# ztaylor797/APMBackend

Hardware: AMD Instinct MI355X
Metric: log-lines/sec z-scored (whole node) (higher is better)
Workload: dtype fp64

## Files before the change

### apmbackend_amd/csrc/kernels/devjoin.hip

```cpp
#include "kernel_api.h"

#include <rocprim/rocprim.hpp>

#include <chrono>
#include <climits>
#include <cstdlib>
#include <cstddef>
#include <cstring>
#include <vector>

#include "devjoin_api.h"
#include "devjoin_dev.h"
#include "devscan.h"
#include "prim.h"
#include "textout.h"

namespace apm {
using namespace dj;

namespace {

constexpr int TB = 256;

__device__ __forceinline__ uint32_t grid_n(uint32_t n) { return (n + TB - 1) / TB; }
// ... 330 lines not shown
          f.flags = PRE_SOAP_VALID;
        }
      }
      return 1;
    }
  }
  return 0;
}

enum : uint8_t { SEL_HOST = 1, SEL_MH = 2, SEL_WALK = 4 };

constexpr int SEL_MH_SHIFT = 22, SEL_WALK_SHIFT = 43;
__device__ __forceinline__ SelCount sel_unpack(uint64_t v) {
  return SelCount{(uint32_t)(v & ((1ull << SEL_MH_SHIFT) - 1)),
                  (uint32_t)((v >> SEL_MH_SHIFT) & ((1ull << (SEL_WALK_SHIFT - SEL_MH_SHIFT)) - 1)),
                  (uint32_t)(v >> SEL_WALK_SHIFT), 0u};
}

constexpr int HF_SLOT = 256;
constexpr int HF_PITCH = HF_SLOT + 16;

__device__ __forceinline__ bool hf_needs_bytes(const Event& e) {
  if (e.kind == LK_APP) return !(e.mask & PM_HOST);
  if (e.mask & PM_HOST) return false;
  if (e.kind == LK_CT_EXIT) return (e.mask & PM_KEYS) && e.ntok >= 3 && (e.mask & PM_BAF);
  if (e.kind == LK_SOAP) return (e.mask & (PM_SOAP_IN | PM_SOAP_ACCT | PM_SOAP_VALUE)) != 0;
  return false;
}

__device__ __forceinline__ uint8_t hf_fields(const Event& e, const uint8_t* __restrict__ p, uint64_t fkey, AudF* aud,
                                             uint32_t i) {
  uint8_t fl = 0;
  if (e.kind == LK_APP) {
    bool host = (e.mask & PM_HOST) != 0;
    if (!host) {
      AudF f;
      host = !aud_fields(e, p, fkey, f);
      if (!host) aud[i] = f;
    }
    if (host) fl |= SEL_HOST;
  } else {
    AudF f;
    const int r = pre_fields(e, p, f);
    if (r < 0) fl |= SEL_HOST;
    else if (r > 0) aud[i] = f;
  }
  return fl;
}

__device__ __forceinline__ uint32_t wave_append(bool want, uint32_t* counter) {
  const uint64_t m = __ballot(want);
  if (!m) return ~0u;
  const uint32_t lane = threadIdx.x & (APM_WAVE - 1);
  const uint32_t leader = (uint32_t)__ffsll((unsigned long long)m) - 1u;
  uint32_t base = 0;
  if (lane == leader) base = atomicAdd(counter, (uint32_t)__popcll(m));
  base = (uint32_t)__shfl((int)base, (int)leader, APM_WAVE);
  return want ? base + (uint32_t)__popcll(m & ((1ull << lane) - 1ull)) : ~0u;
}

__device__ __forceinline__ uint64_t sel_pack(uint8_t fl) {
  return (uint64_t)(fl & SEL_HOST) | ((fl & SEL_MH) ? 1ull << SEL_MH_SHIFT : 0ull) |
         ((fl & SEL_WALK) ? 1ull << SEL_WALK_SHIFT : 0ull);
}

__device__ __forceinline__ uint8_t app_bits(const Event& e) {
  if (e.kind != LK_APP) return 0;
  return (e.mask & PM_AUTR_MAP) ? SEL_MH : (uint8_t)(SEL_WALK | ((e.mask & PM_AUTR_HDR) ? SEL_MH : 0));
}

__device__ __forceinline__ uint8_t hf_event(const Event& e, uint32_t i, const uint8_t* __restrict__ bytes,
                                            const uint32_t* __restrict__ chunk_file,
                                            const uint64_t* __restrict__ file_fkey, AudF* __restrict__ aud,
                                            uint8_t* stage) {
  const uint64_t fkey = e.kind == LK_APP ? file_fkey[chunk_file[e.chunk]] : 0;
  const uint8_t* p = bytes + e.off;
  const uint32_t lead = e.off & 15u;
  const uint32_t nvec = (lead + e.len + 15u) >> 4;
  if (hf_needs_bytes(e) && nvec * 16u <= (uint32_t)HF_SLOT) {
    const uint4* __restrict__ src = reinterpret_cast<const uint4*>(bytes + (e.off - lead));
    uint4* dst = reinterpret_cast<uint4*>(stage + threadIdx.x * HF_PITCH);
    for (uint32_t k = 0; k < nvec; k += 4) {
      const uint4 v0 = src[k];
      const uint4 v1 = k + 1 < nvec ? src[k + 1] : v0;
      const uint4 v2 = k + 2 < nvec ? src[k + 2] : v0;
      const uint4 v3 = k + 3 < nvec ? src[k + 3] : v0;
      dst[k] = v0;
      if (k + 1 < nvec) dst[k + 1] = v1;
      if (k + 2 < nvec) dst[k + 2] = v2;
      if (k + 3 < nvec) dst[k + 3] = v3;
    }
    p = stage + threadIdx.x * HF_PITCH + lead;
  }
  return (uint8_t)(hf_fields(e, p, fkey, aud, i) | app_bits(e));
}

__global__ __launch_bounds__(TB) void k_host_flags(const Event* __restrict__ ev, const uint32_t* __restrict__ n_ev_dev,
                                                   const uint8_t* __restrict__ bytes,
                                                   uint8_t* __restrict__ flag, uint64_t* __restrict__ val,
                                                   AudF* __restrict__ aud, SelCount* __restrict__ totals, uint32_t cap,
                                                   uint32_t* __restrict__ list, uint32_t* __restrict__ list_n) {
  const uint32_t i = blockIdx.x * blockDim.x + threadIdx.x;
  const uint32_t n = min(*n_ev_dev, cap);
  if (blockIdx.x * blockDim.x >= n) return;
  uint32_t ab = 0;
  Event e;
  bool defer = false, front = false;
  if (i < n) {
    e = ev[i];
    if (e.kind == LK_APP && (e.mask & (PM_AUTR_MAP | PM_SW_NAME))) ab = e.len;
    defer = hf_needs_bytes(e);
    front = defer && e.kind == LK_APP;
  }
  const uint32_t f = wave_append(front, &list_n[0]);
  const uint32_t b = wave_append(defer && !front, &list_n[1]);
  if (front) list[f] = i;
  if (defer && !front) list[cap - 1 - b] = i;
  if (i < n && !defer) {
    const uint8_t fl = (uint8_t)(hf_fields(e, bytes + e.off, 0, aud, i) | app_bits(e));
    flag[i] = fl;
    val[i] = sel_pack(fl);
  }
  for (int o = APM_WAVE / 2; o > 0; o >>= 1) ab += __shfl_xor(ab, o, APM_WAVE);
  if ((threadIdx.x & (APM_WAVE - 1)) == 0 && ab) atomicAdd(&totals->aud_bytes, ab);
}

__global__ __launch_bounds__(TB) void k_host_flags_bytes(const Event* __restrict__ ev, const uint8_t* __restrict__ bytes,
                                                         const uint32_t* __restrict__ chunk_file,
                                                         const uint64_t* __restrict__ file_fkey,
                                                         uint8_t* __restrict__ flag, uint64_t* __restrict__ val,
                                                         AudF* __restrict__ aud, uint32_t cap,
                                                         const uint32_t* __restrict__ list,
                                                         const uint32_t* __restrict__ list_n) {
  __shared__ __attribute__((aligned(16))) uint8_t stage[TB * HF_PITCH];
  const uint32_t nf = list_n[0], nb = list_n[1];
  const uint32_t b0 = blockIdx.x * blockDim.x, b1 = b0 + blockDim.x;
  if (b0 >= nf && b1 <= cap - nb) return;
  const uint32_t t = b0 + threadIdx.x;
  if (t >= cap || (t >= nf && t < cap - nb)) return;
  const uint32_t i = list[t];
  const Event e = ev[i];
  const uint8_t fl = hf_event(e, i, bytes, chunk_file, file_fkey, aud, stage);
  flag[i] = fl;
  val[i] = sel_pack(fl);
}

struct SelValF {
  const uint64_t* val;
  __device__ uint64_t operator()(uint32_t i) const { return val[i]; }
};
struct SelScatterG {
  const Event* ev;
  const uint8_t* flag;
  const uint64_t* total;
  Event* out;
  uint32_t *out_idx, *mh_idx, *walk_idx;
  SelCount* totals;
  __device__ void operator()(uint32_t i, uint64_t pos) const {
    if (i == 0) {
      const SelCount t = sel_unpack(*total);
      totals->host = t.host; totals->mh = t.mh; totals->walk = t.walk;
    }
    const uint8_t fl = flag[i];
    if (!fl) return;
    const SelCount p = sel_unpack(pos);
    if (fl & SEL_HOST) { out[p.host] = ev[i]; out_idx[p.host] = i; }
    if (fl & SEL_MH) mh_idx[p.mh] = i;
    if (fl & SEL_WALK) walk_idx[p.walk] = i;
  }
};

enum : uint8_t { SC_NONE = 0, SC_IN = 1, SC_OUT = 2, SC_ACCT = 3, SC_KEY = 4, SC_VALUE = 5 };

__device__ const HostOp* find_hop(const HostOp* __restrict__ h, uint32_t n, uint32_t ev) {
  uint32_t lo = 0, hi = n;
  while (lo < hi) {
    const uint32_t mid = (lo + hi) >> 1;
    if (h[mid].ev < ev) lo = mid + 1; else hi = mid;
  }
  return (lo < n && h[lo].ev == ev) ? &h[lo] : nullptr;
}

__global__ __launch_bounds__(TB) void k_build_ops(DJArgs a) {
  const uint32_t i = blockIdx.x * blockDim.x + threadIdx.x;
  if (i >= a.n_ev) return;
  const Event e = a.ev[i];
  JOp op;
  op.gkey = 0; op.svc = 0; op.ts = apm_nan(); op.num = apm_nan(); op.aux = apm_nan(); op.aux2 = apm_nan();
  op.line = e.line; op.lid = 0; op.svc_ref = 0; op.lid_len = 0; op.svc_len = 0;
  op.flags = 0; op.op = JOP_NONE; op.pad = 0;
  const int32_t file = (int32_t)a.chunk_file[e.chunk];
  const int32_t server = a.file_server[file];
  const uint64_t skey = a.file_skey[file];
  op.server = server;
  uint8_t code = SC_NONE;
  double snum = apm_nan();
  uint64_t shash = 0;
  const uint8_t* p = a.bytes + e.off;
  if (e.kind == LK_APP) {
    AudF f;
    bool ok = false;
    if (a.host_flag[i] & SEL_HOST) {
      const HostOp* h = find_hop(a.hops, a.n_hops, i);
      if (h && h->kind == HOP_AUD) { f = *reinterpret_cast<const AudF*>(&h->op); ok = true; }
      if (!ok) {
        f.h_item = 0; f.el = apm_nan(); f.h_sw = 0; f.ts = apm_nan(); f.ref = 0; f.len = 0; f.flags = 0;
      }
      a.aud[i] = f;
    } else {
      f = a.aud[i];
    }
    if ((e.mask & PM_AUTR_MAP) && (f.flags & AF_ACCT)) {
      if (!(f.flags & AF_ACCT_VALID)) {
        atomicAdd(&a.counts->invalid_acct, 1ULL);
      } else if (f.len > 0) {
        op.op = JOP_ACCT;
        op.gkey = gkey_of(f.h_sw, skey);
        op.num = f.el;
      }
    }
  } else if (a.host_flag[i] & SEL_HOST) {
    const HostOp* h = find_hop(a.hops, a.n_hops, i);
    if (h) {
      switch (h->kind) {
        case HOP_JOIN: op = h->op; break;
        case HOP_SOAP_IN: code = SC_IN; shash = h->lid_hash; break;
        case HOP_SOAP_OUT: code = SC_OUT; break;
        case HOP_SOAP_ACCT: if (h->op.flags & JF_BAF_VALID) { code = SC_ACCT; snum = h->op.num; } break;
        case HOP_SOAP_KEY: code = SC_KEY; break;
        case HOP_SOAP_VALUE: if (h->op.flags & JF_BAF_VALID) { code = SC_VALUE; snum = h->op.num; } break;
        default: break;
      }
    }
  } else if (e.kind >= LK_EJB_ENTRY && e.kind <= LK_CT_EXIT) {
    const bool ejb = e.kind <= LK_EJB_EXIT;
    const bool entry = e.kind == LK_EJB_ENTRY || e.kind == LK_CT_ENTRY;
    op.lid = e.off + e.t0s;
    op.lid_len = (uint16_t)(e.t0e - e.t0s);
    op.svc = e.svc;
    op.flags = JF_HAS_SVC | (ejb ? JF_EJB : 0);
    if (e.tAs == 0xffff) op.flags |= JF_SVC_UNDEF;
    else { op.svc_ref = e.off + e.tAs; op.svc_len = (uint16_t)(e.tAe - e.tAs); }
    op.ts = e.ts;
    const bool empty_lid = op.lid_len == 0;
    if (entry) {
      if (!empty_lid) { op.op = JOP_ENTRY; op.gkey = gkey_of(e.key, skey); }
      else op.flags = 0;
    } else {
      op.num = (e.kind == LK_EJB_EXIT || e.tBs != 0xffff) ? e.num : apm_nan();
      if (e.kind == LK_CT_EXIT && (e.mask & PM_BAF)) {
        const AudF& f = a.aud[i];
        if (f.flags & PRE_BAF) {
          op.flags |= JF_BAF;
          op.aux = f.el;
          if (f.flags & PRE_BAF_VALID) { op.flags |= JF_BAF_VALID; op.aux2 = f.el; }
        }
      }
      if (empty_lid) op.op = JOP_DIRECT;
      else { op.op = e.kind == LK_EJB_EXIT ? JOP_EJB_EXIT : JOP_CT_EXIT; op.gkey = gkey_of(e.key, skey); }
    }
  } else if (e.kind == LK_SOAP) {
    const uint32_t m = e.mask;
    if (m & PM_SOAP_IN) {
      code = SC_IN;
      shash = a.aud[i].h_item;
    } else if (m & PM_SOAP_OUT) {
      code = SC_OUT;
    } else if (m & (PM_SOAP_ACCT | PM_SOAP_KEY | PM_SOAP_VALUE)) {
      const bool acct = m & PM_SOAP_ACCT;
      if (!acct && (m & PM_SOAP_KEY)) {
        code = SC_KEY;
      } else {
        const AudF& f = a.aud[i];
        if (f.flags & PRE_SOAP_VALID) {
          snum = f.el;
          code = acct ? SC_ACCT : SC_VALUE;
        }
      }
    }
  }
  a.ops[i] = op;
  a.soap_code[i] = code;
  a.soap_num[i] = snum;
  a.soap_hash[i] = shash;
}

constexpr uint32_t F_CONST = 1u << 31;
constexpr uint32_t F_ID = 1u | (2u << 2);
constexpr uint32_t F_KEY = 2u | (2u << 2);
constexpr uint32_t F_VALUE = 1u | (0u << 2);

__device__ __forceinline__ uint32_t map_tag(uint32_t g, uint32_t tag) {
  return tag == 0 ? 0u : (tag == 1 ? (g & 3u) : ((g >> 2) & 3u));
}
__device__ __forceinline__ uint32_t fcompose(uint32_t g, uint32_t f) {
  if (g & F_CONST) return g;
  if (f & F_CONST) {
    const uint32_t t = map_tag(g, f & 3u);
    return t ? (F_CONST | t | (f & ~(F_CONST | 3u))) : F_CONST;
  }
  return map_tag(g, f & 3u) | (map_tag(g, (f >> 2) & 3u) << 2);
}
__device__ __forceinline__ uint32_t code_fn(uint8_t c, uint32_t ev) {
  switch (c) {
    case SC_IN: return F_CONST | 1u | ((ev + 1) << 2);
    case SC_OUT: case SC_ACCT: return F_CONST;
    case SC_KEY: return F_KEY;
    case SC_VALUE: return F_VALUE;
    default: return F_ID;
  }
}

__device__ __forceinline__ void soap_range(const uint32_t* lo_tab, uint32_t c, int g, uint32_t& lo, uint32_t& hi) {
  const uint32_t c0 = lo_tab[c], c1 = lo_tab[c + 1];
  const uint32_t n = c1 - c0;
  const uint32_t seg = ((n + SOAP_SEGS - 1) / SOAP_SEGS + APM_WAVE - 1) / APM_WAVE * APM_WAVE;
  lo = min(c1, c0 + (uint32_t)g * seg);
  hi = min(c1, lo + seg);
}

__device__ __forceinline__ uint32_t wave_fscan(uint32_t f, int lane) {
// ... 744 lines not shown

constexpr uint32_t GWB_LDS = 4096;
constexpr int GWB_THREADS = 256;
__global__ __launch_bounds__(GWB_THREADS) void k_group_walk_big(DJArgs a) {
  __shared__ uint32_t lds[GWB_LDS];
  __shared__ uint32_t s_g, s_off;
  const uint32_t nb = a.big[0];
  for (uint32_t b = blockIdx.x; b < nb; b += gridDim.x) {
    const uint32_t slot = a.op_slot_sorted[b];
    if (threadIdx.x == 0) {
      uint32_t g = 0;
      for (uint32_t j = a.slot_head[slot]; j != ~0u; j = a.op_idx[j]) ++g;
      const uint32_t off = atomicAdd(&a.big[1], g);
      uint32_t k = 0;
      for (uint32_t j = a.slot_head[slot]; j != ~0u; j = a.op_idx[j]) a.op_idx_sorted[off + k++] = j;
      a.slot_head[slot] = ~0u;
      s_g = g;
      s_off = off;
    }
    __syncthreads();
    const uint32_t g = s_g;
    uint32_t* v = a.op_idx_sorted + s_off;
    if (g <= GWB_LDS) {
      for (uint32_t t = threadIdx.x; t < g; t += blockDim.x) lds[t] = v[t];
      __syncthreads();
      v = lds;
    }
    block_sort_asc(v, g);
    if (threadIdx.x == 0) walk_group(a, slot, [v](uint32_t q) { return v[q]; }, g);
    __syncthreads();
  }
}

template <class M>
__device__ void walk_group(DJArgs& a, uint32_t slot, const M& mem, uint32_t g) {
  KeyState ks = a.table[slot];
  const double now = a.now;
  bool acct_live = ks.acct_exp >= now;
  if (!(ks.rec_exp >= now) && ks.n_part > 0) {
    atomicAdd(&a.counts->expired_partials, (unsigned long long)ks.n_part);
    part_clear(a, ks);
  }
  NeedEnt* ne = nullptr;
  int32_t nidx = -1;
  if (ks.need >= 0) {
    NeedEnt* c = &a.arena[ks.need];
    if (c->key == ks.key && c->exp >= now) { ne = c; nidx = ks.need; }
  }
  for (uint32_t q = 0; q < g; ++q) {
    const uint32_t ev = mem(q);
    const JOp op = a.ops[ev];
    Emitter em{a.stage, a.ovf, &a.counts->pad[0], ev, 0};
    const bool ts_empty = (op.flags & JF_TS_EMPTY) != 0;
    switch (op.op) {
      case JOP_ENTRY: {
        if (!(ks.rec_exp >= now)) { ks.rec_exp = now + a.rec_ttl; part_clear(a, ks); }
        const int f = part_find(a, ks, op.svc);
        if (f >= 0) part_set(a, ks, f, op.svc, op.ts);
        else if (!part_append(a, ks, op.svc, op.ts)) atomicAdd(&a.counts->partial_overflow, 1ULL);
        break;
      }
      case JOP_EJB_EXIT:
      case JOP_CT_EXIT: {
        const bool ct = op.op == JOP_CT_EXIT;
        const int f = (ks.rec_exp >= now) ? part_find(a, ks, op.svc) : -1;
        if (f < 0) {
          if (!ct) { atomicAdd(&a.counts->ejb_unmatched, 1ULL); break; }
          if ((op.flags & JF_BAF) && (op.flags & JF_BAF_VALID)) {
            ks.acct = op.aux2; ks.acct_exp = now + a.acct_ttl; acct_live = true;
            if (ne && ne->n) need_drain(a, *ne, nidx, op.aux2, em);
          } else if (op.flags & JF_BAF) {
            atomicAdd(&a.counts->invalid_acct, 1ULL);
          }
          em.put(make_tx(op.server, op.svc, LID_NONE, 0, 0, (op.flags & JF_BAF) ? op.aux : apm_nan(), 0.0, true,
                         op.ts, ts_empty, op.num, false));
          break;
        }
        const double pstart = part_get_start(a, ks, f);
        auto remove_part = [&]() { part_remove(a, ks, f); };
        if (acct_live) {
          remove_part();
          em.put(make_tx(op.server, op.svc, lid_src_of(op), op.lid, op.lid_len, ks.acct, pstart, false, op.ts,
                         ts_empty, op.num, false));
          break;
        }
        if (!ne) { nidx = need_alloc(a, op, ks.key); ne = nidx >= 0 ? &a.arena[nidx] : nullptr; ks.need = nidx; }
        double alt = apm_nan();
        if (ct && (op.flags & JF_BAF)) {
          alt = op.aux;
          if (op.flags & JF_BAF_VALID) {
            ks.acct = op.aux2; ks.acct_exp = now + a.acct_ttl; acct_live = true;
            if (ne && ne->n) need_drain(a, *ne, nidx, op.aux2, em);
          } else {
            atomicAdd(&a.counts->invalid_acct, 1ULL);
          }
        }
        if (ne) {
          NeedItem it;
          it.svc = op.svc; it.start = pstart; it.end = op.ts; it.elapsed = op.num; it.alt = alt;
          it.flags = ts_empty ? JF_TS_EMPTY : 0; it.pad = 0;
          need_put(a, *ne, it);
        }
        remove_part();
        break;
      }
      case JOP_ACCT: {
        ks.acct = op.num; ks.acct_exp = now + a.acct_ttl; acct_live = true;
        if (ne && ne->n) need_drain(a, *ne, nidx, op.num, em);
        break;
      }
      case JOP_AUDIT_TX: {
        const bool to_db = (op.flags & JF_TO_DB) != 0;
        if (acct_live) {
          em.put(make_tx(op.server, op.svc, lid_src_of(op), op.lid, op.lid_len, ks.acct, op.aux,
                         (op.flags & JF_START_EMPTY) != 0, op.ts, ts_empty, op.num, to_db));
          break;
        }
        if (!ne) { nidx = need_alloc(a, op, ks.key); ne = nidx >= 0 ? &a.arena[nidx] : nullptr; ks.need = nidx; }
        if (ne) {
          NeedItem it;
          it.svc = op.svc; it.start = op.aux; it.end = op.ts; it.elapsed = op.num; it.alt = op.aux2;
          it.flags = (ts_empty ? JF_TS_EMPTY : 0) | ((op.flags & JF_START_EMPTY) ? JF_START_EMPTY : 0) | (to_db ? JF_TO_DB : 0);
          it.pad = 0;
          need_put(a, *ne, it);
        }
        break;
      }
      default: break;
    }
    a.out_cnt[ev] = em.sub;
  }
  a.table[slot] = ks;
}

__global__ __launch_bounds__(TB) void k_exp_keys(DJArgs a) {
  const uint32_t e = blockIdx.x * blockDim.x + threadIdx.x;
  if (e >= a.n_exp_entries) return;
  uint64_t rem = e, v = 0;
  for (uint32_t r = 0; r < a.n_exp_regions; ++r) {
    const uint64_t n = a.exp_hi[r] - a.exp_lo[r];
    if (rem < n) { v = a.exp_lo[r] + rem; break; }
    rem -= n;
  }
  const uint32_t idx = (uint32_t)(v & (uint64_t)(a.arena_cap - 1));
  const NeedEnt& ne = a.arena[idx];
  a.exp_key[e] = ne.n > 0 ? ne.created : ~0ULL;
  a.exp_idx[e] = idx;
  if (ne.n == 0) {
    a.arena[idx].key = 0;
    if (ne.lblk) chain_free(a.pool, a.pool_ring, a.pool_mask, a.counts, ne.lblk);
  }
}

__global__ __launch_bounds__(TB) void k_exp_count(DJArgs a) {
  const uint32_t e = blockIdx.x * blockDim.x + threadIdx.x;
  if (e > a.n_exp_entries) return;
  if (e == a.n_exp_entries) { a.exp_cnt[e] = 0; return; }
  a.exp_cnt[e] = a.exp_key_sorted[e] == ~0ULL ? 0u : (uint32_t)a.arena[a.exp_idx_sorted[e]].n;
}

__global__ void k_exp_emit(DJArgs a) {
  const uint32_t e = blockIdx.x * blockDim.x + threadIdx.x;
  if (e == 0) {
    a.counts->n_exp_out = a.n_exp_entries ? a.exp_pos[a.n_exp_entries] : 0;
    atomicAdd(&a.counts->need_expired, (unsigned long long)a.counts->n_exp_out);
  }
  if (e >= a.n_exp_entries) return;
  const uint32_t n = a.exp_cnt[e];
  if (!n) return;
  const uint32_t idx = a.exp_idx_sorted[e];
  NeedEnt& ne = a.arena[idx];
  const uint32_t base = a.exp_pos[e];
  int32_t b = 0;
  for (uint32_t k = 0; k < n && base + k < a.out_cap; ++k) {
    const NeedItem& r = need_item(a.pool, ne, (int)k, b);
    a.out[base + k] = make_tx(ne.server, r.svc, LID_NEED, idx, (uint32_t)ne.lid_len, r.alt, r.start,
                              (r.flags & JF_START_EMPTY) != 0, r.end, (r.flags & JF_TS_EMPTY) != 0, r.elapsed,
                              (r.flags & JF_TO_DB) != 0);
  }
  if (ne.iblk) chain_free(a.pool, a.pool_ring, a.pool_mask, a.counts, ne.iblk);
  if (ne.lblk) chain_free(a.pool, a.pool_ring, a.pool_mask, a.counts, ne.lblk);
  ne.iblk = 0;
  ne.n = 0;
  ne.key = 0;
}

__global__ __launch_bounds__(TB) void k_place(DJArgs a) {
  const uint32_t i = blockIdx.x * blockDim.x + threadIdx.x;
  const uint32_t base = a.counts->n_exp_out;
  if (i == 0) a.counts->n_out = base + a.out_pos[a.n_ev];
  if (i >= a.n_ev * 2) return;
  const uint32_t ev = i >> 1, sub = i & 1;
  if (sub >= a.out_cnt[ev]) return;
  const uint32_t p = base + a.out_pos[ev] + sub;
  if (p < a.out_cap) a.out[p] = a.stage[(size_t)ev * 2 + sub];
}

__global__ __launch_bounds__(TB) void k_place_ovf(DJArgs a) {
  const uint32_t k = blockIdx.x * blockDim.x + threadIdx.x;
  const uint32_t n = min(a.counts->pad[0], DJ_OVF_CAP);
  if (k >= n) return;
  const DJOverflow& o = a.ovf[k];
  const uint32_t p = a.counts->n_exp_out + a.out_pos[o.ev] + o.sub;
  if (p < a.out_cap) a.out[p] = o.t;
}

struct U4 {
  uint32_t x, y, z, w;
};
struct U4Plus {
  __device__ __host__ U4 operator()(const U4& a, const U4& b) const { return U4{a.x + b.x, a.y + b.y, a.z + b.z, a.w + b.w}; }
};

__device__ __forceinline__ const char* lid_ptr(const DJFormatArgs& f, const TxDev& t) {
  switch (t.lid_src) {
    case LID_BATCH: return (const char*)f.bytes + t.lid;
    case LID_HOST: return (const char*)f.hbuf + t.lid;
    case LID_NEED: return f.arena[t.lid & (f.arena_cap - 1)].lid;
    case LID_AUD: return f.aud_txt + t.lid;
    default: return "";
  }
}

__device__ __forceinline__ bool stat_usable(const TxDev& t) { return !t.to_db && t.end == t.end && t.end >= 10000.0; }

__device__ uint32_t line_len(const DJFormatArgs& f, const TxDev& t) {
  if (t.raw < 0) return 0;
  const RawSvc rs = f.raw[t.raw];
  uint32_t n = 3 + rs.srv_len + 1 + rs.norm_len + 1 + t.lid_len + 1;
  n += js_num(nullptr, t.acct, nullptr) + 1 + js_num(nullptr, t.start, nullptr) + 1 + js_num(nullptr, t.end, nullptr) +
       1 + js_num(nullptr, t.elapsed, nullptr) + 1 + 1;
  return n + 1;
}

__global__ __launch_bounds__(TB) void k_resolve_len(DJFormatArgs f) {
  const uint32_t i = blockIdx.x * blockDim.x + threadIdx.x;
  const uint32_t n = f.n_out;
  U4* lens = reinterpret_cast<U4*>(f.lens);
  if (i == n) { lens[n] = U4{0, 0, 0, 0}; return; }
  if (i > n) return;
  TxDev t = f.out[i];
  const int32_t raw = reg_find(f.reg, f.reg_mask, regkey_of(t.svc, t.server));
  t.raw = raw >= 0 ? raw : -1;
  f.out[i].raw = t.raw;
  const uint32_t len = line_len(f, t);
  const bool st = stat_usable(t);
  lens[i] = U4{len, st ? 1u : 0u, t.to_db ? 0u : len, t.to_db ? len : 0u};
  if (t.to_db) atomicAdd(&f.counts->n_db, 1u);
  else if (!st) atomicAdd(&f.counts->n_dropped, 1u);
}

__global__ void k_plan_totals(DJFormatArgs f) {
  const U4 o = reinterpret_cast<const U4*>(f.offs)[f.n_out];
  f.counts->text_bytes = o.x;
  f.counts->n_stats = o.y;
  f.counts->tx_text_bytes = o.z;
  f.counts->db_text_bytes = o.w;
  const uint64_t base = ring_place(f.ring_head, o.x, f.ring_cap);
  uint32_t v = DJ_WRITE_OK;
  if ((uint64_t)o.x > f.ring_cap / 4) v = DJ_WRITE_TOO_BIG;
  else if (base + o.x > f.ring_low + f.ring_cap) v = DJ_WRITE_RING_FULL;
  else if ((f.want_tx && o.z > f.txt_cap) || (f.want_db && o.w > f.txt_cap)) v = DJ_WRITE_TXT;
  *f.ring_pos = base;
  f.counts->pad[1] = v;
}

__device__ __forceinline__ uint32_t tx_head_len(const TxDev& t, const RawSvc& rs) {
  return 3u + rs.srv_len + 1u + rs.norm_len + 1u + t.lid_len + 1u;
}
template <class O>
__device__ __forceinline__ void tx_line_head(const DJFormatArgs& f, const TxDev& t, const RawSvc& rs, O& o);
template <class O>
__device__ __forceinline__ void tx_line_tail(const TxDev& t, const RawSvc& rs, O& o, bool& inexact) {
  o.jsnum(t.acct, inexact); o.c('|');
  o.jsnum(t.start, inexact); o.c('|');
  o.jsnum(t.end, inexact); o.c('|');
  o.jsnum(t.elapsed, inexact); o.c('|');
  o.c(rs.toplevel ? 'Y' : 'N');
  o.c('\n');
}
template <class O>
__device__ __forceinline__ void tx_line(const DJFormatArgs& f, const TxDev& t, const RawSvc& rs, O& o, bool& inexact) {
  tx_line_head(f, t, rs, o);
  tx_line_tail(t, rs, o, inexact);
}
template <class O>
__device__ __forceinline__ void tx_line_head(const DJFormatArgs& f, const TxDev& t, const RawSvc& rs, O& o) {
  o.lit("tx|");
  o.s(f.names + rs.srv_off, rs.srv_len);
  o.c('|');
  o.s(f.names + rs.norm_off, rs.norm_len);
  o.c('|');
  if (t.lid_src != LID_NEED || t.lid_len <= NEED_LID) {
    o.s(lid_ptr(f, t), t.lid_len);
  } else {
    const NeedEnt& ne = f.arena[t.lid & (f.arena_cap - 1)];
    o.s((const char*)ne.lid, NEED_LID);
    int rem = (int)t.lid_len - NEED_LID;
    for (int32_t b = ne.lblk; b && rem > 0; b = blk_next(f.pool, b)) {
      const LidBlk* lb = (const LidBlk*)blk_ptr(f.pool, b);
      const int m = rem < LBLK_N ? rem : LBLK_N;
      o.s((const char*)lb->b, m);
      rem -= m;
    }
  }
  o.c('|');
}

constexpr int TXW_LINES = 64;
constexpr int TXW_THREADS = 2 * TXW_LINES;
constexpr uint32_t TXW_LDS = 8192;
__device__ __forceinline__ void write_one(const DJFormatArgs& f, const TxDev& t, uint32_t i, uint64_t ring_base,
                                          char* staged_line);
__device__ __forceinline__ void write_tail(const DJFormatArgs& f, const TxDev& t, uint32_t i, uint64_t ring_base,
                                           char* staged_line);

__device__ __forceinline__ void txw_copy_out(const char* __restrict__ lds, char* __restrict__ out, uint32_t g0,
                                             uint32_t g1) {
  const uint32_t a0 = g0 & ~3u;
  const uint32_t nd = (g1 - a0 + 3) / 4;
  for (uint32_t d = threadIdx.x; d < nd; d += blockDim.x) {
    const uint32_t ga = a0 + 4 * d;
    if (ga >= g0 && ga + 4 <= g1) {
      *reinterpret_cast<uint32_t*>(out + ga) = *reinterpret_cast<const uint32_t*>(lds + 4 * d);
    } else {
      for (uint32_t b = 0; b < 4; ++b)
        if (ga + b >= g0 && ga + b < g1) out[ga + b] = lds[4 * d + b];
    }
  }
}

__global__ __launch_bounds__(TXW_THREADS) void k_write(DJFormatArgs f) {
  __shared__ __align__(16) char stage[TXW_LDS];
  if (f.counts->pad[1] != DJ_WRITE_OK) return;
  const uint64_t ring_base = *f.ring_pos;
  const uint32_t j0 = blockIdx.x * TXW_LINES;
  const uint32_t j1 = min(f.n_out, j0 + TXW_LINES);
  const bool tail = threadIdx.x >= (unsigned)TXW_LINES;
  const uint32_t i = j0 + (threadIdx.x & (TXW_LINES - 1));
  const U4* offs = reinterpret_cast<const U4*>(f.offs);
  const uint64_t rb = ring_base & (f.ring_cap - 1);
  const uint32_t p0 = (uint32_t)(rb + offs[j0].x), p1 = (uint32_t)(rb + offs[j1].x);
  const bool staged = p1 - (p0 & ~3u) <= TXW_LDS;
  if (i < j1) {
    const TxDev t = f.out[i];
    char* const sl = staged ? stage + ((uint32_t)(rb + offs[i].x) - (p0 & ~3u)) : nullptr;
    if (t.raw >= 0) {
      if (tail) write_tail(f, t, i, ring_base, sl);
      else write_one(f, t, i, ring_base, sl);
    }
  }
  if (staged) {
    __syncthreads();
    txw_copy_out(stage, f.ring, p0, p1);
  }
}

__device__ __forceinline__ void write_tail(const DJFormatArgs& f, const TxDev& t, uint32_t i, uint64_t ring_base,
                                           char* staged_line) {
  const U4 o = reinterpret_cast<const U4*>(f.offs)[i];
  const uint64_t vpos = ring_base + o.x;
  char* p0 = staged_line ? staged_line : f.ring + (vpos & (f.ring_cap - 1));
  const RawSvc rs = f.raw[t.raw];
  bool inexact = false;
  OutT<true> w(p0 + tx_head_len(t, rs));
  tx_line_tail(t, rs, w, inexact);
  w.finish();
}

__device__ __forceinline__ void write_one(const DJFormatArgs& f, const TxDev& t, uint32_t i, uint64_t ring_base,
                                          char* staged_line) {
  const U4 o = reinterpret_cast<const U4*>(f.offs)[i];
  const U4 l = reinterpret_cast<const U4*>(f.lens)[i];
  const uint64_t vpos = ring_base + o.x;
  char* p0 = staged_line ? staged_line : f.ring + (vpos & (f.ring_cap - 1));
  const RawSvc rs = f.raw[t.raw];
  bool inexact = false;
  {
    OutT<true> w(p0);
    tx_line_head(f, t, rs, w);
    w.finish();
  }
  const uint32_t len = l.x;
  if (f.want_tx && !t.to_db) {
    OutT<true> w(f.txt_tx + o.z);
    tx_line(f, t, rs, w, inexact);
    w.finish();
  }
  if (f.want_db && t.to_db) {
    OutT<true> w(f.txt_db + o.w);
    tx_line(f, t, rs, w, inexact);
    w.finish();
  }
  if (l.y) {
    const uint32_t j = o.y;
    TxRec r;
    r.end_ms = (int64_t)t.end;
    const int32_t s = f.raw_series[t.raw];
    r.series = s;
    const double e = t.elapsed;
    r.elapsed = (e == e && e >= -2147483647.0 && e <= 2147483647.0) ? (int32_t)e : ELAPSED_NAN;
    f.tx[j] = r;
    f.tx_raw[j] = t.raw;
    f.tx_gid[j] = (int64_t)((vpos << 20) | (uint64_t)(len - 1));
    f.tx_bucket[j] = r.end_ms / 10000;
    if (s < 0) atomicMin(&f.raw_first[t.raw], (int32_t)j);
  }
}

__global__ __launch_bounds__(TB) void k_cands(DJFormatArgs f) {
  const uint32_t j = blockIdx.x * blockDim.x + threadIdx.x;
  if (f.counts->pad[1] != DJ_WRITE_OK || j >= f.counts->n_stats) return;
  if (j == 0 || f.tx_bmax[j] > f.tx_bmax[j - 1]) {
    const uint32_t k = atomicAdd(&f.counts->n_cand, 1u);
    f.cand[k] = j;
    f.cand_bucket[k] = f.tx_bucket[j];
  }
  const int32_t r = f.tx_raw[j];
  if (f.raw_first[r] == (int32_t)j) {
    const uint32_t k = atomicAdd(&f.counts->n_unresolved, 1u);
    f.unresolved[2 * k] = j;
    f.unresolved[2 * k + 1] = (uint32_t)r;
  }
}

__global__ void k_reset_first(DJFormatArgs f) {
  const uint32_t j = blockIdx.x * blockDim.x + threadIdx.x;
  if (f.counts->pad[1] != DJ_WRITE_OK || j >= f.counts->n_stats) return;
  const int32_t r = f.tx_raw[j];
  if (f.raw_first[r] != INT_MAX) f.raw_first[r] = INT_MAX;
}

__global__ void k_rebuild(const KeyState* __restrict__ old, uint32_t old_cap, KeyState* __restrict__ fresh,
                          uint32_t mask, const NeedEnt* __restrict__ arena, uint32_t arena_cap, double now,
                          JoinCounts* cnt, unsigned long long* live, const uint8_t* pool, uint32_t* pool_ring,
                          uint32_t pool_mask) {
  const uint32_t i = blockIdx.x * blockDim.x + threadIdx.x;
  if (i >= old_cap) return;
  KeyState s = old[i];
  if (!s.key) return;
  const bool rec = s.rec_exp >= now && s.n_part > 0;
  const bool acct = s.acct_exp >= now;
  bool need = false;
  if (s.need >= 0) {
    const NeedEnt& ne = arena[(uint32_t)s.need & (arena_cap - 1)];
    need = ne.key == s.key && ne.exp >= now;
  }
  if (!rec && s.n_part > 0 && !(s.rec_exp >= now)) atomicAdd(&cnt->expired_partials, (unsigned long long)s.n_part);
  if (!rec && s.pblk) {
    chain_free(pool, pool_ring, pool_mask, cnt, s.pblk);
    s.pblk = 0;
  }
  if (!rec && !acct && !need) return;
  if (!(s.rec_exp >= now)) s.n_part = 0;
  uint32_t h = home_of(s.key, mask);
  for (uint32_t probe = 0; probe <= mask; ++probe) {
    const uint32_t idx = (h + probe) & mask;
    if (atomicCAS((unsigned long long*)&fresh[idx].key, 0ULL, (unsigned long long)s.key) == 0ULL) {
      fresh[idx] = s;
      atomicAdd(live, 1ULL);
      return;
    }
  }
}

constexpr uint32_t RB_SEG = 8;

__global__ void k_rebuild_starts(const KeyState* __restrict__ t, uint32_t cap, uint32_t* __restrict__ starts) {
  const uint32_t seg = blockIdx.x * blockDim.x + threadIdx.x;
  const uint32_t n_seg = cap / RB_SEG;
  if (seg >= n_seg) return;
  const uint32_t mask = cap - 1, lo = seg * RB_SEG, hi = lo + RB_SEG;
  uint32_t p = lo;
  if (t[(lo + mask) & mask].key != 0)
    while (p < hi && t[p].key != 0) ++p;
  starts[seg] = p;
}

__device__ __forceinline__ bool rb_live(KeyState& s, const NeedEnt* __restrict__ arena, uint32_t arena_cap, double now,
                                        JoinCounts* cnt, const uint8_t* pool, uint32_t* pool_ring, uint32_t pool_mask,
                                        bool& changed) {
  const bool rec = s.rec_exp >= now && s.n_part > 0;
  const bool acct = s.acct_exp >= now;
  bool need = false;
  if (s.need >= 0) {
    const NeedEnt& ne = arena[(uint32_t)s.need & (arena_cap - 1)];
    need = ne.key == s.key && ne.exp >= now;
  }
  if (!rec && s.n_part > 0 && !(s.rec_exp >= now)) atomicAdd(&cnt->expired_partials, (unsigned long long)s.n_part);
  if (!rec && s.pblk) {
    chain_free(pool, pool_ring, pool_mask, cnt, s.pblk);
    s.pblk = 0;
    changed = true;
  }
  if (!rec && !acct && !need) return false;
  if (!(s.rec_exp >= now) && s.n_part != 0) { s.n_part = 0; changed = true; }
  return true;
}

constexpr int RB_TB = 128;
constexpr int RB_BITS = 1024;
__global__ __launch_bounds__(RB_TB) void k_rebuild_inplace(KeyState* __restrict__ t, uint32_t cap,
                                                           const uint32_t* __restrict__ starts,
                                                           const NeedEnt* __restrict__ arena, uint32_t arena_cap,
                                                           double now, JoinCounts* cnt, unsigned long long* live,
                                                           const uint8_t* pool, uint32_t* pool_ring, uint32_t pool_mask) {
  __shared__ uint32_t occ_s[RB_TB][RB_BITS / 32];
  uint32_t* occ = occ_s[threadIdx.x];
  const uint32_t seg = blockIdx.x * blockDim.x + threadIdx.x;
  const uint32_t n_seg = cap / RB_SEG;
  uint32_t n_live = 0;
  if (seg < n_seg) {
    const uint32_t mask = cap - 1, hi = seg * RB_SEG + RB_SEG;
    uint64_t p = starts[seg];
    while (p < hi) {
      if (t[p & mask].key == 0) { ++p; continue; }
      uint64_t q = p;
      while (t[q & mask].key != 0 && q < p + cap) ++q;
      const uint32_t L = (uint32_t)(q - p);
      if (L > RB_BITS) {
        n_live += L;
        p = q + 1;
        continue;
      }
      for (uint32_t i = 0; i < (L + 31) / 32; ++i) occ[i] = 0;
      for (uint64_t r = p; r < q; ++r) {
        KeyState s = t[r & mask];
        bool changed = false;
        if (!rb_live(s, arena, arena_cap, now, cnt, pool, pool_ring, pool_mask, changed)) continue;
        uint32_t i = (uint32_t)(r - (((uint32_t)r - home_of(s.key, mask)) & mask) - p);
        while (i < L && (occ[i >> 5] & (1u << (i & 31)))) ++i;
        if (i >= L) i = (uint32_t)(r - p);
        occ[i >> 5] |= 1u << (i & 31);
        if (p + i != r || changed) t[(p + i) & mask] = s;
        ++n_live;
      }
      for (uint32_t i = 0; i < L; ++i)
        if (!(occ[i >> 5] & (1u << (i & 31)))) t[(p + i) & mask].key = 0;
      p = q + 1;
    }
  }
  for (int o = APM_WAVE / 2; o > 0; o >>= 1) n_live += __shfl_xor(n_live, o, APM_WAVE);
  if ((threadIdx.x & (APM_WAVE - 1)) == 0 && n_live) atomicAdd(live, (unsigned long long)n_live);
}

__global__ __launch_bounds__(TB) void k_rebase_gids(const int64_t* __restrict__ gid, int64_t n,
                                                    const uint32_t* __restrict__ offs, uint64_t base,
                                                    int64_t* __restrict__ out) {
  const int64_t i = (int64_t)blockIdx.x * blockDim.x + threadIdx.x;
  if (i < n) out[i] = (int64_t)(((base + offs[i]) << 20) | ((uint64_t)gid[i] & 0xfffffu));
}

__global__ void k_gather_len(const int64_t* __restrict__ gid, int64_t n_upper, const int64_t* __restrict__ d_n,
                             uint32_t* __restrict__ lens) {
  const int64_t i = (int64_t)blockIdx.x * blockDim.x + threadIdx.x;
  if (i > n_upper) return;
  const int64_t n = d_n ? *d_n : n_upper;
  lens[i] = i >= n ? 0u : (uint32_t)((uint64_t)gid[i] & 0xfffffu) + 1u;
}

constexpr int GL_LINES = 128;
constexpr int GL_TB = 256;

__device__ __forceinline__ uint4 window16(const uint32_t (&w)[8], uint32_t o) {
  const uint32_t q = o >> 2, rb = o & 3u;
  uint32_t d[5];
#pragma unroll
  for (int k = 0; k < 5; ++k) {
    const uint32_t a0 = w[k < 8 ? k : 7], a1 = w[k + 1 < 8 ? k + 1 : 7], a2 = w[k + 2 < 8 ? k + 2 : 7],
                   a3 = w[k + 3 < 8 ? k + 3 : 7], a4 = w[k + 4 < 8 ? k + 4 : 7];
    d[k] = q == 0 ? a0 : q == 1 ? a1 : q == 2 ? a2 : q == 3 ? a3 : a4;
  }
  uint4 r;
  r.x = __builtin_amdgcn_alignbyte(d[1], d[0], rb);
  r.y = __builtin_amdgcn_alignbyte(d[2], d[1], rb);
  r.z = __builtin_amdgcn_alignbyte(d[3], d[2], rb);
  r.w = __builtin_amdgcn_alignbyte(d[4], d[3], rb);
  return r;
}

__device__ __forceinline__ uint4 load_line16(const char* p, uint32_t avail) {
  const uint32_t sh = (uint32_t)((uintptr_t)p & 15u);
  const uint4* pa = reinterpret_cast<const uint4*>(p - sh);
  const uint4 v0 = pa[0];
  const uint4 v1 = sh + avail > 16u ? pa[1] : v0;
  const uint32_t w[8] = {v0.x, v0.y, v0.z, v0.w, v1.x, v1.y, v1.z, v1.w};
  return window16(w, sh);
}

__device__ __forceinline__ uint4 merge16(uint4 a, uint4 b, uint32_t k) {
  auto m = [k](uint32_t x, uint32_t y, uint32_t i) -> uint32_t {
    const uint32_t lo = 4u * i;
    if (k >= lo + 4u) return x;
    if (k <= lo) return y;
    const uint32_t mask = (1u << (8u * (k - lo))) - 1u;
    return (x & mask) | (y & ~mask);
  };
  return make_uint4(m(a.x, b.x, 0), m(a.y, b.y, 1), m(a.z, b.z, 2), m(a.w, b.w, 3));
}

__global__ __launch_bounds__(GL_TB) void k_gather_lines(const int64_t* __restrict__ gid, int64_t n,
                                                        const char* __restrict__ ring, uint64_t ring_cap,
                                                        const uint32_t* __restrict__ offs, char* __restrict__ out) {
  __shared__ uint32_t s_off[GL_LINES + 1];
  __shared__ uint64_t s_src[GL_LINES];
  const int64_t l0 = (int64_t)blockIdx.x * GL_LINES;
  const int cnt = (int)min<int64_t>(GL_LINES, n - l0);
  for (int i = threadIdx.x; i <= cnt; i += GL_TB) s_off[i] = offs[l0 + i];
  for (int i = threadIdx.x; i < cnt; i += GL_TB) s_src[i] = ((uint64_t)gid[l0 + i] >> 20) & (ring_cap - 1);
  __syncthreads();
  const uint32_t O0 = s_off[0], O1 = s_off[cnt];
  const uint32_t c0 = O0 >> 4, c1 = (O1 + 15u) >> 4;
  int lo_hint = 0;
  for (uint32_t c = c0 + threadIdx.x; c < c1; c += GL_TB) {
    const uint32_t p = c << 4;
    const uint32_t q = p < O0 ? O0 : p;
    int lo = lo_hint, hi = cnt;
    while (hi - lo > 1) {
      const int mid = (lo + hi) >> 1;
      if (s_off[mid] <= q) lo = mid; else hi = mid;
    }
    lo_hint = lo;
    if (p >= O0 && p + 16u <= O1) {
      const uint32_t eA = s_off[lo + 1];
      const char* a = ring + s_src[lo] + (p - s_off[lo]);
      if (p + 16u <= eA) {
        *reinterpret_cast<uint4*>(out + p) = load_line16(a, 16u);
        continue;
      }
      if (lo + 2 <= cnt && p + 16u <= s_off[lo + 2]) {
        const uint32_t dA = eA - p;
        const uint4 va = load_line16(a, dA);
        const uint4 vb = load_line16(ring + s_src[lo + 1], 16u - dA);
        const uint32_t w[8] = {0u, 0u, 0u, 0u, vb.x, vb.y, vb.z, vb.w};
        *reinterpret_cast<uint4*>(out + p) = merge16(va, window16(w, 16u - dA), dA);
        continue;
      }
    }
    int l = lo;
    for (uint32_t k = 0; k < 16u; ++k) {
      const uint32_t pos = p + k;
      if (pos < O0) continue;
      if (pos >= O1) break;
      while (pos >= s_off[l + 1]) ++l;
      out[pos] = ring[s_src[l] + (pos - s_off[l])];
    }
  }
}

__global__ __launch_bounds__(256) void k_cache_stats(const KeyState* __restrict__ t, uint32_t cap, double now,
                                                     unsigned long long* __restrict__ out) {
  unsigned long long c[5] = {0, 0, 0, 0, 0};
  for (uint32_t i = blockIdx.x * blockDim.x + threadIdx.x; i < cap; i += gridDim.x * blockDim.x) {
    const KeyState& k = t[i];
    if (!k.key) continue;
    c[0] += 1;
    c[1] += k.acct_exp >= now;
    const bool rec = k.rec_exp >= now && k.n_part > 0;
    c[2] += rec;
    c[3] += rec ? (unsigned long long)k.n_part : 0ull;
    c[4] += k.need >= 0;
  }
  for (int j = 0; j < 5; ++j) {
    unsigned long long v = c[j];
    for (int o = APM_WAVE / 2; o > 0; o >>= 1) v += __shfl_xor(v, o, APM_WAVE);
    if ((threadIdx.x & (APM_WAVE - 1)) == 0 && v) atomicAdd(out + j, v);
  }
}

__global__ __launch_bounds__(1024) void k_min_pos(const int64_t* __restrict__ gid, int64_t n, unsigned long long* out) {
  __shared__ unsigned long long red[1024 / APM_WAVE];
  unsigned long long v = ~0ULL;
  const int64_t stride = (int64_t)gridDim.x * blockDim.x;
  int64_t i = (int64_t)blockIdx.x * blockDim.x + threadIdx.x;
  for (; i + 3 * stride < n; i += 4 * stride) {
    const uint64_t g0 = (uint64_t)gid[i], g1 = (uint64_t)gid[i + stride];
    const uint64_t g2 = (uint64_t)gid[i + 2 * stride], g3 = (uint64_t)gid[i + 3 * stride];
    const unsigned long long a = (g0 >> 20) < (g1 >> 20) ? (g0 >> 20) : (g1 >> 20);
    const unsigned long long b = (g2 >> 20) < (g3 >> 20) ? (g2 >> 20) : (g3 >> 20);
    const unsigned long long m = a < b ? a : b;
    v = m < v ? m : v;
  }
  for (; i < n; i += stride) {
    const unsigned long long p = (unsigned long long)((uint64_t)gid[i] >> 20);
    v = p < v ? p : v;
  }
  for (int o = APM_WAVE / 2; o > 0; o >>= 1) {
    const unsigned long long x = __shfl_xor(v, o, APM_WAVE);
    v = x < v ? x : v;
  }
  if ((threadIdx.x & (APM_WAVE - 1)) == 0) red[threadIdx.x / APM_WAVE] = v;
  __syncthreads();
  if (threadIdx.x == 0) {
    for (int w = 1; w < (int)(blockDim.x / APM_WAVE); ++w) v = red[w] < v ? red[w] : v;
    if (v != ~0ULL) atomicMin(out, v);
  }
}

__global__ void k_relocate(int64_t* __restrict__ gid, int64_t n, char* __restrict__ ring, uint64_t ring_cap,
                           uint64_t below, uint64_t dst_base, unsigned long long* cursor) {
  const int64_t w = ((int64_t)blockIdx.x * blockDim.x + threadIdx.x) / APM_WAVE;
  const int lane = threadIdx.x & (APM_WAVE - 1);
  if (w >= n) return;
  const uint64_t g = (uint64_t)gid[w];
  const uint64_t pos = g >> 20;
  if (pos >= below) return;
  const uint32_t len = (uint32_t)(g & 0xfffffu) + 1u;
  unsigned long long at = 0;
  if (lane == 0) at = atomicAdd(cursor, (unsigned long long)len);
  at = __shfl(at, 0, APM_WAVE);
  const uint64_t np = dst_base + at;
  const char* src = ring + (pos & (ring_cap - 1));
  char* dst = ring + (np & (ring_cap - 1));
  for (uint32_t k = lane; k < len; k += APM_WAVE) dst[k] = src[k];
  if (lane == 0) gid[w] = (int64_t)((np << 20) | (g & 0xfffffu));
}

__global__ void k_pool_fix(JoinCounts* c) {
  const unsigned long long h = c->pool_head, t = c->pool_tail;
  c->pool_head = h < t ? h : t;
  c->pool_tail = c->pool_ptail;
}

__global__ void k_pool_init(uint32_t* ring, uint32_t n, JoinCounts* c) {
  const uint32_t i = blockIdx.x * blockDim.x + threadIdx.x;
  if (i < n) ring[i] = i;
  if (i == 0) { c->pool_head = 0; c->pool_tail = n; c->pool_ptail = n; }
}

__global__ void k_pool_grow(const uint32_t* __restrict__ old_ring, uint32_t old_mask, uint32_t* __restrict__ fresh,
                            uint32_t old_n, uint32_t new_n, const JoinCounts* c) {
  const uint32_t i = blockIdx.x * blockDim.x + threadIdx.x;
  const unsigned long long head = c->pool_head;
  const uint32_t avail = (uint32_t)(c->pool_tail - head);
  if (i < avail) fresh[i] = old_ring[(head + i) & old_mask];
  else if (i < avail + (new_n - old_n)) fresh[i] = old_n + (i - avail);
}

__global__ void k_pool_grow_set(JoinCounts* c, uint32_t old_n, uint32_t new_n) {
  const unsigned long long avail = c->pool_tail - c->pool_head;
  c->pool_head = 0;
  c->pool_tail = c->pool_ptail = avail + (new_n - old_n);
}

__global__ void k_arena_move(const NeedEnt* __restrict__ old, uint32_t old_cap, NeedEnt* __restrict__ fresh,
                             uint32_t fresh_cap, uint64_t lo, uint64_t n) {
  constexpr int Q = sizeof(NeedEnt) / 16;
  const uint64_t t = (uint64_t)blockIdx.x * blockDim.x + threadIdx.x;
  const uint64_t e = t / Q;
  if (e >= n) return;
  const uint64_t v = lo + e;
  const uint4* s = reinterpret_cast<const uint4*>(old + (v & (old_cap - 1)));
  uint4* d = reinterpret_cast<uint4*>(fresh + (v & (fresh_cap - 1)));
  d[t % Q] = s[t % Q];
}

__global__ void k_arena_remap(KeyState* __restrict__ table, uint32_t cap, const NeedEnt* __restrict__ old,
                              uint32_t old_cap, uint32_t fresh_cap, uint64_t lo, uint64_t hi) {
  const uint32_t i = blockIdx.x * blockDim.x + threadIdx.x;
  if (i >= cap) return;
  KeyState& s = table[i];
  if (!s.key || s.need < 0) return;
  const NeedEnt& ne = old[(uint32_t)s.need & (old_cap - 1)];
  s.need = (ne.key == s.key && ne.vidx >= lo && ne.vidx < hi) ? (int32_t)(ne.vidx & (fresh_cap - 1)) : -1;
}

__global__ void k_gather_blocks(const uint8_t* __restrict__ pool, const int32_t* __restrict__ idx, uint32_t n,
                                uint8_t* __restrict__ out) {
  const uint32_t t = blockIdx.x * blockDim.x + threadIdx.x;
  constexpr uint32_t Q = CHAIN_BLK / 16;
  if (t >= n * Q) return;
  const uint32_t b = t / Q, q = t % Q;
  reinterpret_cast<uint4*>(out)[(size_t)b * Q + q] =
      reinterpret_cast<const uint4*>(pool + (size_t)(idx[b] - 1) * CHAIN_BLK)[q];
}

__global__ void k_reg_fill(RegSlot* __restrict__ reg, const int32_t* __restrict__ pairs, uint32_t n) {
  const uint32_t i = blockIdx.x * blockDim.x + threadIdx.x;
  if (i < n) reg[pairs[2 * i]].raw = pairs[2 * i + 1];
}

__global__ void k_scatter_i32(int32_t* __restrict__ dst, const int32_t* __restrict__ pairs, uint32_t n) {
  const uint32_t i = blockIdx.x * blockDim.x + threadIdx.x;
  if (i < n) dst[pairs[2 * i]] = pairs[2 * i + 1];
}

__global__ void k_fill_series(TxRec* __restrict__ tx, const int32_t* __restrict__ raw, uint32_t n,
                              const int32_t* __restrict__ raw_series, unsigned long long* __restrict__ unmapped) {
  const uint32_t i = blockIdx.x * blockDim.x + threadIdx.x;
  if (i >= n) return;
  if (tx[i].series >= 0) return;
  const int32_t s = raw_series[raw[i]];
  tx[i].series = s;
  if (s < 0 && unmapped) atomicAdd(unmapped, 1ULL);
}

__global__ void k_gather_u8(const uint8_t* __restrict__ src, const int32_t* __restrict__ idx, uint32_t n,
                            uint8_t* __restrict__ out) {
  const uint32_t i = blockIdx.x * blockDim.x + threadIdx.x;
  if (i < n) out[i] = src[idx[i]];
}

__global__ void k_count_le(const int64_t* __restrict__ end, int64_t n, int64_t edge, int64_t* __restrict__ out) {
  int64_t lo = 0, hi = n;
  while (lo < hi) {
    const int64_t mid = (lo + hi) >> 1;
    if (end[mid] <= edge) lo = mid + 1; else hi = mid;
  }
  *out = lo;
}

__global__ void k_keys_sync(const KeyState* __restrict__ t, uint32_t cap, uint64_t* __restrict__ keys) {
  const uint32_t i = blockIdx.x * blockDim.x + threadIdx.x;
  if (i < cap) keys[i] = t[i].key;
}

}
}

extern "C" {
using namespace apm;

static bool dj_marks_on() {
  static const bool v = [] { const char* e = std::getenv("APM_DJ_MARKS"); return e && e[0] == '1'; }();
  return v;
}
constexpr int DJ_MARKS = 64;
static double g_mark_t[DJ_MARKS];
static const char* g_mark_n[DJ_MARKS];
static int g_mark_k = 0;

static void dj_check(hipStream_t s, const char* what) {
  if (dj_marks_on() && g_mark_k < DJ_MARKS) {
    g_mark_t[g_mark_k] =
        std::chrono::duration<double, std::milli>(std::chrono::steady_clock::now().time_since_epoch()).count();
    g_mark_n[g_mark_k++] = what;
  }
  static const bool dbg = std::getenv("APM_DJ_DEBUG") != nullptr;
  if (!dbg) return;
  const hipError_t e = hipStreamSynchronize(s);
  if (e != hipSuccess) {
    fprintf(stderr, "[devjoin debug] %s: %s\n", what, hipGetErrorString(e));
    fflush(stderr);
    abort();
  }
}

__global__ void k_gather_field(const uint8_t* __restrict__ base, size_t stride, uint32_t n, int words,
                               uint32_t* __restrict__ out) {
  const uint32_t i = blockIdx.x * blockDim.x + threadIdx.x;
  if (i >= n) return;
  const uint32_t* p = reinterpret_cast<const uint32_t*>(base + (size_t)i * stride);
  for (int k = 0; k < words; ++k) out[(size_t)i * words + k] = p[k];
}

void apm_dj_gather_field(const void* base, size_t stride, uint32_t n, int words, uint32_t* out, hipStream_t s) {
  if (!n) return;
  hipLaunchKernelGGL(k_gather_field, dim3((n + TB - 1) / TB), dim3(TB), 0, s, (const uint8_t*)base, stride, n, words, out);
}

int apm_dj_take_marks(double* t, const char** names, int cap) {
  const int k = std::min(g_mark_k, cap);
  for (int i = 0; i < k; ++i) { t[i] = g_mark_t[i]; names[i] = g_mark_n[i]; }
  g_mark_k = 0;
  return k;
}

static int dj_sort_keys(PrimScratch& sc, const uint64_t* key, uint64_t* key_sorted, const uint32_t* val,
                        uint32_t* val_sorted, size_t n, hipStream_t s) {
  return prim_sort_pairs(sc, key, key_sorted, val, val_sorted, n, s);
}
static int dj_scan_counts(PrimScratch& sc, const uint32_t* cnt, uint32_t* pos, size_t n, hipStream_t s) {
  return prim_exclusive_scan(sc, cnt, pos, 0u, n, rocprim::plus<uint32_t>(), s);
}
static int dj_scan_lens(PrimScratch& sc, const U4* lens, U4* offs, size_t n, hipStream_t s) {
  return prim_exclusive_scan(sc, lens, offs, U4{0, 0, 0, 0}, n, U4Plus(), s);
}
static int dj_scan_bucket_max(PrimScratch& sc, const int64_t* bucket, int64_t* bmax, size_t n, hipStream_t s) {
  return prim_inclusive_scan(sc, bucket, bmax, n, rocprim::maximum<int64_t>(), s);
}

size_t apm_dj_tmp_bytes(uint32_t max_ev, uint32_t max_out) {
  PrimScratch q;
  const size_t n = std::max<size_t>(max_ev, 1) + 1;
  dj_sort_keys(q, nullptr, nullptr, nullptr, nullptr, n, 0);
  dj_scan_counts(q, nullptr, nullptr, n, 0);
  dj_scan_lens(q, nullptr, nullptr, (size_t)max_out + 1, 0);
  dj_scan_bucket_max(q, nullptr, nullptr, (size_t)max_out + 1, 0);
  return q.need + 4096;
}

int apm_dj_select_host(DJArgs* a, const uint32_t* d_n_ev, uint32_t max_ev, hipStream_t s) {
  if (max_ev == 0) return 0;
  uint32_t* list = reinterpret_cast<uint32_t*>(a->sel_pos);
  uint32_t* list_n = dj_select_list_n(a->sel_pos, max_ev);
  const dim3 grid((max_ev + TB - 1) / TB);
  hipLaunchKernelGGL(k_host_flags, grid, dim3(TB), 0, s, a->ev, d_n_ev, a->bytes, a->host_flag, a->sel_val, a->aud,
                     a->n_host, max_ev, list, list_n);
  dj_check(s, "k_host_flags");
  hipLaunchKernelGGL(k_host_flags_bytes, grid, dim3(TB), 0, s, a->ev, a->bytes, a->chunk_file, a->file_fkey,
                     a->host_flag, a->sel_val, a->aud, max_ev, list, list_n);
  dj_check(s, "k_host_flags_bytes");
  uint64_t* total = a->sel_pos + (max_ev + DS_TILE - 1) / DS_TILE + 1;
  if (ds_scan_apply<uint64_t>(SelValF{a->sel_val},
                              SelScatterG{a->ev, a->host_flag, total, a->host_ev, a->host_ev_idx, a->mh_idx,
                                          a->walk_idx, a->n_host},
                              d_n_ev, max_ev, a->sel_pos, total, s) != 0)
    return -1;
  dj_check(s, "k_ds_scan (host selection)");
  return 0;
}

static int apm_dj_audit(DJArgs* a, bool filled, hipStream_t s) {
  if (a->n_files && !filled) HIP_OK(hipMemsetAsync(a->gout.carry, 0, (size_t)a->n_files * sizeof(AudCarry), s));
  const uint32_t N = a->gin.n_autr + a->n_mh;
  if (N) {
    hipLaunchKernelGGL(k_aud_keys, dim3((N + TB - 1) / TB), dim3(TB), 0, s, *a);
    dj_check(s, "k_aud_keys");
    PrimScratch sc(a->tmp, a->tmp_bytes);
    if (dj_sort_keys(sc, a->aud_key, a->aud_key_sorted, a->aud_ord, a->aud_ord_sorted, N, s) != 0) return -1;
    dj_check(s, "rocprim_radix_sort_pairs");
    hipLaunchKernelGGL(k_aud_autr, dim3((N + TB - 1) / TB), dim3(TB), 0, s, *a);
    dj_check(s, "k_aud_autr");
  }
  if (a->n_walk || a->gin.n_txt) {
    if (a->n_files && !filled) HIP_OK(hipMemsetAsync(a->file_first_chunk, 0xff, (size_t)a->n_files * 4, s));
    const uint32_t lanes = std::max(a->n_chunks + 1, a->n_walk + 1);
    hipLaunchKernelGGL(k_aud_chunks, dim3((lanes + TB - 1) / TB), dim3(TB), 0, s, *a);
    dj_check(s, "k_aud_chunks");
    const uint32_t L = a->n_walk + a->n_files;
    hipLaunchKernelGGL(k_aud_walk, dim3((L + 63) / 64), dim3(64), 0, s, *a);
    dj_check(s, "k_aud_walk");
  }
  return 0;
}

int apm_dj_join(DJArgs* a, hipStream_t s) {
  const uint32_t n = a->n_ev;
  PrimScratch sc(a->tmp, a->tmp_bytes);
  static_assert(offsetof(JoinCounts, ejb_unmatched) % 4 == 0, "JoinCounts zero range");
  const uint32_t zw = (uint32_t)(offsetof(JoinCounts, ejb_unmatched) / 4);
  if (n) {
    static_assert(sizeof(AudCarry) % 4 == 0, "carry words");
    const uint32_t cw = a->n_files * (uint32_t)(sizeof(AudCarry) / 4);
    const uint32_t lanes = std::max(std::max(std::max(a->n_chunks + 1, n + 1), zw), cw);
    hipLaunchKernelGGL(k_chunk_events, dim3((lanes + TB - 1) / TB), dim3(TB), 0, s, a->ev, n, a->n_chunks,
                       a->chunk_ev_lo, (uint32_t*)a->counts, zw, a->out_cnt, (uint32_t*)a->gout.carry, cw,
                       (uint32_t*)a->file_first_chunk, a->n_files);
    dj_check(s, "k_chunk_events");
    hipLaunchKernelGGL(k_build_ops, dim3((n + TB - 1) / TB), dim3(TB), 0, s, *a);
    dj_check(s, "k_build_ops");
  } else {
    HIP_OK(hipMemsetAsync(a->counts, 0, offsetof(JoinCounts, ejb_unmatched), s));
  }
  if (apm_dj_audit(a, n != 0, s) != 0) return -1;
  if (n) {
    hipLaunchKernelGGL(k_soap_summary, dim3(a->n_chunks, SOAP_SEGS), dim3(APM_WAVE), 0, s, *a);
    dj_check(s, "k_soap_summary");
    hipLaunchKernelGGL(k_soap_carry, dim3((a->n_chunks + 63) / 64), dim3(64), 0, s, *a);
    dj_check(s, "k_soap_carry");
    hipLaunchKernelGGL(k_soap_apply, dim3(a->n_chunks, SOAP_SEGS), dim3(APM_WAVE), 0, s, *a);
    dj_check(s, "k_soap_apply");
    hipLaunchKernelGGL(k_claim, dim3((n + TB - 1) / TB), dim3(TB), 0, s, *a);
    dj_check(s, "k_claim");
  }
  const uint32_t E = a->n_exp_entries;
  if (E) {
    hipLaunchKernelGGL(k_exp_keys, dim3((E + TB - 1) / TB), dim3(TB), 0, s, *a);
    dj_check(s, "k_exp_keys");
    if (dj_sort_keys(sc, a->exp_key, a->exp_key_sorted, a->exp_idx, a->exp_idx_sorted, E, s) != 0) return -1;
    dj_check(s, "rocprim_radix_sort_pairs");
    hipLaunchKernelGGL(k_exp_count, dim3((E + 1 + TB - 1) / TB), dim3(TB), 0, s, *a);
    dj_check(s, "k_exp_count");
    if (dj_scan_counts(sc, a->exp_cnt, a->exp_pos, (size_t)E + 1, s) != 0) return -1;
    dj_check(s, "rocprim_exclusive_scan");
  }
  hipLaunchKernelGGL(k_exp_emit, dim3((std::max<uint32_t>(E, 1) + TB - 1) / TB), dim3(TB), 0, s, *a);
  dj_check(s, "k_exp_emit");
  if (n) {
    hipLaunchKernelGGL(k_group_walk, dim3((n + TB - 1) / TB), dim3(TB), 0, s, *a);
    dj_check(s, "k_group_walk");
    hipLaunchKernelGGL(k_group_walk_big, dim3(32), dim3(GWB_THREADS), 0, s, *a);
    dj_check(s, "k_group_walk_big");
    if (dj_scan_counts(sc, a->out_cnt, a->out_pos, (size_t)n + 1, s) != 0) return -1;
    dj_check(s, "rocprim_exclusive_scan");
    hipLaunchKernelGGL(k_place, dim3((2 * n + TB - 1) / TB), dim3(TB), 0, s, *a);
    dj_check(s, "k_place");
    hipLaunchKernelGGL(k_place_ovf, dim3(DJ_OVF_CAP / TB), dim3(TB), 0, s, *a);
    dj_check(s, "k_place_ovf");
  } else {
    HIP_OK(hipMemsetAsync(a->out_pos, 0, 4, s));
    hipLaunchKernelGGL(k_place, dim3(1), dim3(TB), 0, s, *a);
    dj_check(s, "k_place");
  }
  hipLaunchKernelGGL(k_pool_fix, dim3(1), dim3(1), 0, s, a->counts);
  dj_check(s, "k_pool_fix");
  return 0;
}

int apm_dj_plan(DJFormatArgs* f, hipStream_t s) {
  const uint32_t n = f->n_out;
  hipLaunchKernelGGL(k_resolve_len, dim3((n + 1 + TB - 1) / TB), dim3(TB), 0, s, *f);
  dj_check(s, "k_resolve_len");
  PrimScratch sc(f->tmp, f->tmp_bytes);
  if (dj_scan_lens(sc, reinterpret_cast<const U4*>(f->lens), reinterpret_cast<U4*>(f->offs), (size_t)n + 1, s) != 0)
    return -1;
  dj_check(s, "rocprim_exclusive_scan (plan)");
  hipLaunchKernelGGL(k_plan_totals, dim3(1), dim3(1), 0, s, *f);
  dj_check(s, "k_plan_totals");
  return 0;
}

int apm_dj_write(DJFormatArgs* f, hipStream_t s) {
  const uint32_t n = f->n_out;
  if (!n) return 0;
  hipLaunchKernelGGL(k_write, dim3((n + TXW_LINES - 1) / TXW_LINES), dim3(TXW_THREADS), 0, s, *f);
  dj_check(s, "k_write");
  PrimScratch sc(f->tmp, f->tmp_bytes);
  if (dj_scan_bucket_max(sc, f->tx_bucket, f->tx_bmax, (size_t)n, s) != 0) return -1;
  dj_check(s, "rocprim_inclusive_scan (bucket max)");
  hipLaunchKernelGGL(k_cands, dim3((n + TB - 1) / TB), dim3(TB), 0, s, *f);
  hipLaunchKernelGGL(k_reset_first, dim3((n + TB - 1) / TB), dim3(TB), 0, s, *f);
  dj_check(s, "k_cands+k_reset_first");
  return 0;
}

namespace {
struct KeyLive {
  __device__ bool operator()(const KeyState& k) const { return k.key != 0; }
};
}

static int dj_select_live(PrimScratch& sc, const KeyState* table, uint32_t cap, KeyState* out, uint32_t* d_n,
                          hipStream_t s) {
  return prim_select(sc, table, out, d_n, cap, KeyLive(), s);
}

size_t apm_dj_live_tmp_bytes(uint32_t cap) {
  PrimScratch q;
  dj_select_live(q, nullptr, cap, nullptr, nullptr, 0);
  return q.need;
}

void apm_dj_live_compact(const KeyState* table, uint32_t cap, KeyState* out, uint32_t* d_n, void* tmp,
                         size_t tmp_bytes, hipStream_t s) {
  PrimScratch sc(tmp, tmp_bytes);
  if (dj_select_live(sc, table, cap, out, d_n, s) != 0)
    throw std::runtime_error("live compaction: scratch smaller than apm_dj_live_tmp_bytes(cap)");
}

size_t apm_dj_rebuild_scratch_bytes(uint32_t cap) { return ((size_t)cap / RB_SEG + 1) * 4; }

void apm_dj_rebuild_inplace(KeyState* table, uint32_t cap, uint32_t* scratch, const NeedEnt* arena, uint32_t arena_cap,
                            double now, JoinCounts* counts, unsigned long long* live, uint8_t* pool,
                            uint32_t* pool_ring, uint32_t pool_mask, hipStream_t s) {
  if (cap < RB_SEG || (cap & (cap - 1))) throw std::runtime_error("in-place rebuild: table size not a power of two >= 8");
  const uint32_t n_seg = cap / RB_SEG;
  hipLaunchKernelGGL(k_rebuild_starts, dim3((n_seg + TB - 1) / TB), dim3(TB), 0, s, table, cap, scratch);
  dj_check(s, "k_rebuild_starts");
  hipLaunchKernelGGL(k_rebuild_inplace, dim3((n_seg + RB_TB - 1) / RB_TB), dim3(RB_TB), 0, s, table, cap, scratch, arena,
                     arena_cap, now, counts, live, pool, pool_ring, pool_mask);
  dj_check(s, "k_rebuild_inplace");
  hipLaunchKernelGGL(k_pool_fix, dim3(1), dim3(1), 0, s, counts);
}

std::vector<double> apm_dj_rebuild_selftest(uint32_t cap, double load, double dead, uint64_t seed, bool copy) {
  std::vector<KeyState> h(cap);
  std::memset(h.data(), 0, (size_t)cap * sizeof(KeyState));
  const uint32_t mask = cap - 1;
  uint64_t x = seed * 0x9E3779B97F4A7C15ull + 1;
  auto rnd = [&]() { x ^= x >> 12; x ^= x << 25; x ^= x >> 27; return x * 0x2545F4914F6CDD1Dull; };
  const double now = 1000.0;
  const uint32_t n = (uint32_t)(load * cap);
  uint64_t want_live = 0, probes_before = 0;
  for (uint32_t i = 0; i < n; ++i) {
    uint64_t k = rnd() | 1;
    uint32_t idx = home_of(k, mask);
    uint32_t d = 0;
    while (h[idx].key && h[idx].key != k) { idx = (idx + 1) & mask; ++d; }
    if (h[idx].key == k) continue;
    KeyState& e = h[idx];
    e.key = k;
    const bool is_dead = (double)(rnd() >> 11) * (1.0 / 9007199254740992.0) < dead;
    e.acct = (double)(k % 1000003);
    e.acct_exp = is_dead ? now - 1 : now + 10;
    e.rec_exp = -__builtin_inf();
    e.need = -1;
    e.n_part = 0;
    e.pblk = 0;
    want_live += !is_dead;
    probes_before += d;
  }
  KeyState* d_t = nullptr;
  KeyState* d_f = nullptr;
  uint32_t* d_scr = nullptr;
  NeedEnt* d_arena = nullptr;
  JoinCounts* d_c = nullptr;
  unsigned long long* d_live = nullptr;
  HIP_OK(hipMalloc((void**)&d_t, (size_t)cap * sizeof(KeyState)));
  HIP_OK(hipMalloc((void**)&d_f, (size_t)cap * sizeof(KeyState)));
  HIP_OK(hipMalloc((void**)&d_scr, apm_dj_rebuild_scratch_bytes(cap)));
  HIP_OK(hipMalloc((void**)&d_arena, sizeof(NeedEnt)));
  HIP_OK(hipMalloc((void**)&d_c, sizeof(JoinCounts)));
  HIP_OK(hipMalloc((void**)&d_live, 8));
  HIP_OK(hipMemset(d_arena, 0, sizeof(NeedEnt)));
  HIP_OK(hipMemset(d_c, 0, sizeof(JoinCounts)));
  HIP_OK(hipMemset(d_live, 0, 8));
  HIP_OK(hipMemset(d_f, 0, (size_t)cap * sizeof(KeyState)));
  HIP_OK(hipMemcpy(d_t, h.data(), (size_t)cap * sizeof(KeyState), hipMemcpyHostToDevice));
  hipEvent_t e0, e1;
  HIP_OK(hipEventCreate(&e0));
  HIP_OK(hipEventCreate(&e1));
  HIP_OK(hipEventRecord(e0, 0));
  if (copy)
    apm_dj_rebuild(d_t, cap, d_f, mask, d_arena, 1, now, d_c, d_live, nullptr, nullptr, 0, 0);
  else
    apm_dj_rebuild_inplace(d_t, cap, d_scr, d_arena, 1, now, d_c, d_live, nullptr, nullptr, 0, 0);
  HIP_OK(hipEventRecord(e1, 0));
  HIP_OK(hipEventSynchronize(e1));
  float ms = 0;
  HIP_OK(hipEventElapsedTime(&ms, e0, e1));
  unsigned long long live = 0;
  HIP_OK(hipMemcpy(&live, d_live, 8, hipMemcpyDeviceToHost));
  std::vector<KeyState> r(cap);
  HIP_OK(hipMemcpy(r.data(), copy ? d_f : d_t, (size_t)cap * sizeof(KeyState), hipMemcpyDeviceToHost));
  for (void* p : {(void*)d_t, (void*)d_f, (void*)d_scr, (void*)d_arena, (void*)d_c, (void*)d_live}) HIP_OK(hipFree(p));
  HIP_OK(hipEventDestroy(e0));
  HIP_OK(hipEventDestroy(e1));
  uint64_t found = 0, dead_left = 0, occupied = 0, probes_after = 0;
  for (uint32_t i = 0; i < cap; ++i) {
    const KeyState& e = h[i];
    if (!e.key) continue;
    uint32_t idx = home_of(e.key, mask), d = 0;
    while (r[idx].key && r[idx].key != e.key && d <= mask) { idx = (idx + 1) & mask; ++d; }
    const bool there = r[idx].key == e.key;
    if (e.acct_exp >= now) {
      found += there && r[idx].acct == e.acct && r[idx].acct_exp == e.acct_exp && r[idx].need == -1;
      probes_after += d;
    } else {
      dead_left += there;
    }
  }
  for (uint32_t i = 0; i < cap; ++i) occupied += r[i].key != 0;
  return {(double)live, (double)want_live, (double)found, (double)dead_left, (double)occupied, (double)probes_before,
          (double)probes_after, 1000.0 * ms};
}
void apm_dj_rebuild(const KeyState* old, uint32_t old_cap, KeyState* fresh, uint32_t fresh_mask, const NeedEnt* arena,
                    uint32_t arena_cap, double now, JoinCounts* counts, unsigned long long* live, uint8_t* pool,
                    uint32_t* pool_ring, uint32_t pool_mask, hipStream_t s) {
  if (old_cap)
    hipLaunchKernelGGL(k_rebuild, dim3((old_cap + TB - 1) / TB), dim3(TB), 0, s, old, old_cap, fresh, fresh_mask, arena,
                       arena_cap, now, counts, live, pool, pool_ring, pool_mask);
  hipLaunchKernelGGL(k_pool_fix, dim3(1), dim3(1), 0, s, counts);
}

void apm_dj_gather_blocks(const uint8_t* pool, const int32_t* idx, uint32_t n, uint8_t* out, hipStream_t s) {
  if (!n) return;
  const uint32_t t = n * (CHAIN_BLK / 16);
  hipLaunchKernelGGL(k_gather_blocks, dim3((t + TB - 1) / TB), dim3(TB), 0, s, pool, idx, n, out);
}

void apm_dj_pool_init(uint32_t* ring, uint32_t n, JoinCounts* counts, hipStream_t s) {
  hipLaunchKernelGGL(k_pool_init, dim3((n + TB - 1) / TB), dim3(TB), 0, s, ring, n, counts);
}

void apm_dj_pool_grow(const uint32_t* old_ring, uint32_t old_mask, uint32_t* fresh_ring, uint32_t old_n, uint32_t new_n,
                      JoinCounts* counts, hipStream_t s) {
  hipLaunchKernelGGL(k_pool_grow, dim3((new_n + TB - 1) / TB), dim3(TB), 0, s, old_ring, old_mask, fresh_ring, old_n,
                     new_n, counts);
  hipLaunchKernelGGL(k_pool_grow_set, dim3(1), dim3(1), 0, s, counts, old_n, new_n);
}

void apm_dj_arena_grow(const NeedEnt* old, uint32_t old_cap, NeedEnt* fresh, uint32_t fresh_cap, uint64_t lo,
                       uint64_t hi, KeyState* table, uint32_t table_cap, hipStream_t s) {
  const uint64_t n = hi - lo;
  const uint64_t threads = n * (sizeof(NeedEnt) / 16);
// ... 71 lines not shown
```

### apmbackend_amd/csrc/kernels/devjoin_api.h

```cpp
#pragma once
#include <vector>
#include <hip/hip_runtime.h>
#include <stdint.h>

#include "../apm_types.h"
#include "devjoin_types.h"

namespace apm {

constexpr int SOAP_SEGS = 16;
constexpr uint32_t DJ_OVF_CAP = 1u << 16;

enum : uint32_t {
  DJ_WRITE_OK = 0,
  DJ_WRITE_TXT = 1,
  DJ_WRITE_TOO_BIG = 2,
  DJ_WRITE_RING_FULL = 3,
};

__host__ __device__ inline uint64_t ring_place(uint64_t head, uint64_t bytes, uint64_t cap) {
  return ((head & (cap - 1)) + bytes > cap) ? (head + cap - 1) & ~(cap - 1) : head;
}

struct DJOverflow {
  uint32_t ev, sub;
  uint32_t pad[14];
  TxDev t;
};

struct AudGen {
  AudCarry* carry;
  AutrEnt* autr;
  AudItem* items;
  char* txt;
  uint32_t n_autr, n_items, n_txt;
  uint32_t cap_autr, cap_items, cap_txt;
};

struct SelCount {
  uint32_t host;
  uint32_t mh;
  uint32_t walk;
  uint32_t aud_bytes;
};

inline uint32_t* dj_select_list_n(uint64_t* sel_pos, uint32_t max_ev) {
  return reinterpret_cast<uint32_t*>(sel_pos) + max_ev;
}

struct DJArgs {
  const Event* ev;
  uint32_t n_ev;
  const uint8_t* bytes;
  const uint32_t* chunk_file;
  const uint8_t* chunk_kind;
  uint32_t n_chunks;
  const int32_t* chunk_next;
  const uint8_t* chunk_first;
  const int32_t* file_server;
  const uint64_t* file_skey;
  const uint64_t* file_fkey;
  const HostOp* hops;
  uint32_t n_hops;
  const uint8_t* hbuf;
  double now;
  uint64_t batch_no;
  double rec_ttl, acct_ttl, need_ttl;
  uint8_t* host_flag;
  uint64_t* sel_val;
  uint64_t* sel_pos;
  Event* host_ev;
  uint32_t* host_ev_idx;
  uint32_t* mh_idx;
  uint32_t* walk_idx;
  SelCount* n_host;
  uint32_t n_mh, n_walk;
  uint32_t n_files;
  AudF* aud;
  AudGen gin, gout;
  uint64_t* aud_key;
  uint64_t* aud_key_sorted;
  uint32_t* aud_ord;
  uint32_t* aud_ord_sorted;
  uint32_t* walk_lo;
  int32_t* file_first_chunk;
  AudItem* aud_slots;
  JOp* ops;
  uint8_t* soap_code;
  double* soap_num;
  uint64_t* soap_hash;
  uint32_t* chunk_ev_lo;
  uint32_t* seg_f;
  uint32_t* seg_in;
  uint64_t* chain_hash;
  SoapState* soap_state;
  uint32_t* op_slot;
  uint32_t* op_slot_sorted;
  uint32_t* op_idx;
  uint32_t* op_idx_sorted;
  uint32_t* slot_head;
  uint32_t* big;
  void* tmp;
  size_t tmp_bytes;
  KeyState* table;
  uint64_t* keys;
  uint32_t table_mask;
  RegSlot* reg;
  uint32_t reg_mask;
  RegMiss* miss;
  uint32_t miss_cap;
  NeedEnt* arena;
  uint32_t arena_cap;
  uint64_t arena_base;
  uint32_t arena_limit;
  uint8_t* pool;
  uint32_t* pool_ring;
  uint32_t pool_mask;
  const uint64_t* exp_lo;
  const uint64_t* exp_hi;
  uint32_t n_exp_regions;
  uint32_t n_exp_entries;
  uint64_t* exp_key;
  uint64_t* exp_key_sorted;
  uint32_t* exp_idx;
  uint32_t* exp_idx_sorted;
  uint32_t* exp_cnt;
  uint32_t* exp_pos;
  uint32_t* out_cnt;
  uint32_t* out_pos;
  TxDev* stage;
  DJOverflow* ovf;
  TxDev* out;
  uint32_t out_cap;
  JoinCounts* counts;
};

struct DJFormatArgs {
  TxDev* out;
  uint32_t n_out;
  const RegSlot* reg;
  uint32_t reg_mask;
  const RawSvc* raw;
  const int32_t* raw_series;
  int32_t* raw_first;
  const char* names;
  const uint8_t* bytes;
  const uint8_t* hbuf;
  const char* aud_txt;
  const NeedEnt* arena;
  uint32_t arena_cap;
  const uint8_t* pool;
  uint32_t* lens;
  uint32_t* offs;
  char* ring;
  uint64_t ring_cap;
  uint64_t ring_head;
  uint64_t ring_low;
  uint64_t* ring_pos;
  uint64_t txt_cap;
  TxRec* tx;
  int32_t* tx_raw;
  int64_t* tx_gid;
  int64_t* tx_bucket;
  int64_t* tx_bmax;
  uint32_t* cand;
  int64_t* cand_bucket;
  uint32_t* unresolved;
  char* txt_tx;
  char* txt_db;
  int want_tx, want_db;
  JoinCounts* counts;
  void* tmp;
  size_t tmp_bytes;
};

}

extern "C" {
size_t apm_dj_tmp_bytes(uint32_t max_ev, uint32_t max_out);
int apm_dj_take_marks(double* t, const char** names, int cap);
void apm_dj_gather_field(const void* base, size_t stride, uint32_t n, int words, uint32_t* out, hipStream_t s);
int apm_dj_select_host(apm::DJArgs* a, const uint32_t* d_n_ev, uint32_t max_ev, hipStream_t s);
int apm_dj_join(apm::DJArgs* a, hipStream_t s);
int apm_dj_plan(apm::DJFormatArgs* f, hipStream_t s);
int apm_dj_write(apm::DJFormatArgs* f, hipStream_t s);
void apm_dj_rebuild(const apm::KeyState* old, uint32_t old_cap, apm::KeyState* fresh, uint32_t fresh_mask,
                    const apm::NeedEnt* arena, uint32_t arena_cap, double now, apm::JoinCounts* counts,
                    unsigned long long* live, uint8_t* pool, uint32_t* pool_ring, uint32_t pool_mask, hipStream_t s);
size_t apm_dj_rebuild_scratch_bytes(uint32_t cap);
std::vector<double> apm_dj_rebuild_selftest(uint32_t cap, double load, double dead, uint64_t seed, bool copy);
void apm_dj_rebuild_inplace(apm::KeyState* table, uint32_t cap, uint32_t* scratch, const apm::NeedEnt* arena,
                            uint32_t arena_cap, double now, apm::JoinCounts* counts, unsigned long long* live,
                            uint8_t* pool, uint32_t* pool_ring, uint32_t pool_mask, hipStream_t s);
size_t apm_dj_live_tmp_bytes(uint32_t cap);
void apm_dj_live_compact(const apm::KeyState* table, uint32_t cap, apm::KeyState* out, uint32_t* d_n, void* tmp,
                         size_t tmp_bytes, hipStream_t s);
void apm_dj_gather_blocks(const uint8_t* pool, const int32_t* idx, uint32_t n, uint8_t* out, hipStream_t s);
void apm_dj_pool_init(uint32_t* ring, uint32_t n, apm::JoinCounts* counts, hipStream_t s);
void apm_dj_pool_grow(const uint32_t* old_ring, uint32_t old_mask, uint32_t* fresh_ring, uint32_t old_n, uint32_t new_n,
                      apm::JoinCounts* counts, hipStream_t s);
void apm_dj_arena_grow(const apm::NeedEnt* old, uint32_t old_cap, apm::NeedEnt* fresh, uint32_t fresh_cap, uint64_t lo,
                       uint64_t hi, apm::KeyState* table, uint32_t table_cap, hipStream_t s);
int apm_dj_gather_plan(const int64_t* gid, int64_t n_upper, const int64_t* d_n, uint32_t* lens, uint32_t* offs,
                       void* tmp, size_t tmp_bytes, hipStream_t s);
int apm_dj_txcopy_plan(const int64_t* gid, int64_t n_upper, const int64_t* d_n, const char* ring, uint64_t ring_cap,
                       uint32_t* lens, uint32_t* offs, uint32_t* fb_count, void* tmp, size_t tmp_bytes, hipStream_t s);
void apm_dj_txcopy_write(const int64_t* gid, int64_t n, const char* ring, uint64_t ring_cap, const uint32_t* offs,
                         char* out, hipStream_t s);
void apm_dj_gather_copy(const int64_t* gid, int64_t n, const char* ring, uint64_t ring_cap, const uint32_t* offs,
                        char* out, uint64_t total_bytes, hipStream_t s);
void apm_dj_rebase_gids(const int64_t* gid, int64_t n, const uint32_t* offs, uint64_t base, int64_t* out,
                        hipStream_t s);
void apm_dj_min_pos(const int64_t* gid, int64_t n, unsigned long long* out, hipStream_t s);
void apm_dj_reg_fill(apm::RegSlot* reg, const int32_t* pairs, uint32_t n, hipStream_t s);
void apm_dj_scatter_i32(int32_t* dst, const int32_t* pairs, uint32_t n, hipStream_t s);
void apm_dj_fill_series(apm::TxRec* tx, const int32_t* raw, uint32_t n, const int32_t* raw_series,
                        unsigned long long* unmapped, hipStream_t s);
void apm_dj_gather_u8(const uint8_t* src, const int32_t* idx, uint32_t n, uint8_t* out, hipStream_t s);
void apm_dj_cache_stats(const apm::KeyState* table, uint32_t cap, double now, unsigned long long* out, hipStream_t s);
void apm_dj_keys_sync(const apm::KeyState* table, uint32_t cap, uint64_t* keys, hipStream_t s);
void apm_dj_count_le(const int64_t* end, int64_t n, int64_t edge, int64_t* out, hipStream_t s);
void apm_dj_relocate(int64_t* gid, int64_t n, char* ring, uint64_t ring_cap, uint64_t below, uint64_t dst_base,
                     unsigned long long* cursor, hipStream_t s);
}
```

### apmbackend_amd/csrc/kernels/devscan.h

```cpp
#pragma once
#include <rocprim/rocprim.hpp>

#include "common.h"

namespace apm {

constexpr int DS_BLOCK = 256, DS_ITEMS = 16, DS_TILE = DS_BLOCK * DS_ITEMS;
constexpr int DS_TILES_BLOCK = 1024, DS_TILES_ITEMS = 4, DS_MAX_TILES = DS_TILES_BLOCK * DS_TILES_ITEMS;

__device__ __forceinline__ uint32_t ds_count(const uint32_t* d_n, uint32_t cap) {
  const uint32_t n = *d_n;
  return n < cap ? n : cap;
}

template <class T, class F>
__global__ __launch_bounds__(DS_BLOCK) void k_ds_reduce(F f, const uint32_t* __restrict__ d_n, uint32_t cap,
                                                        T* __restrict__ tile_sum) {
  const uint32_t n = ds_count(d_n, cap);
  const uint32_t t0 = blockIdx.x * (uint32_t)DS_TILE;
  if (t0 >= n) return;
  T acc = 0;
#pragma unroll
  for (int k = 0; k < DS_ITEMS; ++k) {
    const uint32_t i = t0 + (uint32_t)k * DS_BLOCK + threadIdx.x;
    if (i < n) acc += f(i);
  }
  typedef rocprim::block_reduce<T, DS_BLOCK> R;
  __shared__ typename R::storage_type st;
  T s;
  R().reduce(acc, s, st);
  if (threadIdx.x == 0) tile_sum[blockIdx.x] = s;
}

template <class T>
__global__ __launch_bounds__(DS_TILES_BLOCK) void k_ds_tiles(T* __restrict__ tile_sum, const uint32_t* __restrict__ d_n,
                                                             uint32_t cap, T* __restrict__ total) {
  const uint32_t n = ds_count(d_n, cap);
  const uint32_t nt = (n + DS_TILE - 1) / DS_TILE;
  T v[DS_TILES_ITEMS];
#pragma unroll
  for (int k = 0; k < DS_TILES_ITEMS; ++k) {
    const uint32_t j = threadIdx.x * DS_TILES_ITEMS + k;
    v[k] = j < nt ? tile_sum[j] : T(0);
  }
  typedef rocprim::block_scan<T, DS_TILES_BLOCK> S;
  __shared__ typename S::storage_type st;
  T lane = 0;
#pragma unroll
  for (int k = 0; k < DS_TILES_ITEMS; ++k) lane += v[k];
  T excl, sum;
  S().exclusive_scan(lane, excl, T(0), sum, st);
#pragma unroll
  for (int k = 0; k < DS_TILES_ITEMS; ++k) {
    const uint32_t j = threadIdx.x * DS_TILES_ITEMS + k;
    if (j < nt) tile_sum[j] = excl;
    excl += v[k];
  }
  if (threadIdx.x == 0) *total = sum;
}

template <class T, class F, class G>
__global__ __launch_bounds__(DS_BLOCK) void k_ds_apply(F f, G g, const uint32_t* __restrict__ d_n, uint32_t cap,
                                                       const T* __restrict__ tile_off) {
  const uint32_t n = ds_count(d_n, cap);
  const uint32_t t0 = blockIdx.x * (uint32_t)DS_TILE;
  if (t0 >= n) return;
  const uint32_t i0 = t0 + threadIdx.x * (uint32_t)DS_ITEMS;
  T v[DS_ITEMS];
  T lane = 0;
#pragma unroll
  for (int k = 0; k < DS_ITEMS; ++k) {
    v[k] = i0 + k < n ? f(i0 + k) : T(0);
    lane += v[k];
  }
  typedef rocprim::block_scan<T, DS_BLOCK> S;
  __shared__ typename S::storage_type st;
  T excl;
  S().exclusive_scan(lane, excl, T(0), st);
  T p = tile_off[blockIdx.x] + excl;
#pragma unroll
  for (int k = 0; k < DS_ITEMS; ++k) {
    if (i0 + k < n) g(i0 + k, p);
    p += v[k];
  }
}

template <class T, class F, class G>
int ds_scan_apply(F f, G g, const uint32_t* d_n, uint32_t cap, T* tile_sum, T* total, hipStream_t s) {
  const uint32_t tiles = (cap + DS_TILE - 1) / DS_TILE;
  if (tiles > (uint32_t)DS_MAX_TILES) return -1;
  if (tiles == 0) return 0;
  hipLaunchKernelGGL((k_ds_reduce<T, F>), dim3(tiles), dim3(DS_BLOCK), 0, s, f, d_n, cap, tile_sum);
  hipLaunchKernelGGL((k_ds_tiles<T>), dim3(1), dim3(DS_TILES_BLOCK), 0, s, tile_sum, d_n, cap, total);
  hipLaunchKernelGGL((k_ds_apply<T, F, G>), dim3(tiles), dim3(DS_BLOCK), 0, s, f, g, d_n, cap, (const T*)tile_sum);
  return 0;
}

}
```

### apmbackend_amd/csrc/runtime/devjoin.cpp

```cpp
#include "devjoin.h"

#include <algorithm>
#include <chrono>
#include <climits>
#include <cstddef>
#include <cstdlib>
#include <cstring>
#include <stdexcept>

#include "../kernels/common.h"
#include "binio.h"
#include "d2h.h"
#include "../kernels/devjoin_dev.h"
#include "../kernels/kernel_api.h"
#include "join_util.h"
#include "jsutil.h"

namespace apm {

using namespace jstr;

namespace {
double clock_ms() {
  return std::chrono::duration<double, std::milli>(std::chrono::steady_clock::now().time_since_epoch()).count();
}

JOp blank_op(const Event& e, int32_t server) {
  JOp op;
  std::memset(&op, 0, sizeof(op));
  op.ts = op.num = op.aux = op.aux2 = js::nan();
  op.line = e.line;
  op.server = server;
  op.op = JOP_NONE;
  return op;
}

uint64_t pow2_at_least(uint64_t v) {
  uint64_t p = 1;
  while (p < v) p <<= 1;
  return p;
}
}

DeviceJoin::DeviceJoin(const DevJoinConfig& cfg, Dictionary* dict, const std::vector<FileInfo>* files,
                       const std::vector<std::string>* servers)
    : cfg_(cfg), dict_(dict), files_(files), servers_(servers) {
  cfg_.ring_bytes = pow2_at_least(std::max<uint64_t>(cfg_.ring_bytes, 1ull << 24));
  cfg_.arena_cap = (uint32_t)pow2_at_least(std::max<uint32_t>(cfg_.arena_cap, 1024));
  HIP_OK(hipSetDevice(cfg_.device));
  {
    int lo = 0, hi = 0;
    HIP_OK(hipDeviceGetStreamPriorityRange(&lo, &hi));
    const char* pe = std::getenv("APM_JOIN_PRIO");
    HIP_OK(hipStreamCreateWithPriority(&stream_, hipStreamNonBlocking, pe && pe[0] == '0' ? lo : hi));
    res_.adopt(stream_);
  }
  const uint32_t E = std::max<uint32_t>(cfg_.max_events, 1024);
  out_cap_ = 2 * E + (1u << 16);
  for (int k = 0; k < 2; ++k) {
    Slot& s = sl_[k];
    s.d_bytes = (uint8_t*)res_.dmalloc_on(stream_, cfg_.max_batch_bytes + 256);
    s.d_events = (Event*)res_.dmalloc_on(stream_, (size_t)E * sizeof(Event));
    s.host_flag = (uint8_t*)res_.dmalloc_on(stream_, E + 64);
    s.d_mh_idx = (uint32_t*)res_.dmalloc_on(stream_, (size_t)E * 4);
    s.d_walk_idx = (uint32_t*)res_.dmalloc_on(stream_, (size_t)E * 4);
    s.d_aud = (AudF*)res_.dmalloc_on(stream_, (size_t)E * sizeof(AudF));
    s.d_n_host = (SelCount*)res_.dmalloc_on(stream_, 64);
    res_.pin(s.h_host_ev, (size_t)E * sizeof(Event));
    res_.pin(s.h_host_idx, (size_t)E * 4);
    res_.pin(s.h_n_host, 64);
    std::memset(s.h_n_host.h, 0, 64);
    s.d_chunk_next = (int32_t*)res_.dmalloc_on(stream_, ((size_t)cfg_.max_chunks + 2) * 4);
    s.d_chunk_first = (uint8_t*)res_.dmalloc_on(stream_, (size_t)cfg_.max_chunks + 2);
    res_.pin(s.h_chunk_next, ((size_t)cfg_.max_chunks + 2) * 4);
    res_.pin(s.h_chunk_first, (size_t)cfg_.max_chunks + 2);
    s.d_tx = (TxRec*)res_.dmalloc_on(stream_, (size_t)out_cap_ * sizeof(TxRec));
    s.d_tx_raw = (int32_t*)res_.dmalloc_on(stream_, (size_t)out_cap_ * 4);
    s.d_tx_gid = (int64_t*)res_.dmalloc_on(stream_, (size_t)out_cap_ * 8);
    s.free_ev = res_.new_event();
  }
  table_cap_ = 1u << cfg_.table_bits;
  init_table_cap_ = table_cap_;
  init_arena_cap_ = cfg_.arena_cap;
  d_table_ = (KeyState*)res_.dmalloc_on(stream_, (size_t)table_cap_ * sizeof(KeyState));
  d_reg_ = (RegSlot*)res_.dmalloc_on(stream_, ((size_t)1 << cfg_.reg_bits) * sizeof(RegSlot));
  miss_cap_ = E;
  d_miss_ = (RegMiss*)res_.dmalloc_on(stream_, (size_t)miss_cap_ * sizeof(RegMiss));
  res_.pin(h_miss_, (size_t)miss_cap_ * sizeof(RegMiss));
  d_arena_ = (NeedEnt*)res_.dmalloc_on(stream_, (size_t)cfg_.arena_cap * sizeof(NeedEnt));
  d_exp_lo_ = (uint64_t*)res_.dmalloc_on(stream_, 8 * 4096);
  d_exp_hi_ = (uint64_t*)res_.dmalloc_on(stream_, 8 * 4096);
  res_.pin(h_exp_, 2 * 8 * 4096);
  soap_cap_ = 1u << 16;
  d_soap_ = (SoapState*)res_.dmalloc_on(stream_, (size_t)soap_cap_ * sizeof(SoapState));
  if (E >= (1u << 21)) throw std::runtime_error("device join: gpu.maxLinesPerBatch must be below 2^21");
  d_sel_val_ = (uint64_t*)res_.dmalloc_on(stream_, ((size_t)E + 64) * 8);
  d_sel_pos_ = (uint64_t*)res_.dmalloc_on(stream_, ((size_t)E + 64) * 8);
  d_walk_lo_ = (uint32_t*)res_.dmalloc_on(stream_, ((size_t)cfg_.max_chunks + 2) * 4);
  d_file_first_ = (int32_t*)res_.dmalloc_on(stream_, (size_t)soap_cap_ * 4);
  for (AudGen& g : aud_gen_) {
    g.carry = (AudCarry*)res_.dmalloc_on(stream_, (size_t)soap_cap_ * sizeof(AudCarry));
    aud_reserve(g, 4096, 16384, 1u << 20);
  }
  d_file_server_ = (int32_t*)res_.dmalloc_on(stream_, (size_t)soap_cap_ * 4);
  d_file_skey_ = (uint64_t*)res_.dmalloc_on(stream_, (size_t)soap_cap_ * 8);
  d_file_fkey_ = (uint64_t*)res_.dmalloc_on(stream_, (size_t)soap_cap_ * 8);
  h_file_skey_.reserve(soap_cap_);
  h_file_fkey_.reserve(soap_cap_);
  d_rawtab_ = (RawSvc*)res_.dmalloc_on(stream_, (size_t)cfg_.max_raw * sizeof(RawSvc));
  d_raw_series_ = (int32_t*)res_.dmalloc_on(stream_, (size_t)cfg_.max_raw * 4);
  d_raw_first_ = (int32_t*)res_.dmalloc_on(stream_, (size_t)cfg_.max_raw * 4);
  HIP_OK(hipMemsetAsync(d_raw_series_, 0xff, (size_t)cfg_.max_raw * 4, stream_));
  HIP_OK(hipMemsetAsync(d_raw_first_, 0x7f, (size_t)cfg_.max_raw * 4, stream_));
  raw_info_.reserve(cfg_.max_raw);
  res_.pin(h_rawtab_, (size_t)cfg_.max_raw * sizeof(RawSvc));
  d_reg_fill_ = (int32_t*)res_.dmalloc_on(stream_, (size_t)E * 8);
  res_.pin(h_reg_fill_, (size_t)E * 8);
  d_out_ = (TxDev*)res_.dmalloc_on(stream_, (size_t)out_cap_ * sizeof(TxDev));
  d_lens_ = (uint32_t*)res_.dmalloc_on(stream_, ((size_t)out_cap_ + 1) * 16);
  d_offs_ = (uint32_t*)res_.dmalloc_on(stream_, ((size_t)out_cap_ + 1) * 16);
  d_bucket_ = (int64_t*)res_.dmalloc_on(stream_, (size_t)out_cap_ * 8);
  d_bmax_ = (int64_t*)res_.dmalloc_on(stream_, (size_t)out_cap_ * 8);
  d_cand_ = (uint32_t*)res_.dmalloc_on(stream_, (size_t)out_cap_ * 4);
  d_cand_bucket_ = (int64_t*)res_.dmalloc_on(stream_, (size_t)out_cap_ * 8);
  d_unres_ = (uint32_t*)res_.dmalloc_on(stream_, (size_t)out_cap_ * 8);
  res_.pin(h_cand_, (size_t)out_cap_ * 4);
  res_.pin(h_cand_bucket_, (size_t)out_cap_ * 8);
  res_.pin(h_unres_, (size_t)out_cap_ * 8);
  ensure_tmp();
  sel_tmp_bytes_ = apm_dj_tmp_bytes(E, 1024);
  d_sel_tmp_ = res_.dmalloc_on(stream_, sel_tmp_bytes_);
  d_counts_ = (JoinCounts*)res_.dmalloc_on(stream_, sizeof(JoinCounts));
  res_.pin(h_counts_, sizeof(JoinCounts));
  std::memset(h_counts_, 0, sizeof(JoinCounts));
  d_live_ = (unsigned long long*)res_.dmalloc_on(stream_, 64);
  res_.pin(h_live_, 64);
  pool_n_ = (uint32_t)pow2_at_least(cfg_.pool_blocks ? std::max<uint32_t>(cfg_.pool_blocks, 1024)
                                                   : std::max<uint32_t>(E / 2, 1u << 16));
  d_pool_ = (uint8_t*)res_.dmalloc_on(stream_, (size_t)pool_n_ * CHAIN_BLK);
  d_pool_ring_ = (uint32_t*)res_.dmalloc_on(stream_, (size_t)pool_n_ * 4);
  apm_dj_pool_init(d_pool_ring_, pool_n_, d_counts_, stream_);
  h_counts_->pool_tail = h_counts_->pool_ptail = pool_n_;
  d_ops_ = (JOp*)res_.dmalloc_on(stream_, (size_t)E * sizeof(JOp));
  d_soap_code_ = (uint8_t*)res_.dmalloc_on(stream_, E);
  d_soap_num_ = (double*)res_.dmalloc_on(stream_, (size_t)E * 8);
  d_soap_hash_ = (uint64_t*)res_.dmalloc_on(stream_, (size_t)E * 8);
  d_chunk_ev_lo_ = (uint32_t*)res_.dmalloc_on(stream_, ((size_t)cfg_.max_chunks + 2) * 4);
  d_seg_f_ = (uint32_t*)res_.dmalloc_on(stream_, ((size_t)cfg_.max_chunks + 2) * SOAP_SEGS * 4);
  d_seg_in_ = (uint32_t*)res_.dmalloc_on(stream_, ((size_t)cfg_.max_chunks + 2) * SOAP_SEGS * 4);
  d_chain_hash_ = (uint64_t*)res_.dmalloc_on(stream_, ((size_t)cfg_.max_chunks + 2) * 8);
  d_op_slot_ = (uint32_t*)res_.dmalloc_on(stream_, ((size_t)E + 1) * 4);
  d_op_slot_sorted_ = (uint32_t*)res_.dmalloc_on(stream_, ((size_t)E + 1) * 4);
  d_op_idx_ = (uint32_t*)res_.dmalloc_on(stream_, ((size_t)E + 1) * 4);
  d_op_idx_sorted_ = (uint32_t*)res_.dmalloc_on(stream_, ((size_t)E + 1) * 4);
  exp_cap_ = cfg_.arena_cap;
  d_exp_key_ = (uint64_t*)res_.dmalloc_on(stream_, ((size_t)exp_cap_ + 1) * 8);
  d_exp_key_sorted_ = (uint64_t*)res_.dmalloc_on(stream_, ((size_t)exp_cap_ + 1) * 8);
  d_exp_idx_ = (uint32_t*)res_.dmalloc_on(stream_, ((size_t)exp_cap_ + 1) * 4);
  d_exp_idx_sorted_ = (uint32_t*)res_.dmalloc_on(stream_, ((size_t)exp_cap_ + 1) * 4);
  d_exp_cnt_ = (uint32_t*)res_.dmalloc_on(stream_, ((size_t)exp_cap_ + 1) * 4);
  d_exp_pos_ = (uint32_t*)res_.dmalloc_on(stream_, ((size_t)exp_cap_ + 1) * 4);
  d_out_cnt_ = (uint32_t*)res_.dmalloc_on(stream_, ((size_t)E + 1) * 4);
  d_out_pos_ = (uint32_t*)res_.dmalloc_on(stream_, ((size_t)E + 1) * 4);
  d_stage_ = (TxDev*)res_.dmalloc_on(stream_, (size_t)E * 2 * sizeof(TxDev));
  d_ovf_ = (DJOverflow*)res_.dmalloc_on(stream_, (size_t)DJ_OVF_CAP * sizeof(DJOverflow));
  d_ring_ = (char*)res_.dmalloc_on(stream_, cfg_.ring_bytes);
  d_ring_pos_ = (uint64_t*)res_.dmalloc_on(stream_, 8);
  d_big_ = (uint32_t*)res_.dmalloc_on(stream_, 8);
  HIP_OK(hipStreamSynchronize(stream_));
}

void DeviceJoin::ensure_txt(size_t bytes) {
  if (bytes <= txt_cap_ && d_txt_tx_) return;
  const size_t cap = std::max(bytes, txt_cap_);
  char* p = (char*)res_.dmalloc_raw(cap * 2);
  res_.dfree(d_txt_tx_);
  d_txt_tx_ = p;
  d_txt_db_ = p + cap;
  txt_cap_ = cap;
}

DeviceJoin::~DeviceJoin() {
  hipStreamSynchronize(stream_);
  res_.release_all();
}

void DeviceJoin::sync_file_keys() {
  const size_t n = files_->size();
  if (n <= h_file_fkey_.size()) return;
  if (n > soap_cap_) throw std::runtime_error("device join: too many files");
  const size_t lo = h_file_fkey_.size();
  if (lo == 0) HIP_OK(hipStreamSynchronize(stream_));
  for (size_t i = lo; i < n; ++i) {
    const FileInfo& f = (*files_)[i];
    const std::string& srv = (*servers_)[f.server];
    h_file_skey_.push_back(dj::server_key_of(srv.data(), srv.size()));
    h_file_fkey_.push_back(dj::file_key_of(f.path.data(), f.path.size()));
  }
  HIP_OK(hipMemcpy(d_file_skey_ + lo, h_file_skey_.data() + lo, (n - lo) * 8, hipMemcpyHostToDevice));
  HIP_OK(hipMemcpy(d_file_fkey_ + lo, h_file_fkey_.data() + lo, (n - lo) * 8, hipMemcpyHostToDevice));
}

void DeviceJoin::select_host(int k, const uint32_t* d_n_ev, uint32_t max_ev, hipStream_t ps) {
  Slot& s = sl_[k];
  sync_file_keys();
  DJArgs a{};
  a.ev = s.d_events;
  a.bytes = s.d_bytes;
  a.host_flag = s.host_flag;
  a.chunk_file = s.d_chunk_file;
  a.file_fkey = d_file_fkey_;
  a.aud = s.d_aud;
  a.sel_val = d_sel_val_;
  a.sel_pos = d_sel_pos_;
  a.host_ev = s.h_host_ev.d;
  a.host_ev_idx = s.h_host_idx.d;
  a.mh_idx = s.d_mh_idx;
  a.walk_idx = s.d_walk_idx;
  a.n_host = s.d_n_host;
  a.tmp = d_sel_tmp_;
  a.tmp_bytes = sel_tmp_bytes_;
  if (apm_dj_select_host(&a, d_n_ev, std::min<uint32_t>(max_ev, cfg_.max_events), ps) != 0)
    throw std::runtime_error("device join: scan scratch too small");
}

void DeviceJoin::export_select(int k, CopySegs& cs) {
  Slot& s = sl_[k];
  cs.add(s.h_n_host.d, s.d_n_host, sizeof(SelCount));
}

void DeviceJoin::chunk_upload(int k, uint32_t max_ev, CopySegs& cs) {
  Slot& s = sl_[k];
  cs.add(s.d_chunk_next, s.h_chunk_next.d, (size_t)s.n_chunks * 4);
  cs.add(s.d_chunk_first, s.h_chunk_first.d, s.n_chunks);
  max_ev = std::min<uint32_t>(max_ev, cfg_.max_events);
  cs.zero(s.d_n_host, sizeof(SelCount));
  if (max_ev) cs.zero(dj_select_list_n(d_sel_pos_, max_ev), 8);
}

void DeviceJoin::set_chunks(int k, const std::vector<int32_t>& chunk_file, const uint32_t* d_chunk_file,
                            const uint8_t* d_chunk_kind) {
  Slot& s = sl_[k];
  const uint32_t n = (uint32_t)chunk_file.size();
  std::unordered_map<int32_t, int32_t> last;
  for (uint32_t c = 0; c < n; ++c) {
    s.h_chunk_next[c] = -1;
    auto it = last.find(chunk_file[c]);
    if (it == last.end()) {
      s.h_chunk_first[c] = 1;
    } else {
      s.h_chunk_first[c] = 0;
      s.h_chunk_next[it->second] = (int32_t)c;
    }
    last[chunk_file[c]] = (int32_t)c;
  }
  s.d_chunk_file = d_chunk_file;
  s.d_chunk_kind = d_chunk_kind;
  s.n_chunks = n;
  s.chunk_file = chunk_file;
}

void DeviceJoin::host_prepass(int k, const uint8_t* hb, uint32_t n_host, const ParallelFor& parallel,
                              std::vector<HostOp>& hops_out, std::string& hbuf_out) {
  Slot& s = sl_[k];
  hops_out.clear();
  hbuf_out.clear();
  std::unordered_map<int32_t, int> task_of;
  int nt = 0;
  int32_t last_file = -1;
  int last_t = -1;
  for (uint32_t i = 0; i < n_host; ++i) {
    const int32_t file = s.chunk_file[s.h_host_ev[i].chunk];
    if (file == last_file) {
      tasks_[last_t].idx.push_back(i);
      continue;
    }
    auto it = task_of.find(file);
    int t;
    if (it == task_of.end()) {
      t = nt++;
      task_of.emplace(file, t);
      if ((int)tasks_.size() < nt) tasks_.emplace_back();
      PrepassTask& T = tasks_[t];
      T.file = file;
      T.idx.clear(); T.hops.clear(); T.hbuf.clear();
      T.audit_errors = T.invalid_acct = T.pm_host = 0;
    } else {
      t = it->second;
    }
    last_file = file;
    last_t = t;
    tasks_[t].idx.push_back(i);
  }
  auto work = [&](int t) {
    PrepassTask& T = tasks_[t];
    for (uint32_t i : T.idx) host_event(T, s.h_host_ev[i], s.h_host_idx[i], hb);
  };
  if (parallel && nt > 1) parallel(nt, work);
  else for (int t = 0; t < nt; ++t) work(t);
  size_t total = 0;
  std::vector<uint32_t> base(nt);
  for (int t = 0; t < nt; ++t) {
    base[t] = (uint32_t)hbuf_out.size();
    hbuf_out += tasks_[t].hbuf;
    total += tasks_[t].hops.size();
    audit_errors_ += tasks_[t].audit_errors;
    host_invalid_acct_ += tasks_[t].invalid_acct;
    host_pm_ += tasks_[t].pm_host;
  }
  hops_out.reserve(total);
  std::vector<size_t> pos(nt, 0);
  for (;;) {
    int best = -1;
    uint32_t bev = UINT32_MAX;
// ... 242 lines not shown
    r.srv_len = (int32_t)(*servers_)[m.server].size();
    r.norm_off = intern_name(norm);
    r.norm_len = (int32_t)norm.size();
    r.toplevel = norm.size() >= 2 && norm[0] == 'S' && norm[1] == ':';
    r.pad = 0;
    h_reg_fill_[2 * i] = m.slot;
    h_reg_fill_[2 * i + 1] = n;
    ++n;
  }
  if (names_.size() > names_cap_) {
    const size_t cap = std::max<size_t>(names_.size() * 2, 1 << 20);
    char* p = (char*)res_.dmalloc_raw(cap);
    if (d_names_) {
      HIP_OK(hipMemcpyAsync(p, d_names_, names_uploaded_, hipMemcpyDeviceToDevice, s));
      HIP_OK(hipStreamSynchronize(s));
      res_.dfree(d_names_);
    }
    d_names_ = p;
    names_cap_ = cap;
  }
  if (names_.size() > names_uploaded_) {
    HIP_OK(hipMemcpyAsync(d_names_ + names_uploaded_, names_.data() + names_uploaded_, names_.size() - names_uploaded_,
                          hipMemcpyHostToDevice, s));
    HIP_OK(hipStreamSynchronize(s));
    names_uploaded_ = names_.size();
  }
  HIP_OK(hipMemcpyAsync(d_rawtab_ + first, h_rawtab_ + first, (size_t)(n - first) * sizeof(RawSvc), hipMemcpyHostToDevice, s));
  HIP_OK(hipMemcpyAsync(d_reg_fill_, h_reg_fill_, (size_t)n_miss * 8, hipMemcpyHostToDevice, s));
  apm_dj_reg_fill(d_reg_, d_reg_fill_, n_miss, s);
  n_raw_.store(n, std::memory_order_release);
}

uint64_t DeviceJoin::ring_reserve(uint64_t bytes) {
  std::lock_guard<std::mutex> g(ring_mu_);
  const uint64_t cap = cfg_.ring_bytes;
  if (bytes > cap / 4) throw std::runtime_error("device join: one batch of tx text exceeds a quarter of gpu.txTextRingMB");
  uint64_t base = ring_head_.load(std::memory_order_relaxed);
  if ((base & (cap - 1)) + bytes > cap) base = (base + cap - 1) & ~(cap - 1);
  const uint64_t low = ring_low_.load(std::memory_order_acquire);
  if (base + bytes > low + cap)
    throw std::runtime_error("device join: tx text ring exhausted (pending released-tx lines span more than "
                             "gpu.txTextRingMB; raise it)");
  ring_head_.store(base + bytes, std::memory_order_release);
  return base;
}

void DeviceJoin::set_ring_low(uint64_t low) {
  uint64_t cur = ring_low_.load(std::memory_order_relaxed);
  while (low > cur && !ring_low_.compare_exchange_weak(cur, low)) {
  }
}

void DeviceJoin::release_slot(int k, hipStream_t stats_stream) {
  HIP_OK(hipEventRecord(sl_[k].free_ev, stats_stream));
  sl_[k].used = true;
}

void DeviceJoin::ensure_tmp() {
  const uint32_t E = std::max<uint32_t>(cfg_.max_events, 1024);
  const size_t need = std::max(apm_dj_tmp_bytes(E, out_cap_), apm_dj_tmp_bytes(cfg_.arena_cap, out_cap_));
  if (need <= tmp_bytes_ && d_tmp_) return;
  if (d_tmp_) {
    HIP_OK(hipStreamSynchronize(stream_));
    res_.dfree(d_tmp_);
  }
  tmp_bytes_ = need;
  d_tmp_ = res_.dmalloc_on(stream_, tmp_bytes_);
}

void DeviceJoin::rebuild_table(double now, uint32_t new_cap) {
  hipStream_t st = stream_;
  if (new_cap == table_cap_) {
    rebuild_inplace(now);
    sync_keys();
    HIP_OK(hipMemcpyAsync(h_live_, d_live_, 8, hipMemcpyDeviceToHost, st));
    HIP_OK(hipStreamSynchronize(st));
    keys_live_ = *h_live_;
    keys_since_rebuild_ = 0;
    live_pending_ = false;
    ++table_rebuilds_;
    return;
  }
  KeyState* fresh = (KeyState*)res_.dmalloc_on(stream_, (size_t)new_cap * sizeof(KeyState));
  HIP_OK(hipMemsetAsync(fresh, 0, (size_t)new_cap * sizeof(KeyState), st));
  HIP_OK(hipMemsetAsync(d_live_, 0, 8, st));
  apm_dj_rebuild(d_table_, table_cap_, fresh, new_cap - 1, d_arena_, cfg_.arena_cap, now, d_counts_, d_live_, d_pool_,
                 d_pool_ring_, pool_n_ - 1, st);
  HIP_OK(hipMemcpyAsync(h_live_, d_live_, 8, hipMemcpyDeviceToHost, st));
  HIP_OK(hipStreamSynchronize(st));
  res_.dfree(d_table_);
  if (d_table_spare_) res_.dfree(d_table_spare_);
  d_table_spare_ = nullptr;
  ++table_grows_;
  d_table_ = fresh;
  table_cap_ = new_cap;
  keys_live_ = *h_live_;
  keys_since_rebuild_ = 0;
  live_pending_ = false;
  ++table_rebuilds_;
  sync_keys();
}

void DeviceJoin::sync_keys() {
  if (keys_cap_ != table_cap_) {
    if (d_keys_) {
      HIP_OK(hipStreamSynchronize(stream_));
      res_.dfree(d_keys_);
    }
    d_keys_ = (uint64_t*)res_.dmalloc_on(stream_, (size_t)table_cap_ * 8);
    keys_cap_ = table_cap_;
  }
  apm_dj_keys_sync(d_table_, table_cap_, d_keys_, stream_);
  keys_stale_ = false;
}

void DeviceJoin::rebuild_inplace(double now) {
  const size_t need = apm_dj_rebuild_scratch_bytes(table_cap_);
  if (need > rb_scratch_bytes_) {
    if (d_rb_scratch_) res_.dfree(d_rb_scratch_);
    d_rb_scratch_ = (uint32_t*)res_.dmalloc_on(stream_, need);
    rb_scratch_bytes_ = need;
  }
  HIP_OK(hipMemsetAsync(d_live_, 0, 8, stream_));
  apm_dj_rebuild_inplace(d_table_, table_cap_, d_rb_scratch_, d_arena_, cfg_.arena_cap, now, d_counts_, d_live_,
                         d_pool_, d_pool_ring_, pool_n_ - 1, stream_);
}

void DeviceJoin::rebuild_table_async(double now) {
  hipStream_t st = stream_;
  rebuild_inplace(now);
  sync_keys();
  HIP_OK(hipMemcpyAsync(h_live_, d_live_, 8, hipMemcpyDeviceToHost, st));
  if (!live_ev_) live_ev_ = res_.new_event();
  HIP_OK(hipEventRecord(live_ev_, st));
  keys_since_rebuild_ = 0;
  live_pending_ = true;
  ++table_rebuilds_;
}

void DeviceJoin::idle_upkeep(double now, uint32_t n_next) {
  if (live_pending_) return;
  if ((keys_live_ + keys_since_rebuild_ + n_next) * 2 > table_cap_ && table_rebuilds_ > 0 && async_rebuild_fits(n_next))
    rebuild_table_async(now);
}

void DeviceJoin::grow_arena(uint32_t new_cap, uint64_t lo) {
  hipStream_t st = stream_;
  NeedEnt* fresh = (NeedEnt*)res_.dmalloc_on(stream_, (size_t)new_cap * sizeof(NeedEnt));
  apm_dj_arena_grow(d_arena_, cfg_.arena_cap, fresh, new_cap, lo, arena_head_, d_table_, table_cap_, st);
  HIP_OK(hipStreamSynchronize(st));
  res_.dfree(d_arena_);
  d_arena_ = fresh;
  for (void* p : {(void*)d_exp_key_, (void*)d_exp_key_sorted_}) res_.dfree(p);
  for (void* p : {(void*)d_exp_idx_, (void*)d_exp_idx_sorted_, (void*)d_exp_cnt_, (void*)d_exp_pos_})
    res_.dfree(p);
  cfg_.arena_cap = new_cap;
  exp_cap_ = new_cap;
  d_exp_key_ = (uint64_t*)res_.dmalloc_on(stream_, ((size_t)exp_cap_ + 1) * 8);
  d_exp_key_sorted_ = (uint64_t*)res_.dmalloc_on(stream_, ((size_t)exp_cap_ + 1) * 8);
  d_exp_idx_ = (uint32_t*)res_.dmalloc_on(stream_, ((size_t)exp_cap_ + 1) * 4);
  d_exp_idx_sorted_ = (uint32_t*)res_.dmalloc_on(stream_, ((size_t)exp_cap_ + 1) * 4);
  d_exp_cnt_ = (uint32_t*)res_.dmalloc_on(stream_, ((size_t)exp_cap_ + 1) * 4);
  d_exp_pos_ = (uint32_t*)res_.dmalloc_on(stream_, ((size_t)exp_cap_ + 1) * 4);
  ensure_tmp();
  ++arena_grows_;
}

void DeviceJoin::aud_reserve(AudGen& g, uint32_t autr, uint32_t items, uint64_t txt) {
  if (txt >= (1ull << 31)) throw std::runtime_error("device join: audit carry text beyond 2 GB");
  const bool grow = autr > g.cap_autr || items > g.cap_items || txt > g.cap_txt;
  if (!grow) return;
  HIP_OK(hipStreamSynchronize(stream_));
  if (autr > g.cap_autr) {
    res_.dfree(g.autr);
    g.cap_autr = std::max<uint32_t>(autr * 2, 4096);
    g.autr = (AutrEnt*)res_.dmalloc_on(stream_, (size_t)g.cap_autr * sizeof(AutrEnt));
  }
  if (items > g.cap_items) {
    res_.dfree(g.items);
    g.cap_items = std::max<uint32_t>(items * 2, 16384);
    g.items = (AudItem*)res_.dmalloc_on(stream_, (size_t)g.cap_items * sizeof(AudItem));
  }
  if (txt > g.cap_txt) {
    res_.dfree(g.txt);
    g.cap_txt = (uint32_t)std::min<uint64_t>(std::max<uint64_t>(txt * 2, 1u << 20), (1ull << 32) - 1);
    g.txt = (char*)res_.dmalloc_on(stream_, g.cap_txt);
  }
}

uint64_t DeviceJoin::pool_avail(bool exact) {
  if (exact) {
    HIP_OK(hipMemcpyAsync(h_counts_, d_counts_, sizeof(JoinCounts), hipMemcpyDeviceToHost, stream_));
    HIP_OK(hipStreamSynchronize(stream_));
  }
  return h_counts_->pool_tail - h_counts_->pool_head;
}

void DeviceJoin::grow_pool(uint64_t need_free) {
  hipStream_t st = stream_;
  const uint64_t avail = pool_avail(true);
  uint64_t n = pool_n_;
  while (avail + (n - pool_n_) < need_free) n *= 2;
  if (n >= (1ull << 31)) throw std::runtime_error("device join: chain pool beyond 2^31 blocks");
  uint8_t* pool = (uint8_t*)res_.dmalloc_on(stream_, (size_t)n * CHAIN_BLK);
  uint32_t* ring = (uint32_t*)res_.dmalloc_on(stream_, (size_t)n * 4);
  HIP_OK(hipMemcpyAsync(pool, d_pool_, (size_t)pool_n_ * CHAIN_BLK, hipMemcpyDeviceToDevice, st));
  apm_dj_pool_grow(d_pool_ring_, pool_n_ - 1, ring, pool_n_, (uint32_t)n, d_counts_, st);
  HIP_OK(hipStreamSynchronize(st));
  res_.dfree(d_pool_);
  res_.dfree(d_pool_ring_);
  d_pool_ = pool;
  d_pool_ring_ = ring;
  pool_n_ = (uint32_t)n;
  pool_avail(true);
  ++pool_grows_;
}

void DeviceJoin::ensure_capacity(uint32_t n_ev, uint64_t bytes, double now) {
  if (live_pending_) {
    HIP_OK(hipEventSynchronize(live_ev_));
    keys_live_ = *h_live_;
    live_pending_ = false;
  }
  if ((keys_live_ + keys_since_rebuild_ + n_ev) * 2 > table_cap_) {
    if (table_rebuilds_ > 0 && async_rebuild_fits(n_ev)) {
      rebuild_table_async(now);
      return ensure_rest(n_ev, bytes);
    }
    rebuild_table(now, table_cap_);
    uint64_t cap = table_cap_;
    while ((keys_live_ + n_ev) * 2 > cap) cap *= 2;
    if (cap >= (1ull << 31)) throw std::runtime_error("device join: key table beyond 2^31 slots");
    if (cap != table_cap_) rebuild_table(now, (uint32_t)cap);
  }
  ensure_rest(n_ev, bytes);
}

void DeviceJoin::ensure_rest(uint32_t n_ev, uint64_t bytes) {
  {
    const uint64_t low = regions_.empty() ? arena_head_ : regions_.front().lo;
    const uint64_t used = arena_head_ - low;
    uint64_t cap = cfg_.arena_cap;
    while (cap - used < n_ev) cap *= 2;
    if (cap >= (1ull << 31)) throw std::runtime_error("device join: need arena beyond 2^31 entries");
    if (cap != cfg_.arena_cap) grow_arena((uint32_t)cap, low);
  }
  const uint64_t need = 2ull * n_ev + bytes / LBLK_N + 64;
  if (pool_avail(false) < need && pool_avail(true) < need) grow_pool(need);
}

void DeviceJoin::prepass_ahead(int k, const uint8_t* hb, const ParallelFor& parallel) {
  if (ahead_k_ >= 0) throw std::runtime_error("device join: a pre-pass is already ahead");
  host_prepass(k, hb, sl_[k].h_n_host.h->host, parallel, hops_ahead_, hbuf_ahead_);
  ahead_k_ = k;
}

void DeviceJoin::run(int k, const uint8_t* hb, uint32_t n_ev, uint64_t n_bytes, double now, uint64_t batch_no,
                     bool want_tx, bool want_db, DevJoinBatch& out, const ParallelFor& parallel,
                     const std::function<void()>* meanwhile) {
  Slot& s = sl_[k];
  hipStream_t st = stream_;
  if (n_ev > cfg_.max_events) throw std::runtime_error("device join: more events than maxLinesPerBatch");
  events_ += n_ev;
  phase_t[0] = clock_ms();
  if (ahead_k_ == k) {
    std::swap(hops_, hops_ahead_);
    std::swap(hbuf_, hbuf_ahead_);
    ahead_k_ = -1;
  } else {
    if (ahead_k_ >= 0) throw std::runtime_error("device join: pre-pass ahead for another slot");
    host_prepass(k, hb, s.h_n_host.h->host, parallel, hops_, hbuf_);
  }
  phase_t[1] = clock_ms();
  spans.clear();
  double sp = phase_t[1];
  auto span = [&](const char* name) { const double t = clock_ms(); spans.push_back({name, {sp, t}}); sp = t; };
  res_.reserve(h_hops_, hops_.size(), hops_.size() * 2 + 65536, true);
  res_.reserve(h_hbuf_, hbuf_.size(), hbuf_.size() * 2 + (4 << 20), true);
  span("u.hostgrow");
  if (hops_.size() > d_hops_cap_) {
    d_hops_cap_ = hops_.size() * 2 + 65536;
    d_hops_ = (HostOp*)res_.dmalloc_raw(d_hops_cap_ * sizeof(HostOp));
  }
  if (hbuf_.size() > d_hbuf_cap_) {
    d_hbuf_cap_ = hbuf_.size() * 2 + (4 << 20);
    d_hbuf_ = (uint8_t*)res_.dmalloc_raw(d_hbuf_cap_);
  }
  span("u.devgrow");
  if (!hops_.empty()) {
    std::memcpy(h_hops_, hops_.data(), hops_.size() * sizeof(HostOp));
    span("u.hops.memcpy");
    apm_copy(d_hops_, h_hops_.d, hops_.size() * sizeof(HostOp), st);
    span("u.hops.h2d");
  }
  if (!hbuf_.empty()) {
    std::memcpy(h_hbuf_, hbuf_.data(), hbuf_.size());
    span("u.hbuf.memcpy");
    apm_copy(d_hbuf_, h_hbuf_.d, hbuf_.size(), st);
    span("u.hbuf.h2d");
  }
  sync_file_keys();
  if (files_->size() > files_uploaded_) {
    if (files_->size() > soap_cap_) throw std::runtime_error("device join: too many files");
    std::vector<int32_t> fs(files_->size() - files_uploaded_);
    for (size_t i = files_uploaded_; i < files_->size(); ++i) fs[i - files_uploaded_] = (*files_)[i].server;
    HIP_OK(hipMemcpyAsync(d_file_server_ + files_uploaded_, fs.data(), fs.size() * 4, hipMemcpyHostToDevice, st));
    HIP_OK(hipStreamSynchronize(st));
    files_uploaded_ = files_->size();
  }
  ensure_capacity(n_ev, n_bytes + hbuf_.size(), now);
  span("u.capacity");
  const uint64_t arena_low = regions_.empty() ? arena_head_ : regions_.front().lo;
  const uint32_t arena_limit = (uint32_t)((uint64_t)cfg_.arena_cap - (arena_head_ - arena_low));
  uint32_t n_reg = 0, n_exp = 0;
  while (!regions_.empty() && regions_.front().exp < now && n_reg < 4096) {
    h_exp_[n_reg] = regions_.front().lo;
    h_exp_[4096 + n_reg] = regions_.front().hi;
    n_exp += (uint32_t)(regions_.front().hi - regions_.front().lo);
    regions_.pop_front();
    ++n_reg;
  }
  if (n_reg) {
    apm_copy(d_exp_lo_, h_exp_.d, (size_t)n_reg * 8, st);
    apm_copy(d_exp_hi_, (const uint64_t*)h_exp_.d + 4096, (size_t)n_reg * 8, st);
  }
  span("u.files+exp");
  DJArgs& a = a_;
  a = DJArgs{};
  a.ev = s.d_events; a.n_ev = n_ev; a.bytes = s.d_bytes;
  a.chunk_file = s.d_chunk_file; a.chunk_kind = s.d_chunk_kind; a.n_chunks = s.n_chunks;
  a.chunk_next = s.d_chunk_next; a.chunk_first = s.d_chunk_first; a.file_server = d_file_server_;
  a.file_skey = d_file_skey_; a.file_fkey = d_file_fkey_;
  a.hops = d_hops_; a.n_hops = (uint32_t)hops_.size(); a.hbuf = d_hbuf_;
  a.now = now; a.batch_no = batch_no;
  a.rec_ttl = cfg_.record_ttl_ms; a.acct_ttl = cfg_.acct_ttl_ms; a.need_ttl = cfg_.need_ttl_ms;
  a.host_flag = s.host_flag;
  a.ops = d_ops_; a.soap_code = d_soap_code_; a.soap_num = d_soap_num_; a.soap_hash = d_soap_hash_;
  a.chunk_ev_lo = d_chunk_ev_lo_; a.seg_f = d_seg_f_; a.seg_in = d_seg_in_; a.chain_hash = d_chain_hash_;
  a.soap_state = d_soap_;
  a.op_slot = d_op_slot_; a.op_slot_sorted = d_op_slot_sorted_; a.op_idx = d_op_idx_; a.op_idx_sorted = d_op_idx_sorted_;
  a.tmp = d_tmp_; a.tmp_bytes = tmp_bytes_;
  if (heads_cap_ != table_cap_) {
    if (d_slot_head_) { HIP_OK(hipStreamSynchronize(st)); res_.dfree(d_slot_head_); }
    d_slot_head_ = (uint32_t*)res_.dmalloc_on(stream_, (size_t)table_cap_ * 4);
    HIP_OK(hipMemsetAsync(d_slot_head_, 0xff, (size_t)table_cap_ * 4, st));
    heads_cap_ = table_cap_;
  }
  a.slot_head = d_slot_head_; a.big = d_big_;
  if (keys_stale_ || keys_cap_ != table_cap_) sync_keys();
  a.table = d_table_; a.keys = d_keys_; a.table_mask = table_cap_ - 1;
  a.pool = d_pool_; a.pool_ring = d_pool_ring_; a.pool_mask = pool_n_ - 1;
  a.reg = d_reg_; a.reg_mask = (1u << cfg_.reg_bits) - 1; a.miss = d_miss_; a.miss_cap = miss_cap_;
  a.arena = d_arena_; a.arena_cap = cfg_.arena_cap; a.arena_base = arena_head_; a.arena_limit = arena_limit;
  a.exp_lo = d_exp_lo_; a.exp_hi = d_exp_hi_; a.n_exp_regions = n_reg; a.n_exp_entries = n_exp;
  a.exp_key = d_exp_key_; a.exp_key_sorted = d_exp_key_sorted_; a.exp_idx = d_exp_idx_;
  a.exp_idx_sorted = d_exp_idx_sorted_; a.exp_cnt = d_exp_cnt_; a.exp_pos = d_exp_pos_;
  a.out_cnt = d_out_cnt_; a.out_pos = d_out_pos_; a.stage = d_stage_; a.ovf = d_ovf_;
  a.out = d_out_; a.out_cap = out_cap_; a.counts = d_counts_;
  {
    const SelCount tot = *s.h_n_host;
    AudGen& gin = aud_gen_[aud_cur_];
    AudGen& gout = aud_gen_[aud_cur_ ^ 1];
    aud_reserve(gout, gin.n_autr + tot.mh, gin.n_items + tot.walk, (uint64_t)gin.n_txt + tot.aud_bytes);
    const uint32_t N = gin.n_autr + tot.mh;
    if (N + 1 > aud_key_cap_) {
      HIP_OK(hipStreamSynchronize(st));
      for (void* p : {(void*)d_aud_key_, (void*)d_aud_key_sorted_}) res_.dfree(p);
      for (void* p : {(void*)d_aud_ord_, (void*)d_aud_ord_sorted_}) res_.dfree(p);
      aud_key_cap_ = std::max<uint32_t>(2 * (N + 1), 1u << 14);
      d_aud_key_ = (uint64_t*)res_.dmalloc_on(stream_, (size_t)aud_key_cap_ * 8);
      d_aud_key_sorted_ = (uint64_t*)res_.dmalloc_on(stream_, (size_t)aud_key_cap_ * 8);
      d_aud_ord_ = (uint32_t*)res_.dmalloc_on(stream_, (size_t)aud_key_cap_ * 4);
      d_aud_ord_sorted_ = (uint32_t*)res_.dmalloc_on(stream_, (size_t)aud_key_cap_ * 4);
    }
    if (N > std::max<uint32_t>(cfg_.max_events, cfg_.arena_cap)) {
      const size_t need = apm_dj_tmp_bytes(N, out_cap_);
      if (need > tmp_bytes_) {
        HIP_OK(hipStreamSynchronize(st));
        res_.dfree(d_tmp_);
        tmp_bytes_ = need;
        d_tmp_ = res_.dmalloc_on(stream_, tmp_bytes_);
        a.tmp = d_tmp_; a.tmp_bytes = tmp_bytes_;
      }
    }
    const uint32_t slots = tot.walk + gin.n_items;
    if (slots > aud_slots_cap_) {
      HIP_OK(hipStreamSynchronize(st));
      res_.dfree(d_aud_slots_);
      aud_slots_cap_ = std::max<uint32_t>(2 * slots, 1u << 14);
      d_aud_slots_ = (AudItem*)res_.dmalloc_on(stream_, (size_t)aud_slots_cap_ * sizeof(AudItem));
    }
    a.n_mh = tot.mh; a.n_walk = tot.walk; a.n_files = (uint32_t)files_->size();
    a.aud = s.d_aud; a.gin = gin; a.gout = gout;
    a.mh_idx = s.d_mh_idx; a.walk_idx = s.d_walk_idx;
    a.aud_key = d_aud_key_; a.aud_key_sorted = d_aud_key_sorted_; a.aud_ord = d_aud_ord_; a.aud_ord_sorted = d_aud_ord_sorted_;
    a.walk_lo = d_walk_lo_; a.file_first_chunk = d_file_first_; a.aud_slots = d_aud_slots_;
  }
  if (s.used) HIP_OK(hipStreamWaitEvent(st, s.free_ev, 0));
  static const bool dbg = std::getenv("APM_DJ_DEBUG") != nullptr;
  if (dbg) {
    const hipError_t e = hipStreamSynchronize(st);
    if (e != hipSuccess) { fprintf(stderr, "[devjoin debug] before the join: %s\n", hipGetErrorString(e)); abort(); }
  }
  phase_t[2] = clock_ms();
  if (apm_dj_join(&a, st) != 0) throw std::runtime_error("device join: scan scratch too small");
  HIP_OK(hipMemcpyAsync(h_counts_, d_counts_, sizeof(JoinCounts), hipMemcpyDeviceToHost, st));
  if (meanwhile) (*meanwhile)();
  phase_t[3] = clock_ms();
  HIP_OK(hipStreamSynchronize(st));
  phase_t[4] = clock_ms();
  const JoinCounts c = *h_counts_;
  if (c.n_out > out_cap_) throw std::runtime_error("device join: more tx in one batch than the output capacity");
  if (c.aud_pad) throw std::runtime_error("device join: audit carry over capacity (sizing bug)");
  {
    AudGen& gout = aud_gen_[aud_cur_ ^ 1];
    gout.n_autr = c.aud_autr_n; gout.n_items = c.aud_items_n; gout.n_txt = c.aud_txt_n;
  }
  if (c.pad[0] > DJ_OVF_CAP) throw std::runtime_error("device join: output overflow list full");
  if (c.n_need_new) {
    const uint32_t cnt = std::min(c.n_need_new, arena_limit);
    regions_.push_back(Region{arena_head_, arena_head_ + cnt, now + cfg_.need_ttl_ms});
    arena_head_ += cnt;
  }
  keys_since_rebuild_ += c.n_keys_new;
  if (c.n_miss) register_misses(hb, c.n_miss, st);
  phase_t[5] = clock_ms();
  DJFormatArgs& f = f_;
  f = DJFormatArgs{};
  f.out = d_out_; f.n_out = c.n_out; f.reg = d_reg_; f.reg_mask = (1u << cfg_.reg_bits) - 1;
  f.raw = d_rawtab_; f.raw_series = d_raw_series_; f.raw_first = d_raw_first_; f.names = d_names_;
  f.bytes = s.d_bytes; f.hbuf = d_hbuf_; f.aud_txt = aud_gen_[aud_cur_].txt; f.arena = d_arena_; f.arena_cap = cfg_.arena_cap; f.pool = d_pool_;
  f.lens = d_lens_; f.offs = d_offs_; f.ring = d_ring_; f.ring_cap = cfg_.ring_bytes;
  f.tx = s.d_tx; f.tx_raw = s.d_tx_raw; f.tx_gid = s.d_tx_gid; f.tx_bucket = d_bucket_; f.tx_bmax = d_bmax_;
  f.cand = d_cand_; f.cand_bucket = d_cand_bucket_; f.unresolved = d_unres_;
  f.want_tx = want_tx; f.want_db = want_db; f.counts = d_counts_; f.tmp = d_tmp_; f.tmp_bytes = tmp_bytes_;
  const uint64_t ring_head = ring_head_.load(std::memory_order_acquire);
  f.ring_head = ring_head;
  f.ring_low = ring_low_.load(std::memory_order_acquire);
  f.ring_pos = d_ring_pos_;
  if (want_tx || want_db) ensure_txt(std::max<size_t>(txt_cap_, 4u << 20));
  f.txt_tx = d_txt_tx_;
  f.txt_db = d_txt_db_;
  f.txt_cap = txt_cap_;
  if (apm_dj_plan(&f, st) != 0) throw std::runtime_error("device join: scan scratch too small");
  phase_t[6] = clock_ms();
  const uint32_t spec = std::min<uint32_t>(c.n_out, std::max<uint32_t>(2 * last_cands_, 1024));
  const size_t spec_tx = want_tx ? std::min<size_t>(txt_cap_, 2 * (size_t)last_tx_bytes_ + 65536) : 0;
  const size_t spec_db = want_db ? std::min<size_t>(txt_cap_, 2 * (size_t)last_db_bytes_ + 65536) : 0;
  res_.reserve(h_txt_, spec_tx + spec_db, (spec_tx + spec_db) * 2 + (4 << 20));
  auto mapped = [](void* h) { return HipRes::device_alias(h); };
  auto write_and_copy = [&] {
    if (apm_dj_write(&f, st) != 0) throw std::runtime_error("device join: scan scratch too small");
    CopySegs cs;
    if (spec) {
      cs.add(mapped(h_cand_), d_cand_, (size_t)spec * 4);
      cs.add(mapped(h_cand_bucket_), d_cand_bucket_, (size_t)spec * 8);
      cs.add(mapped(h_unres_), d_unres_, (size_t)spec * 8);
    }
    if (spec_tx) cs.add(mapped(h_txt_), d_txt_tx_, spec_tx);
    if (spec_db) cs.add((char*)mapped(h_txt_) + spec_tx, d_txt_db_, spec_db);
    cs.add(mapped(h_counts_), d_counts_, sizeof(JoinCounts));
    apm_copy_segs(&cs, st);
    HIP_OK(hipStreamSynchronize(st));
  };
  write_and_copy();
  JoinCounts c3 = *h_counts_;
  if (c3.pad[1] == DJ_WRITE_TXT) {
    ensure_txt(std::max<size_t>(c3.tx_text_bytes, c3.db_text_bytes) * 2 + (16 << 20));
    f.txt_tx = d_txt_tx_;
    f.txt_db = d_txt_db_;
    f.txt_cap = txt_cap_;
    static_assert(DJ_WRITE_OK == 0, "the verdict is cleared by a zero fill");
    HIP_OK(hipMemsetAsync(&d_counts_->pad[1], 0, 4, st));
    ++write_regrows_;
    write_and_copy();
    c3 = *h_counts_;
  }
  if (c3.pad[1] == DJ_WRITE_TOO_BIG)
    throw std::runtime_error("device join: one batch of tx text exceeds a quarter of gpu.txTextRingMB");
  if (c3.pad[1] == DJ_WRITE_RING_FULL)
    throw std::runtime_error("device join: tx text ring exhausted (pending released-tx lines span more than "
                             "gpu.txTextRingMB; raise it)");
  if (c3.pad[1] != DJ_WRITE_OK) throw std::runtime_error("device join: write pass skipped");
  phase_t[7] = clock_ms();
  const uint64_t ring_base = ring_place(ring_head, c3.text_bytes, cfg_.ring_bytes);
  {
    std::lock_guard<std::mutex> g(ring_mu_);
    ring_head_.store(ring_base + c3.text_bytes, std::memory_order_release);
  }
  const uint32_t tx_bytes = want_tx ? c3.tx_text_bytes : 0, db_bytes = want_db ? c3.db_text_bytes : 0;
  if (c3.n_cand > spec || c3.n_unresolved > spec || tx_bytes > spec_tx || db_bytes > spec_db) {
    if (c3.n_cand > spec || c3.n_unresolved > spec) {
      HIP_OK(hipMemcpyAsync(h_cand_, d_cand_, (size_t)c3.n_cand * 4, hipMemcpyDeviceToHost, st));
      HIP_OK(hipMemcpyAsync(h_cand_bucket_, d_cand_bucket_, (size_t)c3.n_cand * 8, hipMemcpyDeviceToHost, st));
      HIP_OK(hipMemcpyAsync(h_unres_, d_unres_, (size_t)c3.n_unresolved * 8, hipMemcpyDeviceToHost, st));
    }
    if (tx_bytes > spec_tx || db_bytes > spec_db) {
      if ((size_t)tx_bytes + db_bytes > h_txt_.cap) {
        HIP_OK(hipStreamSynchronize(st));
        res_.reserve(h_txt_, (size_t)tx_bytes + db_bytes, ((size_t)tx_bytes + db_bytes) * 2 + (4 << 20));
      }
      if (tx_bytes) HIP_OK(hipMemcpyAsync(h_txt_, d_txt_tx_, tx_bytes, hipMemcpyDeviceToHost, st));
      if (db_bytes) HIP_OK(hipMemcpyAsync(h_txt_ + tx_bytes, d_txt_db_, db_bytes, hipMemcpyDeviceToHost, st));
    }
    HIP_OK(hipStreamSynchronize(st));
  }
  const char* h_tx_txt = h_txt_;
  const char* h_db_txt = h_txt_ + ((tx_bytes > spec_tx || db_bytes > spec_db) ? tx_bytes : spec_tx);
  last_tx_bytes_ = tx_bytes;
  last_db_bytes_ = db_bytes;
  last_cands_ = std::max(c3.n_cand, c3.n_unresolved);
  out.slot = k;
  out.n_out = c3.n_out;
  out.n_stats = c3.n_stats;
  out.n_db = c3.n_db;
  out.n_dropped = c3.n_dropped;
  out.ring_base = ring_base;
  out.d_tx = s.d_tx;
  out.d_raw = s.d_tx_raw;
  out.d_gid = s.d_tx_gid;
  out.cands.resize(c3.n_cand);
  out.max_bucket = INT64_MIN;
  for (uint32_t i = 0; i < c3.n_cand; ++i) {
    out.cands[i] = {h_cand_[i], h_cand_bucket_[i]};
    out.max_bucket = std::max(out.max_bucket, h_cand_bucket_[i]);
  }
  std::sort(out.cands.begin(), out.cands.end());
  out.unresolved.resize(c3.n_unresolved);
  for (uint32_t i = 0; i < c3.n_unresolved; ++i) out.unresolved[i] = {h_unres_[2 * i], (int32_t)h_unres_[2 * i + 1]};
  std::sort(out.unresolved.begin(), out.unresolved.end());
  out.text_tx.clear();
  out.text_db.clear();
  if (want_tx) out.text_tx.assign(h_tx_txt, tx_bytes);
  if (want_db) out.text_db.assign(h_db_txt, db_bytes);
  tx_ += c3.n_out;
  tx_db_ += c3.n_db;
  aud_cur_ ^= 1;
  idle_upkeep(now, n_ev);
  phase_t[8] = clock_ms();
  {
    double t[64];
    const char* nm[64];
    const int m = apm_dj_take_marks(t, nm, 64);
    double prev = phase_t[2];
    for (int i = 0; i < m; ++i) {
      spans.push_back({nm[i], {prev, t[i]}});
      prev = t[i];
    }
  }
}

size_t DeviceJoin::trim(double now) {
  hipStream_t st = stream_;
  HIP_OK(hipStreamSynchronize(st));
  if (live_pending_) {
    HIP_OK(hipEventSynchronize(live_ev_));
    keys_live_ = *h_live_;
    live_pending_ = false;
  }
  const size_t before = res_.device_bytes();
  const uint64_t tg = table_grows_, ag = arena_grows_;
  auto pow2_at_least = [](uint64_t v) { uint64_t p = 1; while (p < v) p <<= 1; return p; };
  if (table_cap_ > init_table_cap_) {
    rebuild_table(now, table_cap_);
    const uint64_t want = std::max<uint64_t>(init_table_cap_, pow2_at_least(std::max<uint64_t>(keys_live_ * 4, 8)));
    if (want < table_cap_) rebuild_table(now, (uint32_t)want);
  }
  if (d_table_spare_) {
    res_.dfree(d_table_spare_);
    d_table_spare_ = nullptr;
  }
  if (d_slot_head_) {
    res_.dfree(d_slot_head_);
    d_slot_head_ = nullptr;
    heads_cap_ = 0;
  }
  if (d_rb_scratch_) {
    res_.dfree(d_rb_scratch_);
    d_rb_scratch_ = nullptr;
    rb_scratch_bytes_ = 0;
  }
  {
    const uint64_t lo = regions_.empty() ? arena_head_ : regions_.front().lo;
    const uint64_t live = arena_head_ - lo;
    const uint64_t acap = std::max<uint64_t>(init_arena_cap_, pow2_at_least(std::max<uint64_t>(live * 4, 1024)));
    if (acap < cfg_.arena_cap) grow_arena((uint32_t)acap, lo);
// ... 142 lines not shown
      std::memcpy(iblk.data(), h.data() + n_live + 2 * n_ents, n_ents * 4);
      std::memcpy(lblk.data(), h.data() + n_live + 3 * n_ents, n_ents * 4);
    }
  }
  struct Blk { uint8_t b[CHAIN_BLK]; };
  std::vector<Blk> blocks;
  {
    std::vector<int32_t> cur;
    std::vector<size_t> slot_of;
    for (uint32_t i = 0; i < n_live; ++i) {
      const size_t o = live_off + (size_t)i * sizeof(KeyState) + offsetof(KeyState, pblk);
      if (const int32_t b = pblk[i]) { cur.push_back(b); slot_of.push_back(o); }
    }
    for (size_t i = 0; i < n_ents; ++i) {
      const size_t e = ents_off + i * sizeof(NeedEnt);
      const size_t oi = e + offsetof(NeedEnt, iblk), ol = e + offsetof(NeedEnt, lblk);
      if (!ekey[i]) { put32(oi, 0); put32(ol, 0); continue; }
      if (const int32_t b = iblk[i]) { cur.push_back(b); slot_of.push_back(oi); }
      if (const int32_t b = lblk[i]) { cur.push_back(b); slot_of.push_back(ol); }
    }
    std::vector<int32_t> parent(cur.size(), -1);
    int32_t* d_idx = nullptr;
    uint8_t* d_out = nullptr;
    size_t cap = 0;
    while (!cur.empty()) {
      if (cur.size() > cap) {
        if (d_idx) { res_.dfree(d_idx); res_.dfree(d_out); }
        cap = cur.size() * 2;
        d_idx = (int32_t*)res_.dmalloc_raw(cap * 4);
        d_out = (uint8_t*)res_.dmalloc_raw(cap * CHAIN_BLK);
      }
      HIP_OK(hipMemcpyAsync(d_idx, cur.data(), cur.size() * 4, hipMemcpyHostToDevice, st));
      apm_dj_gather_blocks(d_pool_, d_idx, (uint32_t)cur.size(), d_out, st);
      const size_t base = blocks.size();
      blocks.resize(base + cur.size());
      HIP_OK(hipMemcpyAsync(blocks.data() + base, d_out, cur.size() * CHAIN_BLK, hipMemcpyDeviceToHost, st));
      HIP_OK(hipStreamSynchronize(st));
      std::vector<int32_t> nxt, nparent;
      for (size_t i = 0; i < cur.size(); ++i) {
        const int32_t nb = (int32_t)(base + i + 1);
        if (parent[i] < 0) put32(slot_of[i], nb);
        else *(int32_t*)blocks[(size_t)parent[i]].b = nb;
        const int32_t next = *(const int32_t*)blocks[base + i].b;
        *(int32_t*)blocks[base + i].b = 0;
        if (next) { nxt.push_back(next); nparent.push_back((int32_t)(base + i)); }
      }
      cur.swap(nxt);
      parent.swap(nparent);
    }
    if (d_idx) { res_.dfree(d_idx); res_.dfree(d_out); }
  }
  span("ck.j.chains");
  w.vec(blocks);
}

void DeviceJoin::save(BinWriter& w) {
  hipStream_t st = stream_;
  save_spans.clear();
  double sp0 = clock_ms();
  auto span = [&](const char* name) { const double t = clock_ms(); save_spans.push_back({name, {sp0, t}}); sp0 = t; };
  HIP_OK(hipStreamSynchronize(st));
  HIP_OK(hipMemcpy(h_counts_, d_counts_, sizeof(JoinCounts), hipMemcpyDeviceToHost));
  w.pod(*h_counts_);
  for (uint64_t v : {events_, tx_, tx_db_, audit_errors_, host_pm_, host_invalid_acct_, host_events_}) w.pod(v);
  if (w.is_memory()) {
    save_tables(w);
  } else {
    BinWriter mw{BinWriter::Memory{}};
    CkDefer* const d = ck_defer();
    ck_defer() = nullptr;
    save_tables(mw);
    ck_defer() = d;
    const MemBlob b = mw.take_memory();
    w.raw(b.data(), b.size());
  }
  sp0 = clock_ms();
  {
    std::vector<SoapState> ss(files_->size());
    if (!ss.empty()) HIP_OK(hipMemcpy(ss.data(), d_soap_, ss.size() * sizeof(SoapState), hipMemcpyDeviceToHost));
    w.vec(ss);
  }
  {
    const int32_t n = n_raw();
    std::vector<RawInfo> ri(raw_info_.begin(), raw_info_.begin() + n);
    w.vec(ri);
    std::vector<int32_t> top(n);
    for (int32_t i = 0; i < n; ++i) top[i] = h_rawtab_[i].toplevel;
    w.vec(top);
  }
  span("ck.j.soap+registry");
  {
    const AudGen& g = aud_gen_[aud_cur_];
    const uint32_t nf = (uint32_t)files_->size();
    std::vector<AudCarry> carry(nf);
    std::vector<AutrEnt> autr(g.n_autr);
    std::vector<AudItem> items(g.n_items);
    std::string txt(g.n_txt, '\0');
    if (nf) HIP_OK(hipMemcpy(carry.data(), g.carry, (size_t)nf * sizeof(AudCarry), hipMemcpyDeviceToHost));
    if (g.n_autr) HIP_OK(hipMemcpy(autr.data(), g.autr, (size_t)g.n_autr * sizeof(AutrEnt), hipMemcpyDeviceToHost));
    if (g.n_items) HIP_OK(hipMemcpy(items.data(), g.items, (size_t)g.n_items * sizeof(AudItem), hipMemcpyDeviceToHost));
    if (g.n_txt) HIP_OK(hipMemcpy(&txt[0], g.txt, g.n_txt, hipMemcpyDeviceToHost));
    w.vec(carry);
    w.vec(autr);
    w.vec(items);
    w.str(txt);
  }
  span("ck.j.audit");
}

void DeviceJoin::load(BinReader& rd) {
  hipStream_t st = stream_;
  JoinCounts c;
  rd.pod(c);
  HIP_OK(hipMemcpy(d_counts_, &c, sizeof(JoinCounts), hipMemcpyHostToDevice));
  *h_counts_ = c;
  for (uint64_t* v : {&events_, &tx_, &tx_db_, &audit_errors_, &host_pm_, &host_invalid_acct_, &host_events_}) rd.pod(*v);
  {
    auto live = rd.vec<KeyState>();
    uint64_t cap = table_cap_;
    while (live.size() * 2 > cap) cap *= 2;
    HIP_OK(hipStreamSynchronize(st));
    if (cap != table_cap_) {
      res_.dfree(d_table_);
      if (d_table_spare_) res_.dfree(d_table_spare_);
      d_table_spare_ = nullptr;
      table_cap_ = (uint32_t)cap;
      d_table_ = (KeyState*)res_.dmalloc_on(stream_, (size_t)table_cap_ * sizeof(KeyState));
      ensure_tmp();
    } else {
      HIP_OK(hipMemsetAsync(d_table_, 0, (size_t)table_cap_ * sizeof(KeyState), st));
    }
    if (!live.empty()) {
      KeyState* tmp = (KeyState*)res_.dmalloc_raw(live.size() * sizeof(KeyState));
      HIP_OK(hipMemcpy(tmp, live.data(), live.size() * sizeof(KeyState), hipMemcpyHostToDevice));
      HIP_OK(hipMemsetAsync(d_live_, 0, 8, st));
      apm_dj_rebuild(tmp, (uint32_t)live.size(), d_table_, table_cap_ - 1, d_arena_, cfg_.arena_cap, -__builtin_inf(),
                     d_counts_, d_live_, d_pool_, d_pool_ring_, pool_n_ - 1, st);
      HIP_OK(hipStreamSynchronize(st));
      res_.dfree(tmp);
    }
    keys_live_ = live.size();
    keys_since_rebuild_ = 0;
    live_pending_ = false;
    sync_keys();
  }
  {
    const uint32_t saved_cap = rd.pod<uint32_t>();
    if (saved_cap != cfg_.arena_cap) {
      HIP_OK(hipStreamSynchronize(st));
      res_.dfree(d_arena_);
      cfg_.arena_cap = saved_cap;
      d_arena_ = (NeedEnt*)res_.dmalloc_on(stream_, (size_t)cfg_.arena_cap * sizeof(NeedEnt));
      for (void* p : {(void*)d_exp_key_, (void*)d_exp_key_sorted_}) res_.dfree(p);
      for (void* p : {(void*)d_exp_idx_, (void*)d_exp_idx_sorted_, (void*)d_exp_cnt_, (void*)d_exp_pos_})
        res_.dfree(p);
      exp_cap_ = saved_cap;
      d_exp_key_ = (uint64_t*)res_.dmalloc_on(stream_, ((size_t)exp_cap_ + 1) * 8);
      d_exp_key_sorted_ = (uint64_t*)res_.dmalloc_on(stream_, ((size_t)exp_cap_ + 1) * 8);
      d_exp_idx_ = (uint32_t*)res_.dmalloc_on(stream_, ((size_t)exp_cap_ + 1) * 4);
      d_exp_idx_sorted_ = (uint32_t*)res_.dmalloc_on(stream_, ((size_t)exp_cap_ + 1) * 4);
      d_exp_cnt_ = (uint32_t*)res_.dmalloc_on(stream_, ((size_t)exp_cap_ + 1) * 4);
      d_exp_pos_ = (uint32_t*)res_.dmalloc_on(stream_, ((size_t)exp_cap_ + 1) * 4);
      ensure_tmp();
    }
  }
  rd.pod(arena_head_);
  regions_.clear();
  for (uint64_t n = rd.pod<uint64_t>(); n; --n) {
    Region r;
    rd.pod(r.lo); rd.pod(r.hi); rd.pod(r.exp);
    regions_.push_back(r);
  }
  {
    auto ents = rd.vec<NeedEnt>();
    const uint64_t lo = regions_.empty() ? arena_head_ : regions_.front().lo;
    if (ents.size() != arena_head_ - lo) throw std::runtime_error("checkpoint: need arena size mismatch");
    const uint64_t cap = cfg_.arena_cap;
    if (ents.size() > cap) throw std::runtime_error("checkpoint: need arena larger than the ring");
    HIP_OK(hipStreamSynchronize(st));
    if (!ents.empty()) {
      const uint64_t first = lo & (cap - 1);
      const uint64_t n1 = std::min<uint64_t>(ents.size(), cap - first);
      HIP_OK(hipMemcpy(d_arena_ + first, ents.data(), n1 * sizeof(NeedEnt), hipMemcpyHostToDevice));
      if (ents.size() > n1)
        HIP_OK(hipMemcpy(d_arena_, ents.data() + n1, (ents.size() - n1) * sizeof(NeedEnt), hipMemcpyHostToDevice));
    }
  }
  {
    struct Blk { uint8_t b[CHAIN_BLK]; };
    auto blocks = rd.vec<Blk>();
    HIP_OK(hipStreamSynchronize(st));
    uint64_t n = pool_n_;
    while (n < 2 * blocks.size() + (1u << 16)) n *= 2;
    if (n != pool_n_) {
      res_.dfree(d_pool_);
      res_.dfree(d_pool_ring_);
      pool_n_ = (uint32_t)n;
      d_pool_ = (uint8_t*)res_.dmalloc_on(stream_, (size_t)pool_n_ * CHAIN_BLK);
      d_pool_ring_ = (uint32_t*)res_.dmalloc_on(stream_, (size_t)pool_n_ * 4);
      HIP_OK(hipStreamSynchronize(st));
    }
    if (!blocks.empty())
      HIP_OK(hipMemcpy(d_pool_, blocks.data(), blocks.size() * CHAIN_BLK, hipMemcpyHostToDevice));
    apm_dj_pool_init(d_pool_ring_, pool_n_, d_counts_, st);
    const unsigned long long taken = blocks.size();
    HIP_OK(hipMemcpyAsync((uint8_t*)d_counts_ + offsetof(JoinCounts, pool_head), &taken, 8, hipMemcpyHostToDevice, st));
    HIP_OK(hipStreamSynchronize(st));
    pool_avail(true);
  }
  {
    auto ss = rd.vec<SoapState>();
    if (ss.size() > soap_cap_) throw std::runtime_error("checkpoint: too many files");
    if (!ss.empty()) HIP_OK(hipMemcpy(d_soap_, ss.data(), ss.size() * sizeof(SoapState), hipMemcpyHostToDevice));
  }
  {
    auto ri = rd.vec<RawInfo>();
    auto top = rd.vec<int32_t>();
    if (ri.size() > cfg_.max_raw) throw std::runtime_error("checkpoint: more raw services than gpu.maxRawServices");
    const uint32_t rmask = (1u << cfg_.reg_bits) - 1;
    std::vector<RegSlot> reg((size_t)rmask + 1);
    for (auto& r : reg) { r.key = 0; r.raw = RAW_EMPTY; r.pad = 0; }
    raw_info_.clear();
    for (size_t i = 0; i < ri.size(); ++i) {
      raw_info_.push_back(ri[i]);
      RawSvc& r = h_rawtab_[i];
      const std::string& srv = (*servers_)[ri[i].server];
      const std::string norm = dict_->service_name(ri[i].norm_id);
      r.srv_off = intern_name(srv);
      r.srv_len = (int32_t)srv.size();
      r.norm_off = intern_name(norm);
      r.norm_len = (int32_t)norm.size();
      r.toplevel = top[i];
      r.pad = 0;
      const uint64_t k = dj::regkey_of(ri[i].svc, ri[i].server);
      for (uint32_t h = dj::home_of(k, rmask);; h = (h + 1) & rmask)
        if (!reg[h].key) { reg[h].key = k; reg[h].raw = (int32_t)i; break; }
    }
    HIP_OK(hipMemcpy(d_reg_, reg.data(), reg.size() * sizeof(RegSlot), hipMemcpyHostToDevice));
    if (!ri.empty()) HIP_OK(hipMemcpy(d_rawtab_, h_rawtab_, ri.size() * sizeof(RawSvc), hipMemcpyHostToDevice));
    if (names_.size() > names_cap_) {
      names_cap_ = std::max<size_t>(names_.size() * 2, 1 << 20);
      d_names_ = (char*)res_.dmalloc_raw(names_cap_);
    }
    if (!names_.empty()) HIP_OK(hipMemcpy(d_names_, names_.data(), names_.size(), hipMemcpyHostToDevice));
    names_uploaded_ = names_.size();
    n_raw_.store((int32_t)ri.size(), std::memory_order_release);
  }
  {
    auto carry = rd.vec<AudCarry>();
    auto autr = rd.vec<AutrEnt>();
    auto items = rd.vec<AudItem>();
    const std::string txt = rd.str();
    if (carry.size() > soap_cap_) throw std::runtime_error("checkpoint: too many files");
    HIP_OK(hipStreamSynchronize(st));
    aud_cur_ = 0;
    AudGen& g = aud_gen_[0];
    aud_reserve(g, (uint32_t)autr.size(), (uint32_t)items.size(), txt.size());
    HIP_OK(hipStreamSynchronize(st));
    HIP_OK(hipMemset(g.carry, 0, (size_t)soap_cap_ * sizeof(AudCarry)));
    HIP_OK(hipMemset(aud_gen_[1].carry, 0, (size_t)soap_cap_ * sizeof(AudCarry)));
    if (!carry.empty()) HIP_OK(hipMemcpy(g.carry, carry.data(), carry.size() * sizeof(AudCarry), hipMemcpyHostToDevice));
    if (!autr.empty()) HIP_OK(hipMemcpy(g.autr, autr.data(), autr.size() * sizeof(AutrEnt), hipMemcpyHostToDevice));
    if (!items.empty()) HIP_OK(hipMemcpy(g.items, items.data(), items.size() * sizeof(AudItem), hipMemcpyHostToDevice));
    if (!txt.empty()) HIP_OK(hipMemcpy(g.txt, txt.data(), txt.size(), hipMemcpyHostToDevice));
    g.n_autr = (uint32_t)autr.size();
    g.n_items = (uint32_t)items.size();
    g.n_txt = (uint32_t)txt.size();
  }
  files_uploaded_ = 0;
  HIP_OK(hipStreamSynchronize(st));
}

void DeviceJoin::reset_ring(uint64_t head) {
  std::lock_guard<std::mutex> g(ring_mu_);
  ring_head_.store(head, std::memory_order_release);
  ring_low_.store(0, std::memory_order_release);
}

}
```

### apmbackend_amd/csrc/runtime/devjoin.h

```cpp
#pragma once
#include <hip/hip_runtime.h>

#include <atomic>
#include <cstdint>
#include <deque>
#include <functional>
#include <mutex>
#include <string>
#include <unordered_map>
#include <vector>

#include "../apm_types.h"
#include "../kernels/devjoin_api.h"
#include "hipres.h"
#include "join.h"

namespace apm {

struct CopySegs;

struct DevJoinConfig {
  uint32_t max_events = 1u << 20;
  uint64_t max_batch_bytes = 64ull << 20;
  uint32_t max_chunks = 4096;
// ... 84 lines not shown
    uint8_t* host_flag = nullptr;
    uint32_t* d_mh_idx = nullptr;
    uint32_t* d_walk_idx = nullptr;
    AudF* d_aud = nullptr;
    SelCount* d_n_host = nullptr;
    Mapped<Event> h_host_ev;
    Mapped<uint32_t> h_host_idx;
    Mapped<SelCount> h_n_host;
    int32_t* d_chunk_next = nullptr;
    uint8_t* d_chunk_first = nullptr;
    Mapped<int32_t> h_chunk_next;
    Mapped<uint8_t> h_chunk_first;
    const uint32_t* d_chunk_file = nullptr;
    const uint8_t* d_chunk_kind = nullptr;
    uint32_t n_chunks = 0;
    std::vector<int32_t> chunk_file;
    TxRec* d_tx = nullptr;
    int32_t* d_tx_raw = nullptr;
    int64_t* d_tx_gid = nullptr;
    hipEvent_t free_ev = nullptr;
    bool used = false;
  } sl_[2];

  struct RawInfo { int32_t server; int32_t norm_id; uint64_t svc; };

  struct PrepassTask {
    int32_t file = -1;
    std::vector<uint32_t> idx;
    std::vector<HostOp> hops;
    std::string hbuf;
    uint64_t audit_errors = 0, invalid_acct = 0, pm_host = 0;
    uint32_t put(std::string_view s) { const uint32_t o = (uint32_t)hbuf.size(); hbuf.append(s.data(), s.size()); return o; }
  };
  void host_prepass(int k, const uint8_t* host_bytes, uint32_t n_host, const ParallelFor& parallel,
                    std::vector<HostOp>& hops, std::string& hbuf);
  void host_event(PrepassTask& t, const Event& e, uint32_t ev, const uint8_t* host_bytes);
  void on_app(PrepassTask& t, const Event& e, uint32_t ev, std::string_view line);
  void save_tables(class BinWriter& w);
  void aud_reserve(AudGen& g, uint32_t autr, uint32_t items, uint64_t txt);
  int32_t intern_name(const std::string& s);
  void register_misses(const uint8_t* host_bytes, uint32_t n_miss, hipStream_t s);
  void ensure_capacity(uint32_t n_ev, uint64_t bytes, double now);
  void rebuild_table(double now, uint32_t new_cap);
  void rebuild_table_async(double now);
  bool async_rebuild_fits(uint64_t n_ev) const {
    return (keys_live_ + keys_since_rebuild_ + n_ev) * 8 <= (uint64_t)table_cap_ * 5;
  }
  void ensure_rest(uint32_t n_ev, uint64_t bytes);
  void rebuild_inplace(double now);
  void idle_upkeep(double now, uint32_t n_next);
  void grow_arena(uint32_t new_cap, uint64_t lo);
  void grow_pool(uint64_t need_free);
  uint64_t pool_avail(bool exact);
  void ensure_tmp();

  DevJoinConfig cfg_;
  uint32_t init_table_cap_ = 0, init_arena_cap_ = 0;
  Dictionary* dict_;
  const std::vector<FileInfo>* files_;
  const std::vector<std::string>* servers_;
  hipStream_t stream_ = nullptr;
  HipRes res_;
  uint8_t* d_stage_bytes_ = nullptr;

  std::vector<HostOp> hops_;
  std::string hbuf_;
  std::vector<HostOp> hops_ahead_;
  std::string hbuf_ahead_;
  int ahead_k_ = -1;
  PinnedBuf<HostOp> h_hops_;
  PinnedBuf<uint8_t> h_hbuf_;
  HostOp* d_hops_ = nullptr;
  uint8_t* d_hbuf_ = nullptr;
  size_t d_hops_cap_ = 0, d_hbuf_cap_ = 0;
  std::vector<PrepassTask> tasks_;
  void* d_sel_tmp_ = nullptr;
  size_t sel_tmp_bytes_ = 0;
  uint64_t audit_errors_ = 0, host_pm_ = 0, host_invalid_acct_ = 0, host_events_ = 0, events_ = 0, tx_ = 0, tx_db_ = 0;

  DJArgs a_{};
  DJFormatArgs f_{};
  KeyState* d_table_ = nullptr;
  uint64_t* d_keys_ = nullptr;
  uint32_t keys_cap_ = 0;
  bool keys_stale_ = true;
  void sync_keys();
  unsigned long long* d_cstats_ = nullptr;
  unsigned long long* h_cstats_ = nullptr;
  unsigned long long cstats_last_[5] = {0, 0, 0, 0, 0};
  uint32_t cstats_cap_ = 0, cstats_last_cap_ = 0;
  hipEvent_t cstats_ev_ = nullptr;
  bool cstats_pending_ = false, cstats_have_ = false;
  KeyState* d_table_spare_ = nullptr;
  uint32_t table_cap_ = 0;
  uint64_t keys_since_rebuild_ = 0, keys_live_ = 0;
  bool live_pending_ = false;
  hipEvent_t live_ev_ = nullptr;
  uint32_t* d_rb_scratch_ = nullptr;
  size_t rb_scratch_bytes_ = 0;
  uint8_t* d_pool_ = nullptr;
  uint32_t* d_pool_ring_ = nullptr;
  uint32_t pool_n_ = 0;
  unsigned long long* h_live_ = nullptr;
  uint64_t table_grows_ = 0, arena_grows_ = 0, pool_grows_ = 0, table_rebuilds_ = 0, trims_ = 0;
  RegSlot* d_reg_ = nullptr;
  RegMiss* d_miss_ = nullptr;
  RegMiss* h_miss_ = nullptr;
  uint32_t miss_cap_ = 0;
  NeedEnt* d_arena_ = nullptr;
  uint64_t arena_head_ = 0;
  struct Region { uint64_t lo, hi; double exp; };
  std::deque<Region> regions_;
  uint64_t* d_exp_lo_ = nullptr;
  uint64_t* d_exp_hi_ = nullptr;
  Mapped<uint64_t> h_exp_;
  SoapState* d_soap_ = nullptr;
  AudGen aud_gen_[2]{};
  int aud_cur_ = 0;
  uint64_t* d_sel_val_ = nullptr;
  uint64_t* d_sel_pos_ = nullptr;
  uint64_t *d_aud_key_ = nullptr, *d_aud_key_sorted_ = nullptr;
  uint32_t *d_aud_ord_ = nullptr, *d_aud_ord_sorted_ = nullptr;
  uint32_t aud_key_cap_ = 0;
  uint32_t* d_walk_lo_ = nullptr;
  int32_t* d_file_first_ = nullptr;
  AudItem* d_aud_slots_ = nullptr;
  uint32_t aud_slots_cap_ = 0;
  static constexpr size_t kCkBounce = 32u << 20;
  char* h_ck_bounce_ = nullptr;
  uint32_t soap_cap_ = 0;
  int32_t* d_file_server_ = nullptr;
  uint64_t* d_file_skey_ = nullptr;
  uint64_t* d_file_fkey_ = nullptr;
  std::vector<uint64_t> h_file_skey_, h_file_fkey_;
  void sync_file_keys();
  size_t files_uploaded_ = 0;
  RawSvc* d_rawtab_ = nullptr;
  int32_t* d_raw_series_ = nullptr;
  int32_t* d_raw_first_ = nullptr;
  std::vector<RawInfo> raw_info_;
  std::atomic<int32_t> n_raw_{0};
  std::string names_;
  std::unordered_map<std::string, int32_t> name_off_;
  char* d_names_ = nullptr;
  size_t names_uploaded_ = 0, names_cap_ = 0;
  int32_t* d_reg_fill_ = nullptr;
  int32_t* h_reg_fill_ = nullptr;
  RawSvc* h_rawtab_ = nullptr;
  TxDev* d_out_ = nullptr;
  uint32_t out_cap_ = 0;
  uint32_t* d_lens_ = nullptr;
  uint32_t* d_offs_ = nullptr;
  int64_t* d_bucket_ = nullptr;
  int64_t* d_bmax_ = nullptr;
  uint32_t* d_cand_ = nullptr;
  int64_t* d_cand_bucket_ = nullptr;
  uint32_t* d_unres_ = nullptr;
  uint32_t* h_cand_ = nullptr;
  int64_t* h_cand_bucket_ = nullptr;
  uint32_t* h_unres_ = nullptr;
  char* d_txt_tx_ = nullptr;
  char* d_txt_db_ = nullptr;
  size_t txt_cap_ = 0;
  PinnedBuf<char> h_txt_;
  uint32_t last_tx_bytes_ = 0, last_db_bytes_ = 0, last_cands_ = 0;
  uint64_t* d_ring_pos_ = nullptr;
  uint32_t* d_slot_head_ = nullptr;
  uint32_t heads_cap_ = 0;
  uint32_t* d_big_ = nullptr;
  uint64_t write_regrows_ = 0;
  void ensure_txt(size_t bytes);
  void* d_tmp_ = nullptr;
  size_t tmp_bytes_ = 0;
  JoinCounts* d_counts_ = nullptr;
  JoinCounts* h_counts_ = nullptr;
  unsigned long long* d_live_ = nullptr;
  JOp* d_ops_ = nullptr;
  uint8_t* d_soap_code_ = nullptr;
  double* d_soap_num_ = nullptr;
  uint64_t* d_soap_hash_ = nullptr;
  uint32_t* d_chunk_ev_lo_ = nullptr;
  uint32_t* d_seg_f_ = nullptr;
  uint32_t* d_seg_in_ = nullptr;
  uint64_t* d_chain_hash_ = nullptr;
  uint32_t *d_op_slot_ = nullptr, *d_op_slot_sorted_ = nullptr, *d_op_idx_ = nullptr, *d_op_idx_sorted_ = nullptr;
  uint64_t *d_exp_key_ = nullptr, *d_exp_key_sorted_ = nullptr;
  uint32_t *d_exp_idx_ = nullptr, *d_exp_idx_sorted_ = nullptr, *d_exp_cnt_ = nullptr, *d_exp_pos_ = nullptr;
  uint32_t exp_cap_ = 0;
  uint32_t* d_out_cnt_ = nullptr;
  uint32_t* d_out_pos_ = nullptr;
  TxDev* d_stage_ = nullptr;
  DJOverflow* d_ovf_ = nullptr;
  char* d_ring_ = nullptr;
  std::mutex ring_mu_;
  std::atomic<uint64_t> ring_head_{0};
  std::atomic<uint64_t> ring_low_{0};
};

}
```

Baseline: 328.0 million.

## Fuse count/scan/emit stages into reduce-then-apply scans with totals hooks

Replaces several count kernel + rocprim scan + emit/place/totals kernel sequences (expiry emit, output placement, plan length scan, candidate bucket-max scan) with a generic two-pass reduce/apply scan that calls functors for per-element output and a total hook. The per-block reduce is folded into k_resolve_len for small plans, and pool_fix moves into the place kernels. This drops intermediate arrays (exp_cnt/exp_pos, bmax) and several kernel launches per batch, cutting launch overhead and global memory traffic. The cost is more templated code and a tile-count limit that falls back to a multi-item path or fails on very large inputs.

```diff
diff --git a/apmbackend_amd/csrc/kernels/devjoin.hip b/apmbackend_amd/csrc/kernels/devjoin.hip
--- a/apmbackend_amd/csrc/kernels/devjoin.hip
+++ b/apmbackend_amd/csrc/kernels/devjoin.hip
@@ -506,21 +506,22 @@
 struct SelScatterG {
   const Event* ev;
   const uint8_t* flag;
-  const uint64_t* total;
   Event* out;
   uint32_t *out_idx, *mh_idx, *walk_idx;
-  SelCount* totals;
   __device__ void operator()(uint32_t i, uint64_t pos) const {
-    if (i == 0) {
-      const SelCount t = sel_unpack(*total);
-      totals->host = t.host; totals->mh = t.mh; totals->walk = t.walk;
-    }
     const uint8_t fl = flag[i];
     if (!fl) return;
     const SelCount p = sel_unpack(pos);
     if (fl & SEL_HOST) { out[p.host] = ev[i]; out_idx[p.host] = i; }
     if (fl & SEL_MH) mh_idx[p.mh] = i;
     if (fl & SEL_WALK) walk_idx[p.walk] = i;
+  }
+};
+struct SelTotalH {
+  SelCount* totals;
+  __device__ void operator()(uint64_t total) const {
+    const SelCount t = sel_unpack(total);
+    totals->host = t.host; totals->mh = t.mh; totals->walk = t.walk;
   }
 };
 
@@ -1571,25 +1572,29 @@
   }
 }
 
-__global__ __launch_bounds__(TB) void k_exp_count(DJArgs a) {
-  const uint32_t e = blockIdx.x * blockDim.x + threadIdx.x;
-  if (e > a.n_exp_entries) return;
-  if (e == a.n_exp_entries) { a.exp_cnt[e] = 0; return; }
-  a.exp_cnt[e] = a.exp_key_sorted[e] == ~0ULL ? 0u : (uint32_t)a.arena[a.exp_idx_sorted[e]].n;
-}
-
-__global__ void k_exp_emit(DJArgs a) {
-  const uint32_t e = blockIdx.x * blockDim.x + threadIdx.x;
-  if (e == 0) {
-    a.counts->n_exp_out = a.n_exp_entries ? a.exp_pos[a.n_exp_entries] : 0;
-    atomicAdd(&a.counts->need_expired, (unsigned long long)a.counts->n_exp_out);
-  }
-  if (e >= a.n_exp_entries) return;
-  const uint32_t n = a.exp_cnt[e];
+__device__ __forceinline__ uint32_t exp_count(const DJArgs& a, uint32_t e) {
+  return a.exp_key_sorted[e] == ~0ULL ? 0u : (uint32_t)a.arena[a.exp_idx_sorted[e]].n;
+}
+struct ExpCountF {
+  DJArgs a;
+  __device__ uint32_t operator()(uint32_t e) const { return exp_count(a, e); }
+};
+struct ExpTotalH {
+  JoinCounts* counts;
+  __device__ void operator()(uint32_t total) const {
+    counts->n_exp_out = total;
+    atomicAdd(&counts->need_expired, (unsigned long long)total);
+  }
+};
+struct ExpEmitG {
+  DJArgs a;
+  __device__ void operator()(uint32_t e, uint32_t base) const;
+};
+__device__ void ExpEmitG::operator()(uint32_t e, uint32_t base) const {
+  const uint32_t n = exp_count(a, e);
   if (!n) return;
   const uint32_t idx = a.exp_idx_sorted[e];
   NeedEnt& ne = a.arena[idx];
-  const uint32_t base = a.exp_pos[e];
   int32_t b = 0;
   for (uint32_t k = 0; k < n && base + k < a.out_cap; ++k) {
     const NeedItem& r = need_item(a.pool, ne, (int)k, b);
@@ -1604,19 +1609,43 @@
   ne.key = 0;
 }
 
-__global__ __launch_bounds__(TB) void k_place(DJArgs a) {
-  const uint32_t i = blockIdx.x * blockDim.x + threadIdx.x;
-  const uint32_t base = a.counts->n_exp_out;
-  if (i == 0) a.counts->n_out = base + a.out_pos[a.n_ev];
-  if (i >= a.n_ev * 2) return;
-  const uint32_t ev = i >> 1, sub = i & 1;
-  if (sub >= a.out_cnt[ev]) return;
-  const uint32_t p = base + a.out_pos[ev] + sub;
-  if (p < a.out_cap) a.out[p] = a.stage[(size_t)ev * 2 + sub];
+struct PlaceCountF {
+  const uint32_t* out_cnt;
+  __device__ uint32_t operator()(uint32_t ev) const { return out_cnt[ev]; }
+};
+struct PlaceG {
+  DJArgs a;
+  __device__ void operator()(uint32_t ev, uint32_t pos) const {
+    a.out_pos[ev] = pos;
+    const uint32_t cnt = min(a.out_cnt[ev], 2u);
+    const uint32_t base = a.counts->n_exp_out + pos;
+    for (uint32_t sub = 0; sub < cnt; ++sub)
+      if (base + sub < a.out_cap) a.out[base + sub] = a.stage[(size_t)ev * 2 + sub];
+  }
+};
+struct PlaceTotalH {
+  DJArgs a;
+  __device__ void operator()(uint32_t total) const {
+    a.out_pos[a.n_ev] = total;
+    a.counts->n_out = a.counts->n_exp_out + total;
+  }
+};
+
+__device__ __forceinline__ void pool_fix(JoinCounts* c) {
+  const unsigned long long h = c->pool_head, t = c->pool_tail;
+  c->pool_head = h < t ? h : t;
+  c->pool_tail = c->pool_ptail;
+}
+
+__global__ void k_place_none(DJArgs a) {
+  a.out_pos[0] = 0;
+  a.counts->n_out = a.counts->n_exp_out;
+  pool_fix(a.counts);
 }
 
 __global__ __launch_bounds__(TB) void k_place_ovf(DJArgs a) {
   const uint32_t k = blockIdx.x * blockDim.x + threadIdx.x;
+  if (k == 0) pool_fix(a.counts);
   const uint32_t n = min(a.counts->pad[0], DJ_OVF_CAP);
   if (k >= n) return;
   const DJOverflow& o = a.ovf[k];
@@ -1652,25 +1681,51 @@
   return n + 1;
 }
 
-__global__ __launch_bounds__(TB) void k_resolve_len(DJFormatArgs f) {
+struct U4Sum {
+  __device__ U4 identity() const { return U4{0, 0, 0, 0}; }
+  __device__ U4 operator()(const U4& a, const U4& b) const { return U4Plus()(a, b); }
+};
+
+__global__ __launch_bounds__(TB) void k_resolve_len(DJFormatArgs f, U4* __restrict__ tile_sum) {
+  static_assert(TB == DS_BLOCK, "k_resolve_len's blocks are the plan scan's tiles");
   const uint32_t i = blockIdx.x * blockDim.x + threadIdx.x;
   const uint32_t n = f.n_out;
   U4* lens = reinterpret_cast<U4*>(f.lens);
-  if (i == n) { lens[n] = U4{0, 0, 0, 0}; return; }
-  if (i > n) return;
-  TxDev t = f.out[i];
-  const int32_t raw = reg_find(f.reg, f.reg_mask, regkey_of(t.svc, t.server));
-  t.raw = raw >= 0 ? raw : -1;
-  f.out[i].raw = t.raw;
-  const uint32_t len = line_len(f, t);
-  const bool st = stat_usable(t);
-  lens[i] = U4{len, st ? 1u : 0u, t.to_db ? 0u : len, t.to_db ? len : 0u};
-  if (t.to_db) atomicAdd(&f.counts->n_db, 1u);
-  else if (!st) atomicAdd(&f.counts->n_dropped, 1u);
-}
-
-__global__ void k_plan_totals(DJFormatArgs f) {
-  const U4 o = reinterpret_cast<const U4*>(f.offs)[f.n_out];
+  U4 l = U4{0, 0, 0, 0};
+  if (i < n) {
+    TxDev t = f.out[i];
+    const int32_t raw = reg_find(f.reg, f.reg_mask, regkey_of(t.svc, t.server));
+    t.raw = raw >= 0 ? raw : -1;
+    f.out[i].raw = t.raw;
+    const uint32_t len = line_len(f, t);
+    const bool st = stat_usable(t);
+    l = U4{len, st ? 1u : 0u, t.to_db ? 0u : len, t.to_db ? len : 0u};
+    if (t.to_db) atomicAdd(&f.counts->n_db, 1u);
+    else if (!st) atomicAdd(&f.counts->n_dropped, 1u);
+  }
+  if (i <= n) lens[i] = l;
+  if (!tile_sum) return;
+  typedef rocprim::block_reduce<U4, TB> R;
+  __shared__ typename R::storage_type st;
+  U4 sum;
+  R().reduce(l, sum, st, U4Plus());
+  if (threadIdx.x == 0) tile_sum[blockIdx.x] = sum;
+}
+
+struct PlanLenF {
+  const U4* lens;
+  __device__ U4 operator()(uint32_t i) const { return lens[i]; }
+};
+struct PlanOffsG {
+  U4* offs;
+  __device__ void operator()(uint32_t i, const U4& p) const { offs[i] = p; }
+};
+struct PlanTotalH {
+  DJFormatArgs f;
+  __device__ void operator()(const U4& o) const;
+};
+__device__ void PlanTotalH::operator()(const U4& o) const {
+  reinterpret_cast<U4*>(f.offs)[f.n_out] = o;
   f.counts->text_bytes = o.x;
   f.counts->n_stats = o.y;
   f.counts->tx_text_bytes = o.z;
@@ -1827,10 +1882,17 @@
   }
 }
 
-__global__ __launch_bounds__(TB) void k_cands(DJFormatArgs f) {
-  const uint32_t j = blockIdx.x * blockDim.x + threadIdx.x;
+struct BucketF {
+  const int64_t* bucket;
+  __device__ int64_t operator()(uint32_t j) const { return bucket[j]; }
+};
+struct CandG {
+  DJFormatArgs f;
+  __device__ void operator()(uint32_t j, int64_t bmax) const;
+};
+__device__ void CandG::operator()(uint32_t j, int64_t bmax) const {
   if (f.counts->pad[1] != DJ_WRITE_OK || j >= f.counts->n_stats) return;
-  if (j == 0 || f.tx_bmax[j] > f.tx_bmax[j - 1]) {
+  if (j == 0 || f.tx_bucket[j] > bmax) {
     const uint32_t k = atomicAdd(&f.counts->n_cand, 1u);
     f.cand[k] = j;
     f.cand_bucket[k] = f.tx_bucket[j];
@@ -2135,11 +2197,7 @@
   if (lane == 0) gid[w] = (int64_t)((np << 20) | (g & 0xfffffu));
 }
 
-__global__ void k_pool_fix(JoinCounts* c) {
-  const unsigned long long h = c->pool_head, t = c->pool_tail;
-  c->pool_head = h < t ? h : t;
-  c->pool_tail = c->pool_ptail;
-}
+__global__ void k_pool_fix(JoinCounts* c) { pool_fix(c); }
 
 __global__ void k_pool_init(uint32_t* ring, uint32_t n, JoinCounts* c) {
   const uint32_t i = blockIdx.x * blockDim.x + threadIdx.x;
@@ -2292,20 +2350,88 @@
 static int dj_scan_counts(PrimScratch& sc, const uint32_t* cnt, uint32_t* pos, size_t n, hipStream_t s) {
   return prim_exclusive_scan(sc, cnt, pos, 0u, n, rocprim::plus<uint32_t>(), s);
 }
-static int dj_scan_lens(PrimScratch& sc, const U4* lens, U4* offs, size_t n, hipStream_t s) {
-  return prim_exclusive_scan(sc, lens, offs, U4{0, 0, 0, 0}, n, U4Plus(), s);
-}
-static int dj_scan_bucket_max(PrimScratch& sc, const int64_t* bucket, int64_t* bmax, size_t n, hipStream_t s) {
-  return prim_inclusive_scan(sc, bucket, bmax, n, rocprim::maximum<int64_t>(), s);
+
+extern "C++" {
+static bool dj_scan_small(size_t n) { return ds_tiles<1>(n) - 1 <= (size_t)DS_MAX_TILES; }
+template <class T>
+static int dj_scan_tiles(PrimScratch& sc, size_t n, T** tile_sum) {
+  const size_t need = ds_tiles<1>(n) * sizeof(T);
+  sc.need = std::max(sc.need, need);
+  *tile_sum = nullptr;
+  if (sc.size_only) return 0;
+  if (need > sc.cap) return -1;
+  *tile_sum = static_cast<T*>(sc.tmp);
+  return 0;
+}
+template <class T, class Op, class F, class G, class H>
+static int dj_scan_apply(PrimScratch& sc, Op op, F f, G g, H h, size_t n, const char* const (&mark)[2],
+                         hipStream_t s) {
+  T* tile_sum;
+  if (dj_scan_tiles(sc, n, &tile_sum) != 0) return -1;
+  if (!tile_sum) return 0;
+  const uint32_t cap = (uint32_t)n;
+  if (dj_scan_small(n)) {
+    hipLaunchKernelGGL((k_ds_reduce<T, 1, Op, F>), dim3((uint32_t)ds_tiles<1>(n) - 1), dim3(DS_BLOCK), 0, s, op, f,
+                       nullptr, cap, tile_sum);
+    dj_check(s, mark[0]);
+    if (ds_apply_op<T, 1>(op, f, g, h, nullptr, cap, (const T*)tile_sum, (T*)nullptr, s) != 0) return -1;
+  } else {
+    if (ds_tiles<DS_ITEMS>(n) - 1 > (size_t)DS_MAX_TILES) return -1;
+    hipLaunchKernelGGL((k_ds_reduce<T, DS_ITEMS, Op, F>), dim3((uint32_t)ds_tiles<DS_ITEMS>(n) - 1), dim3(DS_BLOCK), 0,
+                       s, op, f, nullptr, cap, tile_sum);
+    dj_check(s, mark[0]);
+    if (ds_apply_op<T, DS_ITEMS>(op, f, g, h, nullptr, cap, (const T*)tile_sum, (T*)nullptr, s) != 0) return -1;
+  }
+  dj_check(s, mark[1]);
+  return 0;
+}
+
+static int dj_scan_expiry(PrimScratch& sc, const DJArgs* a, size_t n, hipStream_t s) {
+  static const char* const mark[2] = {"k_ds_reduce (expiry)", "k_ds_apply (expiry emit)"};
+  const DJArgs z = a ? *a : DJArgs{};
+  return dj_scan_apply<uint32_t>(sc, DsPlus<uint32_t>(), ExpCountF{z}, ExpEmitG{z}, ExpTotalH{z.counts}, n, mark, s);
+}
+static int dj_scan_place(PrimScratch& sc, const DJArgs* a, size_t n, hipStream_t s) {
+  static const char* const mark[2] = {"k_ds_reduce (place)", "k_ds_apply (place)"};
+  const DJArgs z = a ? *a : DJArgs{};
+  return dj_scan_apply<uint32_t>(sc, DsPlus<uint32_t>(), PlaceCountF{z.out_cnt}, PlaceG{z}, PlaceTotalH{z}, n, mark, s);
+}
+static int dj_scan_cands(PrimScratch& sc, const DJFormatArgs* f, size_t n, hipStream_t s) {
+  static const char* const mark[2] = {"k_ds_reduce (bucket max)", "k_ds_apply (cands)"};
+  const DJFormatArgs z = f ? *f : DJFormatArgs{};
+  return dj_scan_apply<int64_t>(sc, DsMax<int64_t>{INT64_MIN}, BucketF{z.tx_bucket}, CandG{z}, DsNoTotal(), n, mark, s);
+}
+static int dj_plan(PrimScratch& sc, const DJFormatArgs* f, size_t n, hipStream_t s) {
+  U4* tile_sum;
+  if (dj_scan_tiles(sc, n, &tile_sum) != 0) return -1;
+  if (!tile_sum) return 0;
+  const bool small = dj_scan_small(n);
+  hipLaunchKernelGGL(k_resolve_len, dim3(((uint32_t)n + 1 + TB - 1) / TB), dim3(TB), 0, s, *f,
+                     small ? tile_sum : (U4*)nullptr);
+  dj_check(s, "k_resolve_len");
+  const PlanLenF lf{reinterpret_cast<const U4*>(f->lens)};
+  const PlanOffsG og{reinterpret_cast<U4*>(f->offs)};
+  if (small) {
+    if (ds_apply_op<U4, 1>(U4Sum(), lf, og, PlanTotalH{*f}, nullptr, (uint32_t)n, (const U4*)tile_sum, (U4*)nullptr,
+                           s) != 0)
+      return -1;
+    dj_check(s, "k_ds_apply (plan)");
+    return 0;
+  }
+  static const char* const mark[2] = {"k_ds_reduce (plan)", "k_ds_apply (plan)"};
+  return dj_scan_apply<U4>(sc, U4Sum(), lf, og, PlanTotalH{*f}, n, mark, s);
+}
+
 }
 
 size_t apm_dj_tmp_bytes(uint32_t max_ev, uint32_t max_out) {
   PrimScratch q;
   const size_t n = std::max<size_t>(max_ev, 1) + 1;
   dj_sort_keys(q, nullptr, nullptr, nullptr, nullptr, n, 0);
-  dj_scan_counts(q, nullptr, nullptr, n, 0);
-  dj_scan_lens(q, nullptr, nullptr, (size_t)max_out + 1, 0);
-  dj_scan_bucket_max(q, nullptr, nullptr, (size_t)max_out + 1, 0);
+  dj_scan_expiry(q, nullptr, n, 0);
+  dj_scan_place(q, nullptr, n, 0);
+  dj_plan(q, nullptr, (size_t)max_out + 1, 0);
+  dj_scan_cands(q, nullptr, (size_t)max_out + 1, 0);
   return q.need + 4096;
 }
 
@@ -2322,9 +2448,8 @@
   dj_check(s, "k_host_flags_bytes");
   uint64_t* total = a->sel_pos + (max_ev + DS_TILE - 1) / DS_TILE + 1;
   if (ds_scan_apply<uint64_t>(SelValF{a->sel_val},
-                              SelScatterG{a->ev, a->host_flag, total, a->host_ev, a->host_ev_idx, a->mh_idx,
-                                          a->walk_idx, a->n_host},
-                              d_n_ev, max_ev, a->sel_pos, total, s) != 0)
+                              SelScatterG{a->ev, a->host_flag, a->host_ev, a->host_ev_idx, a->mh_idx, a->walk_idx},
+                              d_n_ev, max_ev, a->sel_pos, total, s, SelTotalH{a->n_host}) != 0)
     return -1;
   dj_check(s, "k_ds_scan (host selection)");
   return 0;
@@ -2389,45 +2514,26 @@
     dj_check(s, "k_exp_keys");
     if (dj_sort_keys(sc, a->exp_key, a->exp_key_sorted, a->exp_idx, a->exp_idx_sorted, E, s) != 0) return -1;
     dj_check(s, "rocprim_radix_sort_pairs");
-    hipLaunchKernelGGL(k_exp_count, dim3((E + 1 + TB - 1) / TB), dim3(TB), 0, s, *a);
-    dj_check(s, "k_exp_count");
-    if (dj_scan_counts(sc, a->exp_cnt, a->exp_pos, (size_t)E + 1, s) != 0) return -1;
-    dj_check(s, "rocprim_exclusive_scan");
-  }
-  hipLaunchKernelGGL(k_exp_emit, dim3((std::max<uint32_t>(E, 1) + TB - 1) / TB), dim3(TB), 0, s, *a);
-  dj_check(s, "k_exp_emit");
+    if (dj_scan_expiry(sc, a, E, s) != 0) return -1;
+  }
   if (n) {
     hipLaunchKernelGGL(k_group_walk, dim3((n + TB - 1) / TB), dim3(TB), 0, s, *a);
     dj_check(s, "k_group_walk");
     hipLaunchKernelGGL(k_group_walk_big, dim3(32), dim3(GWB_THREADS), 0, s, *a);
     dj_check(s, "k_group_walk_big");
-    if (dj_scan_counts(sc, a->out_cnt, a->out_pos, (size_t)n + 1, s) != 0) return -1;
-    dj_check(s, "rocprim_exclusive_scan");
-    hipLaunchKernelGGL(k_place, dim3((2 * n + TB - 1) / TB), dim3(TB), 0, s, *a);
-    dj_check(s, "k_place");
+    if (dj_scan_place(sc, a, n, s) != 0) return -1;
     hipLaunchKernelGGL(k_place_ovf, dim3(DJ_OVF_CAP / TB), dim3(TB), 0, s, *a);
     dj_check(s, "k_place_ovf");
   } else {
-    HIP_OK(hipMemsetAsync(a->out_pos, 0, 4, s));
-    hipLaunchKernelGGL(k_place, dim3(1), dim3(TB), 0, s, *a);
-    dj_check(s, "k_place");
-  }
-  hipLaunchKernelGGL(k_pool_fix, dim3(1), dim3(1), 0, s, a->counts);
-  dj_check(s, "k_pool_fix");
+    hipLaunchKernelGGL(k_place_none, dim3(1), dim3(1), 0, s, *a);
+    dj_check(s, "k_place_none");
+  }
   return 0;
 }
 
 int apm_dj_plan(DJFormatArgs* f, hipStream_t s) {
-  const uint32_t n = f->n_out;
-  hipLaunchKernelGGL(k_resolve_len, dim3((n + 1 + TB - 1) / TB), dim3(TB), 0, s, *f);
-  dj_check(s, "k_resolve_len");
   PrimScratch sc(f->tmp, f->tmp_bytes);
-  if (dj_scan_lens(sc, reinterpret_cast<const U4*>(f->lens), reinterpret_cast<U4*>(f->offs), (size_t)n + 1, s) != 0)
-    return -1;
-  dj_check(s, "rocprim_exclusive_scan (plan)");
-  hipLaunchKernelGGL(k_plan_totals, dim3(1), dim3(1), 0, s, *f);
-  dj_check(s, "k_plan_totals");
-  return 0;
+  return dj_plan(sc, f, f->n_out, s);
 }
 
 int apm_dj_write(DJFormatArgs* f, hipStream_t s) {
@@ -2436,11 +2542,9 @@
   hipLaunchKernelGGL(k_write, dim3((n + TXW_LINES - 1) / TXW_LINES), dim3(TXW_THREADS), 0, s, *f);
   dj_check(s, "k_write");
   PrimScratch sc(f->tmp, f->tmp_bytes);
-  if (dj_scan_bucket_max(sc, f->tx_bucket, f->tx_bmax, (size_t)n, s) != 0) return -1;
-  dj_check(s, "rocprim_inclusive_scan (bucket max)");
-  hipLaunchKernelGGL(k_cands, dim3((n + TB - 1) / TB), dim3(TB), 0, s, *f);
+  if (dj_scan_cands(sc, f, n, s) != 0) return -1;
   hipLaunchKernelGGL(k_reset_first, dim3((n + TB - 1) / TB), dim3(TB), 0, s, *f);
-  dj_check(s, "k_cands+k_reset_first");
+  dj_check(s, "k_reset_first");
   return 0;
 }
 
diff --git a/apmbackend_amd/csrc/kernels/devjoin_api.h b/apmbackend_amd/csrc/kernels/devjoin_api.h
--- a/apmbackend_amd/csrc/kernels/devjoin_api.h
+++ b/apmbackend_amd/csrc/kernels/devjoin_api.h
@@ -124,8 +124,6 @@
   uint64_t* exp_key_sorted;
   uint32_t* exp_idx;
   uint32_t* exp_idx_sorted;
-  uint32_t* exp_cnt;
-  uint32_t* exp_pos;
   uint32_t* out_cnt;
   uint32_t* out_pos;
   TxDev* stage;
@@ -162,7 +160,6 @@
   int32_t* tx_raw;
   int64_t* tx_gid;
   int64_t* tx_bucket;
-  int64_t* tx_bmax;
   uint32_t* cand;
   int64_t* cand_bucket;
   uint32_t* unresolved;
diff --git a/apmbackend_amd/csrc/kernels/devscan.h b/apmbackend_amd/csrc/kernels/devscan.h
--- a/apmbackend_amd/csrc/kernels/devscan.h
+++ b/apmbackend_amd/csrc/kernels/devscan.h
@@ -6,94 +6,129 @@
 namespace apm {
 
 constexpr int DS_BLOCK = 256, DS_ITEMS = 16, DS_TILE = DS_BLOCK * DS_ITEMS;
-constexpr int DS_TILES_BLOCK = 1024, DS_TILES_ITEMS = 4, DS_MAX_TILES = DS_TILES_BLOCK * DS_TILES_ITEMS;
+constexpr int DS_MAX_TILES = 4096;
+
+template <class T>
+struct DsPlus {
+  __device__ T identity() const { return T(0); }
+  __device__ T operator()(const T& a, const T& b) const { return a + b; }
+};
+template <class T>
+struct DsMax {
+  T lowest;
+  __device__ T identity() const { return lowest; }
+  __device__ T operator()(const T& a, const T& b) const { return a < b ? b : a; }
+};
+struct DsNoTotal {
+  template <class T>
+  __device__ void operator()(const T&) const {}
+};
 
 __device__ __forceinline__ uint32_t ds_count(const uint32_t* d_n, uint32_t cap) {
+  if (!d_n) return cap;
   const uint32_t n = *d_n;
   return n < cap ? n : cap;
 }
 
-template <class T, class F>
-__global__ __launch_bounds__(DS_BLOCK) void k_ds_reduce(F f, const uint32_t* __restrict__ d_n, uint32_t cap,
+template <class T, int ITEMS, class Op, class F>
+__global__ __launch_bounds__(DS_BLOCK) void k_ds_reduce(Op op, F f, const uint32_t* __restrict__ d_n, uint32_t cap,
                                                         T* __restrict__ tile_sum) {
   const uint32_t n = ds_count(d_n, cap);
-  const uint32_t t0 = blockIdx.x * (uint32_t)DS_TILE;
+  const uint32_t t0 = blockIdx.x * (uint32_t)(DS_BLOCK * ITEMS);
   if (t0 >= n) return;
-  T acc = 0;
+  T acc = op.identity();
 #pragma unroll
-  for (int k = 0; k < DS_ITEMS; ++k) {
+  for (int k = 0; k < ITEMS; ++k) {
     const uint32_t i = t0 + (uint32_t)k * DS_BLOCK + threadIdx.x;
-    if (i < n) acc += f(i);
+    if (i < n) acc = op(acc, f(i));
   }
   typedef rocprim::block_reduce<T, DS_BLOCK> R;
   __shared__ typename R::storage_type st;
   T s;
-  R().reduce(acc, s, st);
+  R().reduce(acc, s, st, op);
   if (threadIdx.x == 0) tile_sum[blockIdx.x] = s;
 }
 
-template <class T>
-__global__ __launch_bounds__(DS_TILES_BLOCK) void k_ds_tiles(T* __restrict__ tile_sum, const uint32_t* __restrict__ d_n,
-                                                             uint32_t cap, T* __restrict__ total) {
+template <class T, int ITEMS, class Op, class F, class G, class H>
+__global__ __launch_bounds__(DS_BLOCK) void k_ds_apply(Op op, F f, G g, H h, const uint32_t* __restrict__ d_n,
+                                                       uint32_t cap, const T* __restrict__ tile_sum,
+                                                       T* __restrict__ total) {
+  constexpr uint32_t TILE = (uint32_t)(DS_BLOCK * ITEMS);
   const uint32_t n = ds_count(d_n, cap);
-  const uint32_t nt = (n + DS_TILE - 1) / DS_TILE;
-  T v[DS_TILES_ITEMS];
+  if (n == 0) {
+    if (blockIdx.x == 0 && threadIdx.x == 0) {
+      if (total) *total = op.identity();
+      h(op.identity());
+    }
+    return;
+  }
+  const uint32_t t0 = blockIdx.x * TILE;
+  if (t0 >= n) return;
+  typedef rocprim::block_reduce<T, DS_BLOCK> R;
+  typedef rocprim::block_scan<T, DS_BLOCK> S;
+  __shared__ typename R::storage_type rst;
+  __shared__ typename S::storage_type sst;
+  __shared__ T s_off;
+  T off = op.identity();
+  if (blockIdx.x) {
+    T acc = op.identity();
+    for (uint32_t j = threadIdx.x; j < blockIdx.x; j += DS_BLOCK) acc = op(acc, tile_sum[j]);
+    T r;
+    R().reduce(acc, r, rst, op);
+    if (threadIdx.x == 0) s_off = r;
+    __syncthreads();
+    off = s_off;
+  }
+  const uint32_t i0 = t0 + threadIdx.x * (uint32_t)ITEMS;
+  T v[ITEMS];
+  T lane = op.identity();
 #pragma unroll
-  for (int k = 0; k < DS_TILES_ITEMS; ++k) {
-    const uint32_t j = threadIdx.x * DS_TILES_ITEMS + k;
-    v[k] = j < nt ? tile_sum[j] : T(0);
+  for (int k = 0; k < ITEMS; ++k) {
+    v[k] = i0 + k < n ? f(i0 + k) : op.identity();
+    lane = op(lane, v[k]);
   }
-  typedef rocprim::block_scan<T, DS_TILES_BLOCK> S;
-  __shared__ typename S::storage_type st;
-  T lane = 0;
+  T excl, tile;
+  S().exclusive_scan(lane, excl, op.identity(), tile, sst, op);
+  T p = op(off, excl);
 #pragma unroll
-  for (int k = 0; k < DS_TILES_ITEMS; ++k) lane += v[k];
-  T excl, sum;
-  S().exclusive_scan(lane, excl, T(0), sum, st);
-#pragma unroll
-  for (int k = 0; k < DS_TILES_ITEMS; ++k) {
-    const uint32_t j = threadIdx.x * DS_TILES_ITEMS + k;
-    if (j < nt) tile_sum[j] = excl;
-    excl += v[k];
+  for (int k = 0; k < ITEMS; ++k) {
+    if (i0 + k < n) g(i0 + k, p);
+    p = op(p, v[k]);
   }
-  if (threadIdx.x == 0) *total = sum;
-}
-
-template <class T, class F, class G>
-__global__ __launch_bounds__(DS_BLOCK) void k_ds_apply(F f, G g, const uint32_t* __restrict__ d_n, uint32_t cap,
-                                                       const T* __restrict__ tile_off) {
-  const uint32_t n = ds_count(d_n, cap);
-  const uint32_t t0 = blockIdx.x * (uint32_t)DS_TILE;
-  if (t0 >= n) return;
-  const uint32_t i0 = t0 + threadIdx.x * (uint32_t)DS_ITEMS;
-  T v[DS_ITEMS];
-  T lane = 0;
-#pragma unroll
-  for (int k = 0; k < DS_ITEMS; ++k) {
-    v[k] = i0 + k < n ? f(i0 + k) : T(0);
-    lane += v[k];
-  }
-  typedef rocprim::block_scan<T, DS_BLOCK> S;
-  __shared__ typename S::storage_type st;
-  T excl;
-  S().exclusive_scan(lane, excl, T(0), st);
-  T p = tile_off[blockIdx.x] + excl;
-#pragma unroll
-  for (int k = 0; k < DS_ITEMS; ++k) {
-    if (i0 + k < n) g(i0 + k, p);
-    p += v[k];
+  if (threadIdx.x == 0 && n - t0 <= TILE) {
+    const T t = op(off, tile);
+    if (total) *total = t;
+    h(t);
   }
 }
 
-template <class T, class F, class G>
-int ds_scan_apply(F f, G g, const uint32_t* d_n, uint32_t cap, T* tile_sum, T* total, hipStream_t s) {
-  const uint32_t tiles = (cap + DS_TILE - 1) / DS_TILE;
+template <int ITEMS>
+constexpr size_t ds_tiles(size_t cap) {
+  return (cap + (size_t)(DS_BLOCK * ITEMS) - 1) / (size_t)(DS_BLOCK * ITEMS) + 1;
+}
+
+template <class T, int ITEMS, class Op, class F, class G, class H>
+int ds_apply_op(Op op, F f, G g, H h, const uint32_t* d_n, uint32_t cap, const T* tile_sum, T* total, hipStream_t s) {
+  const uint32_t tiles = (uint32_t)ds_tiles<ITEMS>(cap) - 1;
   if (tiles > (uint32_t)DS_MAX_TILES) return -1;
-  if (tiles == 0) return 0;
-  hipLaunchKernelGGL((k_ds_reduce<T, F>), dim3(tiles), dim3(DS_BLOCK), 0, s, f, d_n, cap, tile_sum);
-  hipLaunchKernelGGL((k_ds_tiles<T>), dim3(1), dim3(DS_TILES_BLOCK), 0, s, tile_sum, d_n, cap, total);
-  hipLaunchKernelGGL((k_ds_apply<T, F, G>), dim3(tiles), dim3(DS_BLOCK), 0, s, f, g, d_n, cap, (const T*)tile_sum);
+  hipLaunchKernelGGL((k_ds_apply<T, ITEMS, Op, F, G, H>), dim3(tiles ? tiles : 1), dim3(DS_BLOCK), 0, s, op, f, g, h, d_n,
+                     cap, tile_sum, total);
   return 0;
 }
 
+template <class T, int ITEMS, class Op, class F, class G, class H>
+int ds_scan_apply_op(Op op, F f, G g, H h, const uint32_t* d_n, uint32_t cap, T* tile_sum, T* total, hipStream_t s) {
+  const uint32_t tiles = (uint32_t)ds_tiles<ITEMS>(cap) - 1;
+  if (tiles > (uint32_t)DS_MAX_TILES) return -1;
+  if (tiles)
+    hipLaunchKernelGGL((k_ds_reduce<T, ITEMS, Op, F>), dim3(tiles), dim3(DS_BLOCK), 0, s, op, f, d_n, cap, tile_sum);
+  return ds_apply_op<T, ITEMS>(op, f, g, h, d_n, cap, (const T*)tile_sum, total, s);
 }
+
+template <class T, class F, class G, class H = DsNoTotal>
+int ds_scan_apply(F f, G g, const uint32_t* d_n, uint32_t cap, T* tile_sum, T* total, hipStream_t s, H h = H()) {
+  if (cap == 0) return 0;
+  return ds_scan_apply_op<T, DS_ITEMS>(DsPlus<T>(), f, g, h, d_n, cap, tile_sum, total, s);
+}
+
+}
diff --git a/apmbackend_amd/csrc/runtime/devjoin.cpp b/apmbackend_amd/csrc/runtime/devjoin.cpp
--- a/apmbackend_amd/csrc/runtime/devjoin.cpp
+++ b/apmbackend_amd/csrc/runtime/devjoin.cpp
@@ -120,7 +120,6 @@
   d_lens_ = (uint32_t*)res_.dmalloc_on(stream_, ((size_t)out_cap_ + 1) * 16);
   d_offs_ = (uint32_t*)res_.dmalloc_on(stream_, ((size_t)out_cap_ + 1) * 16);
   d_bucket_ = (int64_t*)res_.dmalloc_on(stream_, (size_t)out_cap_ * 8);
-  d_bmax_ = (int64_t*)res_.dmalloc_on(stream_, (size_t)out_cap_ * 8);
   d_cand_ = (uint32_t*)res_.dmalloc_on(stream_, (size_t)out_cap_ * 4);
   d_cand_bucket_ = (int64_t*)res_.dmalloc_on(stream_, (size_t)out_cap_ * 8);
   d_unres_ = (uint32_t*)res_.dmalloc_on(stream_, (size_t)out_cap_ * 8);
@@ -158,8 +157,6 @@
   d_exp_key_sorted_ = (uint64_t*)res_.dmalloc_on(stream_, ((size_t)exp_cap_ + 1) * 8);
   d_exp_idx_ = (uint32_t*)res_.dmalloc_on(stream_, ((size_t)exp_cap_ + 1) * 4);
   d_exp_idx_sorted_ = (uint32_t*)res_.dmalloc_on(stream_, ((size_t)exp_cap_ + 1) * 4);
-  d_exp_cnt_ = (uint32_t*)res_.dmalloc_on(stream_, ((size_t)exp_cap_ + 1) * 4);
-  d_exp_pos_ = (uint32_t*)res_.dmalloc_on(stream_, ((size_t)exp_cap_ + 1) * 4);
   d_out_cnt_ = (uint32_t*)res_.dmalloc_on(stream_, ((size_t)E + 1) * 4);
   d_out_pos_ = (uint32_t*)res_.dmalloc_on(stream_, ((size_t)E + 1) * 4);
   d_stage_ = (TxDev*)res_.dmalloc_on(stream_, (size_t)E * 2 * sizeof(TxDev));
@@ -708,7 +705,7 @@
   res_.dfree(d_arena_);
   d_arena_ = fresh;
   for (void* p : {(void*)d_exp_key_, (void*)d_exp_key_sorted_}) res_.dfree(p);
-  for (void* p : {(void*)d_exp_idx_, (void*)d_exp_idx_sorted_, (void*)d_exp_cnt_, (void*)d_exp_pos_})
+  for (void* p : {(void*)d_exp_idx_, (void*)d_exp_idx_sorted_})
     res_.dfree(p);
   cfg_.arena_cap = new_cap;
   exp_cap_ = new_cap;
@@ -716,8 +713,6 @@
   d_exp_key_sorted_ = (uint64_t*)res_.dmalloc_on(stream_, ((size_t)exp_cap_ + 1) * 8);
   d_exp_idx_ = (uint32_t*)res_.dmalloc_on(stream_, ((size_t)exp_cap_ + 1) * 4);
   d_exp_idx_sorted_ = (uint32_t*)res_.dmalloc_on(stream_, ((size_t)exp_cap_ + 1) * 4);
-  d_exp_cnt_ = (uint32_t*)res_.dmalloc_on(stream_, ((size_t)exp_cap_ + 1) * 4);
-  d_exp_pos_ = (uint32_t*)res_.dmalloc_on(stream_, ((size_t)exp_cap_ + 1) * 4);
   ensure_tmp();
   ++arena_grows_;
 }
@@ -910,7 +905,7 @@
   a.arena = d_arena_; a.arena_cap = cfg_.arena_cap; a.arena_base = arena_head_; a.arena_limit = arena_limit;
   a.exp_lo = d_exp_lo_; a.exp_hi = d_exp_hi_; a.n_exp_regions = n_reg; a.n_exp_entries = n_exp;
   a.exp_key = d_exp_key_; a.exp_key_sorted = d_exp_key_sorted_; a.exp_idx = d_exp_idx_;
-  a.exp_idx_sorted = d_exp_idx_sorted_; a.exp_cnt = d_exp_cnt_; a.exp_pos = d_exp_pos_;
+  a.exp_idx_sorted = d_exp_idx_sorted_;
   a.out_cnt = d_out_cnt_; a.out_pos = d_out_pos_; a.stage = d_stage_; a.ovf = d_ovf_;
   a.out = d_out_; a.out_cap = out_cap_; a.counts = d_counts_;
   {
@@ -987,7 +982,7 @@
   f.raw = d_rawtab_; f.raw_series = d_raw_series_; f.raw_first = d_raw_first_; f.names = d_names_;
   f.bytes = s.d_bytes; f.hbuf = d_hbuf_; f.aud_txt = aud_gen_[aud_cur_].txt; f.arena = d_arena_; f.arena_cap = cfg_.arena_cap; f.pool = d_pool_;
   f.lens = d_lens_; f.offs = d_offs_; f.ring = d_ring_; f.ring_cap = cfg_.ring_bytes;
-  f.tx = s.d_tx; f.tx_raw = s.d_tx_raw; f.tx_gid = s.d_tx_gid; f.tx_bucket = d_bucket_; f.tx_bmax = d_bmax_;
+  f.tx = s.d_tx; f.tx_raw = s.d_tx_raw; f.tx_gid = s.d_tx_gid; f.tx_bucket = d_bucket_;
   f.cand = d_cand_; f.cand_bucket = d_cand_bucket_; f.unresolved = d_unres_;
   f.want_tx = want_tx; f.want_db = want_db; f.counts = d_counts_; f.tmp = d_tmp_; f.tmp_bytes = tmp_bytes_;
   const uint64_t ring_head = ring_head_.load(std::memory_order_acquire);
@@ -1436,15 +1431,13 @@
       cfg_.arena_cap = saved_cap;
       d_arena_ = (NeedEnt*)res_.dmalloc_on(stream_, (size_t)cfg_.arena_cap * sizeof(NeedEnt));
       for (void* p : {(void*)d_exp_key_, (void*)d_exp_key_sorted_}) res_.dfree(p);
-      for (void* p : {(void*)d_exp_idx_, (void*)d_exp_idx_sorted_, (void*)d_exp_cnt_, (void*)d_exp_pos_})
+      for (void* p : {(void*)d_exp_idx_, (void*)d_exp_idx_sorted_})
         res_.dfree(p);
       exp_cap_ = saved_cap;
       d_exp_key_ = (uint64_t*)res_.dmalloc_on(stream_, ((size_t)exp_cap_ + 1) * 8);
       d_exp_key_sorted_ = (uint64_t*)res_.dmalloc_on(stream_, ((size_t)exp_cap_ + 1) * 8);
       d_exp_idx_ = (uint32_t*)res_.dmalloc_on(stream_, ((size_t)exp_cap_ + 1) * 4);
       d_exp_idx_sorted_ = (uint32_t*)res_.dmalloc_on(stream_, ((size_t)exp_cap_ + 1) * 4);
-      d_exp_cnt_ = (uint32_t*)res_.dmalloc_on(stream_, ((size_t)exp_cap_ + 1) * 4);
-      d_exp_pos_ = (uint32_t*)res_.dmalloc_on(stream_, ((size_t)exp_cap_ + 1) * 4);
       ensure_tmp();
     }
   }
diff --git a/apmbackend_amd/csrc/runtime/devjoin.h b/apmbackend_amd/csrc/runtime/devjoin.h
--- a/apmbackend_amd/csrc/runtime/devjoin.h
+++ b/apmbackend_amd/csrc/runtime/devjoin.h
@@ -260,7 +260,6 @@
   uint32_t* d_lens_ = nullptr;
   uint32_t* d_offs_ = nullptr;
   int64_t* d_bucket_ = nullptr;
-  int64_t* d_bmax_ = nullptr;
   uint32_t* d_cand_ = nullptr;
   int64_t* d_cand_bucket_ = nullptr;
   uint32_t* d_unres_ = nullptr;
@@ -293,7 +292,7 @@
   uint64_t* d_chain_hash_ = nullptr;
   uint32_t *d_op_slot_ = nullptr, *d_op_slot_sorted_ = nullptr, *d_op_idx_ = nullptr, *d_op_idx_sorted_ = nullptr;
   uint64_t *d_exp_key_ = nullptr, *d_exp_key_sorted_ = nullptr;
-  uint32_t *d_exp_idx_ = nullptr, *d_exp_idx_sorted_ = nullptr, *d_exp_cnt_ = nullptr, *d_exp_pos_ = nullptr;
+  uint32_t *d_exp_idx_ = nullptr, *d_exp_idx_sorted_ = nullptr;
   uint32_t exp_cap_ = 0;
   uint32_t* d_out_cnt_ = nullptr;
   uint32_t* d_out_pos_ = nullptr;
```

After: 316.9 million. -3.4%, worse.
